# google-research/Splat-SLAM

Measured on AMD Instinct MI355X. Metric: mapping frames/sec + render ms @640x480, 300k Gaussians; PSNR vs ref, higher is better.
Workload: dtype f32

## Files before the change

include/splat_hip.h:

```cpp
#ifndef SPLAT_HIP_H_
#define SPLAT_HIP_H_

#include <stddef.h>
#include <stdint.h>

#ifdef __cplusplus
extern "C" {
#endif

#define SGR_ABI_VERSION 10

#define SGR_HOST

typedef enum SgrStatus {
  SGR_OK = 0,
  SGR_ERR_INVALID = -1,
  SGR_ERR_WORKSPACE = -2,
  SGR_ERR_CAPACITY = -3,
  SGR_ERR_HIP = -4
} SgrStatus;

typedef struct SgrSettings {
  int32_t num_gaussians;
  int32_t image_height;
  int32_t image_width;
  int32_t sh_degree;
  int32_t sh_coeffs;
  float tanfovx;
  float tanfovy;
  float scale_modifier;
  int32_t prefiltered;
  int32_t debug;
  const float* bg;
  const float* viewmatrix;
  const float* projmatrix;
  const float* projmatrix_raw;
  const float* campos;
} SgrSettings;

typedef struct SgrInputs {
  const float* means3D;
  const float* opacities;
  const float* shs;
  const float* colors_precomp;
  const float* scales;
  const float* rotations;
  const float* cov3D_precomp;
} SgrInputs;

typedef struct SgrOutputs {
  float* color;
  float* depth;
  float* opacity;
  int32_t* radii;
  int32_t* n_touched;
} SgrOutputs;

typedef struct SgrWorkspace {
  void* saved;
  size_t saved_bytes;
  void* scratch;
  size_t scratch_bytes;
  int64_t capacity;
  int32_t counters_clean;
  int32_t max_list_hint;
} SgrWorkspace;

typedef struct SgrGradOutputs {
  const float* dL_dcolor;
  const float* dL_ddepth;
} SgrGradOutputs;

typedef struct SgrGradInputs {
  float* dL_dmeans3D;
  float* dL_dmeans2D;
  float* dL_dopacities;
  float* dL_dshs;
  float* dL_dcolors_precomp;
  float* dL_dscales;
  float* dL_drotations;
  float* dL_dcov3D_precomp;
  float* dL_dtau;
  int32_t accumulate;
  float* stat_grad_accum;
  float* stat_denom;
  float* stat_max_radii;
} SgrGradInputs;

int sgr_abi_version(void);
const char* sgr_last_error(void);

size_t sgr_saved_bytes(int32_t num_gaussians, int32_t image_height, int32_t image_width, int64_t capacity);
size_t sgr_scratch_bytes(int32_t num_gaussians, int32_t image_height, int32_t image_width, int64_t capacity);

int sgr_forward(const SgrSettings* settings, const SgrInputs* in, const SgrOutputs* out,
                const SgrWorkspace* ws, SGR_HOST int64_t* num_rendered_host, void* stream);

int sgr_backward(const SgrSettings* settings, const SgrInputs* in, const int32_t* radii,
                 const SgrGradOutputs* grad_out, const SgrGradInputs* grad_in,
                 const SgrWorkspace* ws, void* stream);

typedef struct SgrBackwardView {
  SgrSettings settings;
  const int32_t* radii;
  SgrWorkspace ws;
  const float* dL_dcolor;
  const float* dL_ddepth;
  float* dL_dmeans2D;
  float* dL_dtau;
} SgrBackwardView;
int sgr_backward_views(int32_t num_views, const SgrBackwardView* views, const SgrInputs* in, const SgrGradInputs* grad_in,
                       void* stream);

int sgr_densify_stats(int64_t n, const float* dL_dmeans2D, const int32_t* radii, float* stat_grad_accum, float* stat_denom,
                      float* stat_max_radii, void* stream);

int sgr_query(const void* saved, SGR_HOST int64_t* num_rendered_host, SGR_HOST int32_t* overflow_host, void* stream);

int sgr_query_header(const void* saved, SGR_HOST uint32_t words_host[16], void* stream);

int sgr_header_to_host(const void* saved, void* pinned_host64, void* stream);

int sgr_query_stats(const SgrWorkspace* ws, int32_t num_gaussians, int32_t image_height, int32_t image_width,
                    const int32_t* radii, SGR_HOST int64_t stats_host[4], void* stream);
int sgr_query_depth_keys(const SgrWorkspace* ws, int32_t num_gaussians, int32_t image_height, int32_t image_width,
                         const int32_t* radii, float* depth_out, void* stream);
int sgr_query_list_histogram(const SgrWorkspace* ws, int32_t num_gaussians, int32_t image_height, int32_t image_width,
                             SGR_HOST int64_t hist_host[8], void* stream);

#define SGR_OPT_FUSED_BLEND 0
#define SGR_OPT_UPSTREAM_POSE_JACOBIAN 1
#define SGR_OPT_SEGMENT_TEST 2
#define SGR_OPT_COUNT 3
int sgr_set_option(int32_t option, int32_t value);
int sgr_get_option(int32_t option);

#define SGR_PROFILE_KINDS 7
int sgr_profile_enable(uint32_t kind_mask);
int sgr_profile_read(SGR_HOST float ms_host[SGR_PROFILE_KINDS], SGR_HOST int64_t launches_host[SGR_PROFILE_KINDS]);

int sgr_mapping_loss(int32_t H, int32_t W, const float* image, const float* depth,
                     const float* gt_image, const float* gt_depth,
                     const float* exposure_a, const float* exposure_b,
                     float alpha, float rgb_boundary_threshold, float upstream,
                     float* loss, float* dL_dimage, float* dL_ddepth, float* dL_dexp_a, float* dL_dexp_b,
                     void* scratch, size_t scratch_bytes, void* stream);

size_t sgr_ssim_scratch_bytes(int32_t B, int32_t C, int32_t H, int32_t W);
int sgr_ssim(int32_t B, int32_t C, int32_t H, int32_t W, const float* img1, const float* img2, float* ssim_out, float* maps,
             void* scratch, size_t scratch_bytes, void* stream);
int sgr_ssim_backward(int32_t B, int32_t C, int32_t H, int32_t W, const float* img1, const float* img2, const float* maps,
                      const float* upstream, int32_t upstream_stride, float upstream_scale, float* dL_dimg1, void* stream);

typedef struct SgrMetricFrame {
  const float* render;
  const float* gt_image;
  const float* depth;
  const float* gt_depth;
  const float* exposure_a;
  const float* exposure_b;
} SgrMetricFrame;
int sgr_render_metrics(int32_t n, const SgrMetricFrame* frames, int32_t C, int32_t H, int32_t W, float global_scale, float* out,
                       void* scratch, size_t scratch_bytes, void* stream);

#define SGR_TSDF_UNIT_FLOATS (5 * 4096)
#define SGR_TSDF_MAX_FRAMES 16
typedef struct SgrTsdfVolume {
  float voxel_length;
  float sdf_trunc;
  float depth_trunc;
  int32_t hash_capacity;
  int32_t pool_capacity;
  void* state;
  float* pool;
} SgrTsdfVolume;
typedef struct SgrTsdfFrame {
  const float* render;
  const float* depth;
  const float* gt_depth;
  const float* exposure_a;
  const float* exposure_b;
  float fx, fy, cx, cy;
  float w2c[16];
  float global_scale;
} SgrTsdfFrame;
size_t sgr_tsdf_bytes(int32_t hash_capacity);
int sgr_tsdf_reset(const SgrTsdfVolume* vol, void* stream);
int sgr_tsdf_rehash(const SgrTsdfVolume* src, const SgrTsdfVolume* dst, void* stream);
int sgr_tsdf_touch(const SgrTsdfVolume* vol, int32_t n, const SgrTsdfFrame* frames, int32_t H, int32_t W, void* stream);
int sgr_tsdf_integrate(const SgrTsdfVolume* vol, int32_t n, const SgrTsdfFrame* frames, int32_t H, int32_t W, int32_t n_touched,
                       void* stream);
size_t sgr_tsdf_extract_bytes(int32_t hash_capacity, int32_t pool_capacity);
int sgr_tsdf_extract_count(const SgrTsdfVolume* vol, int32_t n_units, void* scratch, size_t scratch_bytes, int32_t* totals,
                           void* stream);
int sgr_tsdf_extract(const SgrTsdfVolume* vol, int32_t n_units, void* scratch, size_t scratch_bytes, float* vertices,
                     float* colors, int32_t* triangles, void* stream);
size_t sgr_mesh_bytes(int32_t V, int32_t F);
int sgr_mesh_components(int32_t V, int32_t F, const float* vertices, const int32_t* triangles, int32_t min_len, void* scratch,
                        size_t scratch_bytes, int32_t* totals, void* stream);
int sgr_mesh_compact(int32_t V, int32_t F, const float* vertices, const float* colors, const int32_t* triangles, void* scratch,
                     size_t scratch_bytes, float* out_vertices, float* out_colors, int32_t* out_triangles, int32_t* vertex_map,
                     void* stream);

size_t sgr_surface_sample_bytes(int32_t F);
int sgr_surface_sample(int32_t V, int32_t F, const float* vertices, const int32_t* triangles, int32_t n, uint64_t seed, void* scratch,
                       size_t scratch_bytes, float* points, int32_t* tri_idx, double* total_area, void* stream);
size_t sgr_nn_grid_bytes(int32_t n);
int sgr_nn_grid_build(int32_t n, const float* points, SGR_HOST const float* transform, void* grid, size_t grid_bytes, void* stream);
int sgr_nn_query(int32_t n, const void* grid, size_t grid_bytes, int32_t nq, const float* query, SGR_HOST const float* transform,
                 float max_dist, float* dist, int32_t* idx, void* stream);
size_t sgr_eval_reduce_bytes(void);
int sgr_icp_accumulate(int32_t n, const float* source, SGR_HOST const float* transform, const int32_t* idx, int32_t n_target,
                       const float* target, double* sums, void* scratch, size_t scratch_bytes, void* stream);
int sgr_cloud_metrics(int32_t na, const float* dist_a, int32_t nb, const float* dist_b, float thresh, double* out, void* scratch,
                      size_t scratch_bytes, void* stream);

#define SGR_CULL_MAX_FRAMES 16
#define SGR_CULL_SUBPIXEL_BITS 8
#define SGR_CULL_GUARD_PIXELS 16384
#define SGR_CULL_RULE_ALL 0
#define SGR_CULL_RULE_ANY 1
typedef struct SgrCullFrame {
  double w2c[12];
  double fx, fy, cx, cy;
} SgrCullFrame;
int sgr_cull_project(int32_t V, const float* vertices, int32_t n, const SgrCullFrame* frames, double near, int32_t* xy, float* z,
                     void* stream);
size_t sgr_cull_raster_bytes(int32_t F, int32_t n);
int sgr_cull_raster(int32_t V, int32_t F, const int32_t* triangles, int32_t n, const int32_t* xy, const float* z, int32_t H, int32_t W,
                    float* depth, int32_t* skipped, void* scratch, size_t scratch_bytes, void* stream);
int sgr_cull_visibility(int32_t V, int32_t n, const int32_t* xy, const float* z, const float* depth, int32_t H, int32_t W, int32_t edge,
                        float far, float eps, int32_t* seen, void* stream);
size_t sgr_cull_select_bytes(int32_t V, int32_t F);
int sgr_cull_select(int32_t V, int32_t F, const int32_t* triangles, const int32_t* seen, int32_t min_views, int32_t rule, void* scratch,
                    size_t scratch_bytes, int32_t* totals, void* stream);
int sgr_cull_compact(int32_t V, int32_t F, const float* vertices, const float* colors, const int32_t* triangles, void* scratch,
                     size_t scratch_bytes, float* out_vertices, float* out_colors, int32_t* out_triangles, int32_t* vertex_map,
                     void* stream);

int sgr_adam_step(int64_t n, float* param, const float* grad, float* exp_avg, float* exp_avg_sq,
                  float lr, float beta1, float beta2, float eps, int64_t step, void* stream);

typedef struct SgrAdamTensor {
  float* param;
  const float* grad;
  float* exp_avg;
  float* exp_avg_sq;
  int64_t n;
  int64_t step;
} SgrAdamTensor;
int sgr_adam_step_multi(int32_t count, const SgrAdamTensor* tensors, float lr, float beta1, float beta2, float eps, void* stream);

int sgr_activate(int64_t n, const float* scaling, const float* rotation, const float* opacity,
                 float* scales_out, float* rot_out, float* opac_out, void* stream);

typedef struct SgrAdamGroup {
  float* param;
  float* grad;
  float* exp_avg;
  float* exp_avg_sq;
  float lr;
  int32_t skip;
  int64_t step;
} SgrAdamGroup;
int sgr_gaussian_adam_step(int64_t n, const SgrAdamGroup groups[5], float beta1, float beta2, float eps,
                           float iso_weight, void* stream);

int sgr_gaussian_adam_shard(int64_t n_total, const SgrAdamGroup groups[5], SGR_HOST const int64_t row0[5],
                            SGR_HOST const int64_t row1[5], float beta1, float beta2, float eps, float iso_weight, void* stream);

typedef struct SgrMapView {
  SgrSettings settings;
  SgrOutputs out;
  SgrWorkspace ws;
  const float* gt_image;
  const float* gt_depth;
  const float* exposure_a;
  const float* exposure_b;
  float* loss;
  float* dL_dimage;
  float* dL_ddepth;
  float* dL_dexposure;
  float* dL_dtau;
  void* loss_scratch;
  size_t loss_scratch_bytes;
} SgrMapView;
// ... 567 lines not shown
```

splat_slam_amd/csrc/sgr_api.hip:

```cpp
#include <cstdarg>
#include <cstdio>
#include <cstring>
#include <cstdlib>
#include <vector>

#include <hip/hip_runtime.h>

#include "sgr_common.h"

namespace sgr {

void launch_preprocess_fwd(const ViewTab&, int, const LOff&, const Common&, const SgrInputs&, hipStream_t);
void launch_preprocess_bwd(const ViewTab&, int, const LOff&, const Common&, const SgrInputs&, const SgrGradInputs&, const FusedAdam*,
                           hipStream_t, bool mapping_loop = false);
void launch_binning(const ViewTab&, int, const LOff&, hipStream_t);
void launch_zero_heads(const ViewTab&, int, const LOff&, size_t, hipStream_t);
void launch_blend_fwd(const ViewTab&, int, const LOff&, const float*, const LossTab*, const LossCoef*, hipStream_t);
void launch_blend_bwd(const ViewTab&, int, const LOff&, const float*, const LossTab*, const LossCoef*, hipStream_t);
void launch_blend_fused(const ViewTab&, int, const LOff&, const float*, const LossTab&, const LossCoef&, hipStream_t);
bool blend_can_fuse(const LOff&);

static int g_opt[SGR_OPT_COUNT] = {1, 0, 0};

static thread_local char g_err[512] = "";
int set_error(int code, const char* fmt, ...) {
  va_list ap;
  va_start(ap, fmt);
  vsnprintf(g_err, sizeof(g_err), fmt, ap);
  va_end(ap);
  return code;
}
#define HIP_TRY(expr)                                                                                   \
  do {                                                                                                  \
    hipError_t _e = (expr);                                                                             \
    if (_e != hipSuccess) return set_error(SGR_ERR_HIP, "%s failed: %s", #expr, hipGetErrorString(_e)); \
  } while (0)

int debug_flags() {
  static int f = -1;
  if (f < 0) { const char* e = getenv("SGR_DEBUG"); f = e ? atoi(e) : 0; }
  return f | (g_opt[SGR_OPT_SEGMENT_TEST] ? 0 : 4);
}

static Layout make_layout(int N, int H, int W, int64_t cap) { return Layout(N, H, W, cap); }

struct ProfState {
  static constexpr int kRing = 2048;
  uint32_t mask = 0;
  hipEvent_t ev[SGR_PROFILE_KINDS][kRing][2];
  bool created[SGR_PROFILE_KINDS] = {};
  int used[SGR_PROFILE_KINDS] = {};
  double ms[SGR_PROFILE_KINDS] = {};
  int64_t launches[SGR_PROFILE_KINDS] = {};
};
static ProfState g_prof;
static void prof_drain(int k) {
  for (int i = 0; i < g_prof.used[k]; ++i) {
    float t = 0.f;
    if (hipEventSynchronize(g_prof.ev[k][i][1]) == hipSuccess &&
        hipEventElapsedTime(&t, g_prof.ev[k][i][0], g_prof.ev[k][i][1]) == hipSuccess) {
      g_prof.ms[k] += t;
      g_prof.launches[k] += 1;
    }
  }
  g_prof.used[k] = 0;
}
void prof_begin(int k, hipStream_t st) {
  if (!(g_prof.mask & (1u << k))) return;
  if (!g_prof.created[k]) {
    for (int i = 0; i < ProfState::kRing; ++i) { (void)hipEventCreate(&g_prof.ev[k][i][0]); (void)hipEventCreate(&g_prof.ev[k][i][1]); }
    g_prof.created[k] = true;
  }
  if (g_prof.used[k] == ProfState::kRing) prof_drain(k);
  (void)hipEventRecord(g_prof.ev[k][g_prof.used[k]][0], st);
}
void prof_end(int k, hipStream_t st) {
  if (!(g_prof.mask & (1u << k))) return;
  (void)hipEventRecord(g_prof.ev[k][g_prof.used[k]][1], st);
  g_prof.used[k] += 1;
}

__global__ void __launch_bounds__(256) stats_kernel(int N, int ntiles, const int32_t* __restrict__ radii,
                                                     const uint2* __restrict__ ranges, const uint32_t* __restrict__ tile_maxc,
                                                     unsigned long long* __restrict__ out) {
  unsigned long long v = 0, r = 0, re = 0, ne = 0;
  for (int i = blockIdx.x * blockDim.x + threadIdx.x; i < N; i += gridDim.x * blockDim.x) v += radii[i] > 0;
  for (int t = blockIdx.x * blockDim.x + threadIdx.x; t < ntiles; t += gridDim.x * blockDim.x) {
    uint32_t c = ranges[(size_t)t * kRngStride].y - (ranges[(size_t)t * kRngStride].x & ~kOverfull);
    r += c; re += min(c, tile_maxc[t]); ne += c > 0;
  }
  atomicAdd(&out[0], v); atomicAdd(&out[1], r); atomicAdd(&out[2], re); atomicAdd(&out[3], ne);
}

__global__ void __launch_bounds__(256) hist_kernel(int ntiles, const uint2* __restrict__ ranges, const uint32_t* __restrict__ tile_maxc,
                                                    unsigned long long* __restrict__ out) {
  for (int t = blockIdx.x * blockDim.x + threadIdx.x; t < ntiles; t += gridDim.x * blockDim.x) {
    uint32_t c = ranges[(size_t)t * kRngStride].y - (ranges[(size_t)t * kRngStride].x & ~kOverfull);
    c = min(c, tile_maxc[t]);
    int b = c == 0 ? 0 : c <= 4 ? 1 : c <= 8 ? 2 : c <= 16 ? 3 : c <= 32 ? 4 : c <= 64 ? 5 : c <= 256 ? 6 : 7;
    atomicAdd(&out[b], 1ull);
  }
}


__global__ void __launch_bounds__(256) depth_keys_kernel(int N, const GRec* __restrict__ grec, const int32_t* __restrict__ radii,
                                                          float* __restrict__ out) {
  const int i = blockIdx.x * blockDim.x + threadIdx.x;
  if (i < N) out[i] = radii[i] > 0 ? grec[i].depth : 0.f;
}

static int check_settings(const SgrSettings* s, const SgrInputs* in) {
  const int N = s->num_gaussians, H = s->image_height, W = s->image_width;
  if (N < 0 || H <= 0 || W <= 0) return set_error(SGR_ERR_INVALID, "bad sizes N=%d H=%d W=%d", N, H, W);
  if (H > 65535 * kTile || W > 65535 * kTile) return set_error(SGR_ERR_INVALID, "image too large");
  if (!s->bg || !s->viewmatrix || !s->projmatrix || !s->projmatrix_raw || !s->campos)
    return set_error(SGR_ERR_INVALID, "settings: bg/viewmatrix/projmatrix/projmatrix_raw/campos must be device pointers");
  if (N > 0) {
    if (!in->means3D || !in->opacities) return set_error(SGR_ERR_INVALID, "means3D and opacities are required");
    if ((in->shs != nullptr) == (in->colors_precomp != nullptr))
      return set_error(SGR_ERR_INVALID, "Please provide excatly one of either SHs or precomputed colors!");
    if (((in->scales != nullptr) && (in->rotations != nullptr)) == (in->cov3D_precomp != nullptr) ||
        ((in->scales != nullptr) != (in->rotations != nullptr)))
      return set_error(SGR_ERR_INVALID, "Please provide exactly one of either scale/rotation pair or precomputed 3D covariance!");
    if (in->shs && (s->sh_degree < 0 || s->sh_degree > 3 || s->sh_coeffs < (s->sh_degree + 1) * (s->sh_degree + 1)))
      return set_error(SGR_ERR_INVALID, "sh_degree %d needs %d coefficients, shs has %d", s->sh_degree,
                       (s->sh_degree + 1) * (s->sh_degree + 1), s->sh_coeffs);
  }
  return SGR_OK;
}

static int check_workspace(const SgrWorkspace* ws, const Layout& L) {
  if (ws->capacity <= 0 || ws->capacity > 0xffffffffll) return set_error(SGR_ERR_INVALID, "bad capacity %lld", (long long)ws->capacity);
  if (!ws->saved || ws->saved_bytes < L.saved_bytes)
    return set_error(SGR_ERR_WORKSPACE, "saved workspace too small: %zu < %zu", ws->saved_bytes, L.saved_bytes);
  if (!ws->scratch || ws->scratch_bytes < L.scratch_bytes)
    return set_error(SGR_ERR_WORKSPACE, "scratch workspace too small: %zu < %zu", ws->scratch_bytes, L.scratch_bytes);
  return SGR_OK;
}

static Common make_common(const SgrSettings* s) {
  Common c;
  c.deg = s->sh_degree; c.M = s->sh_coeffs; c.tanfovx = s->tanfovx; c.tanfovy = s->tanfovy; c.mod = s->scale_modifier;
  c.bg = s->bg;
  c.upstream_pose_jac = g_opt[SGR_OPT_UPSTREAM_POSE_JACOBIAN];
  return c;
}

static void tab_set_view(ViewTab& t, int v, const SgrSettings* s, const SgrOutputs* out, const SgrWorkspace* ws) {
  t.viewmatrix[v] = s->viewmatrix; t.projmatrix[v] = s->projmatrix; t.campos[v] = s->campos; t.projraw[v] = s->projmatrix_raw;
  t.saved[v] = (char*)ws->saved; t.scratch[v] = (char*)ws->scratch;
  if (out) {
    t.color[v] = out->color; t.depth[v] = out->depth; t.opacity[v] = out->opacity; t.radii[v] = out->radii;
    t.n_touched[v] = out->n_touched;
  }
}

static int forward_batch(const ViewTab& tab, int nviews, const Layout& L, const Common& cm, const SgrInputs& in, hipStream_t st,
                         bool counters_clean = false, int max_list_hint = 0) {
  LOff d = L.dev();
  d.set_hint(max_list_hint);
  if (!counters_clean) launch_zero_heads(tab, nviews, d, L.zero_bytes, st);
  launch_preprocess_fwd(tab, nviews, d, cm, in, st);
  launch_binning(tab, nviews, d, st);
  return SGR_OK;
}

}

using namespace sgr;

extern "C" {

int sgr_abi_version(void) { return SGR_ABI_VERSION; }
const char* sgr_last_error(void) { return g_err; }

size_t sgr_saved_bytes(int32_t N, int32_t H, int32_t W, int64_t cap) { return make_layout(N, H, W, cap).saved_bytes; }
size_t sgr_scratch_bytes(int32_t N, int32_t H, int32_t W, int64_t cap) { return make_layout(N, H, W, cap).scratch_bytes; }

int sgr_forward(const SgrSettings* s, const SgrInputs* in, const SgrOutputs* out, const SgrWorkspace* ws,
                int64_t* num_rendered_host, void* stream) {
  if (!s || !in || !out || !ws) return set_error(SGR_ERR_INVALID, "null argument");
  if (int rc = check_settings(s, in)) return rc;
  const int N = s->num_gaussians;
  if (!out->color || !out->depth || !out->opacity || (N > 0 && (!out->radii || !out->n_touched)))
    return set_error(SGR_ERR_INVALID, "null output pointer");
  Layout L = make_layout(N, s->image_height, s->image_width, ws->capacity);
  if (int rc = check_workspace(ws, L)) return rc;
  hipStream_t st = (hipStream_t)stream;
  ViewTab tab = {};
  tab_set_view(tab, 0, s, out, ws);
  Common cm = make_common(s);
  if (int rc = forward_batch(tab, 1, L, cm, *in, st, ws->counters_clean != 0, ws->max_list_hint)) return rc;
  if (num_rendered_host) {
    uint32_t h2[2] = {0u, 0u};
    HIP_TRY(hipMemcpyAsync(h2, (char*)ws->saved + L.o_hdr, 8, hipMemcpyDeviceToHost, st));
    HIP_TRY(hipStreamSynchronize(st));
    const uint32_t R = h2[0];
    *num_rendered_host = R;
    if (h2[1] == 2u)
      return set_error(SGR_ERR_INVALID, "more than %u splats on one 8x8 tile: the map has degenerated (16-bit tile counters)", kTileCountLimit);
    if ((int64_t)R > L.cap) return set_error(SGR_ERR_CAPACITY, "%u (tile, Gaussian) pairs exceed capacity %lld", R, (long long)L.cap);
  }
  LOff d1 = L.dev();
  d1.set_hint(ws->max_list_hint);
  launch_blend_fwd(tab, 1, d1, s->bg, nullptr, nullptr, st);
  HIP_TRY(hipGetLastError());
  return SGR_OK;
}

int sgr_backward(const SgrSettings* s, const SgrInputs* in, const int32_t* radii, const SgrGradOutputs* go,
                 const SgrGradInputs* gi, const SgrWorkspace* ws, void* stream) {
  if (!s || !in || !go || !gi || !ws) return set_error(SGR_ERR_INVALID, "null argument");
  if (int rc = check_settings(s, in)) return rc;
  const int N = s->num_gaussians;
  if (!go->dL_dcolor) return set_error(SGR_ERR_INVALID, "dL_dcolor is required");
  if (N > 0 && !radii) return set_error(SGR_ERR_INVALID, "radii is required");
  if (gi->stat_grad_accum && (!gi->stat_denom || !gi->stat_max_radii))
    return set_error(SGR_ERR_INVALID, "stat_grad_accum needs stat_denom and stat_max_radii");
  Layout L = make_layout(N, s->image_height, s->image_width, ws->capacity);
  if (int rc = check_workspace(ws, L)) return rc;
  hipStream_t st = (hipStream_t)stream;
  if (N == 0) {
    if (gi->dL_dtau) HIP_TRY(hipMemsetAsync(gi->dL_dtau, 0, 24, st));
    return SGR_OK;
  }
  ViewTab tab = {};
  tab_set_view(tab, 0, s, nullptr, ws);
  tab.radii[0] = const_cast<int32_t*>(radii);
  tab.dL_dcolor[0] = go->dL_dcolor; tab.dL_ddepth[0] = go->dL_ddepth; tab.dL_dtau[0] = gi->dL_dtau;
  LOff d = L.dev();
  Common cm = make_common(s);
  launch_blend_bwd(tab, 1, d, s->bg, nullptr, nullptr, st);
  launch_preprocess_bwd(tab, 1, d, cm, *in, *gi, nullptr, st);
  HIP_TRY(hipGetLastError());
  return SGR_OK;
}

}

__global__ void __launch_bounds__(256) densify_stats_kernel(int64_t n, const float* __restrict__ m2, const int32_t* __restrict__ radii,
                                                            float* __restrict__ accum, float* __restrict__ denom, float* __restrict__ maxr) {
#pragma clang fp contract(off)
  const int64_t i = (int64_t)blockIdx.x * blockDim.x + threadIdx.x;
  if (i >= n) return;
  const int r = radii[i];
  if (r <= 0) return;
  const F3 g = ld3(m2 + 3 * i);
  accum[i] += sqrtf(g.x * g.x + g.y * g.y);
  denom[i] += 1.f;
  maxr[i] = fmaxf(maxr[i], (float)r);
}

extern "C" {

int sgr_densify_stats(int64_t n, const float* dL_dmeans2D, const int32_t* radii, float* stat_grad_accum, float* stat_denom,
                      float* stat_max_radii, void* stream) {
  if (n < 0 || (n > 0 && (!dL_dmeans2D || !radii || !stat_grad_accum || !stat_denom || !stat_max_radii)))
    return set_error(SGR_ERR_INVALID, "densify_stats: null argument");
  if (n > 0)
    hipLaunchKernelGGL(densify_stats_kernel, dim3((unsigned)((n + 255) / 256)), dim3(256), 0, (hipStream_t)stream, n, dL_dmeans2D, radii,
                       stat_grad_accum, stat_denom, stat_max_radii);
  HIP_TRY(hipGetLastError());
  return SGR_OK;
}

int sgr_backward_views(int32_t num_views, const SgrBackwardView* views, const SgrInputs* in, const SgrGradInputs* grad_in, void* stream) {
  if (num_views < 0 || (num_views > 0 && (!views || !in || !grad_in))) return set_error(SGR_ERR_INVALID, "backward_views: null argument");
  if (num_views == 0) return SGR_OK;
  hipStream_t st = (hipStream_t)stream;
  const SgrBackwardView& f = views[0];
  bool uniform = in->shs && in->scales && in->rotations && !in->colors_precomp && !in->cov3D_precomp && f.settings.sh_degree == 0 &&
                 f.settings.num_gaussians > 0;
  for (int v = 0; v < num_views; ++v) {
    const SgrBackwardView& m = views[v];
    if (int rc = check_settings(&m.settings, in)) return rc;
    if (!m.dL_dcolor || (m.settings.num_gaussians > 0 && !m.radii)) return set_error(SGR_ERR_INVALID, "backward_views: dL_dcolor and radii are required");
    uniform = uniform && m.settings.num_gaussians == f.settings.num_gaussians && m.settings.image_height == f.settings.image_height &&
              m.settings.image_width == f.settings.image_width && m.settings.tanfovx == f.settings.tanfovx &&
              m.settings.tanfovy == f.settings.tanfovy && m.settings.scale_modifier == f.settings.scale_modifier &&
              m.settings.sh_degree == f.settings.sh_degree && m.settings.sh_coeffs == f.settings.sh_coeffs &&
              m.settings.bg == f.settings.bg && m.ws.capacity == f.ws.capacity;
    for (int u = 0; u < v; ++u) uniform = uniform && views[u].ws.scratch != m.ws.scratch && views[u].ws.saved != m.ws.saved;
  }
  SgrGradInputs g = *grad_in;
  g.dL_dmeans2D = nullptr;
  g.dL_dtau = nullptr;
  if (!uniform) {
    for (int v = 0; v < num_views; ++v) {
      const SgrBackwardView& m = views[v];
      const int N = m.settings.num_gaussians;
      Layout L = make_layout(N, m.settings.image_height, m.settings.image_width, m.ws.capacity);
      if (int rc = check_workspace(&m.ws, L)) return rc;
      if (N == 0) {
        if (m.dL_dtau) HIP_TRY(hipMemsetAsync(m.dL_dtau, 0, 24, st));
        continue;
      }
      ViewTab tab = {};
      tab_set_view(tab, 0, &m.settings, nullptr, &m.ws);
      tab.radii[0] = const_cast<int32_t*>(m.radii);
      tab.dL_dcolor[0] = m.dL_dcolor; tab.dL_ddepth[0] = m.dL_ddepth; tab.dL_dtau[0] = m.dL_dtau; tab.dL_dmeans2D[0] = m.dL_dmeans2D;
      SgrGradInputs gv = g;
      gv.accumulate = (grad_in->accumulate || v > 0) ? 1 : 0;
      Common cm = make_common(&m.settings);
      LOff d = L.dev();
      launch_blend_bwd(tab, 1, d, m.settings.bg, nullptr, nullptr, st);
      launch_preprocess_bwd(tab, 1, d, cm, *in, gv, nullptr, st);
    }
    HIP_TRY(hipGetLastError());
    return SGR_OK;
  }
  Layout L = make_layout(f.settings.num_gaussians, f.settings.image_height, f.settings.image_width, f.ws.capacity);
  LOff d = L.dev();
  Common cm = make_common(&f.settings);
  for (int base = 0; base < num_views; base += kMaxViews) {
    const int nv = num_views - base < kMaxViews ? num_views - base : kMaxViews;
    ViewTab tab = {};
    for (int v = 0; v < nv; ++v) {
      const SgrBackwardView& m = views[base + v];
      if (int rc = check_workspace(&m.ws, L)) return rc;
      tab_set_view(tab, v, &m.settings, nullptr, &m.ws);
      tab.radii[v] = const_cast<int32_t*>(m.radii);
      tab.dL_dcolor[v] = m.dL_dcolor; tab.dL_ddepth[v] = m.dL_ddepth; tab.dL_dtau[v] = m.dL_dtau; tab.dL_dmeans2D[v] = m.dL_dmeans2D;
    }
    SgrGradInputs gv = g;
    gv.accumulate = (grad_in->accumulate || base > 0) ? 1 : 0;
    launch_blend_bwd(tab, nv, d, f.settings.bg, nullptr, nullptr, st);
    launch_preprocess_bwd(tab, nv, d, cm, *in, gv, nullptr, st);
  }
  HIP_TRY(hipGetLastError());
  return SGR_OK;
}

}

static int map_views_impl(int32_t num_views, const SgrMapView* views, const SgrInputs* in, const SgrGradInputs* grads, float alpha,
                          float rgb_boundary_threshold, int32_t forward_only, FusedAdam* fused, bool* fused_done,
                          void* stream, bool store_sinks = false, const SgrSsimTerm* term = nullptr) {
  if (fused_done) *fused_done = false;
  if (num_views < 0 || (num_views > 0 && (!views || !in)) || (!forward_only && !grads))
    return set_error(SGR_ERR_INVALID, "map_views: null argument");
  if (num_views == 0) return SGR_OK;
  if (forward_only) term = nullptr;
  if (term) {
    if (!term->arena || term->max_views <= 0)
      return set_error(SGR_ERR_INVALID, "map_views: SSIM term without an arena");
    for (int v = 0; v < num_views; ++v) {
      const SgrMapView& m = views[v];
      const int H = m.settings.image_height, W = m.settings.image_width;
      if (!m.out.color || !m.out.depth || !m.out.opacity)
        return set_error(SGR_ERR_INVALID, "map_views: the SSIM loss needs every view's rendered image, depth and opacity");
      if (term->arena_bytes < sgr_ssim_term_bytes(term->max_views, H, W))
        return set_error(SGR_ERR_WORKSPACE, "map_views: SSIM arena too small (need %zu for %d views of %dx%d)",
                         sgr_ssim_term_bytes(term->max_views, H, W), term->max_views, W, H);
      if (!m.loss_scratch || m.loss_scratch_bytes < (size_t)ssim_loss_nparts(H, W) * sizeof(LossPart))
        return set_error(SGR_ERR_WORKSPACE, "map_views: loss_scratch too small for the SSIM loss (need %zu)",
                         (size_t)ssim_loss_nparts(H, W) * sizeof(LossPart));
    }
  }
  hipStream_t st = (hipStream_t)stream;
  bool uniform = true;
  const SgrMapView& f = views[0];
  for (int v = 0; v < num_views; ++v) {
    const SgrMapView& m = views[v];
    if (int rc = check_settings(&m.settings, in)) return rc;
    uniform = uniform && m.settings.num_gaussians == f.settings.num_gaussians && m.settings.image_height == f.settings.image_height &&
              m.settings.image_width == f.settings.image_width && m.settings.tanfovx == f.settings.tanfovx &&
              m.settings.tanfovy == f.settings.tanfovy && m.settings.scale_modifier == f.settings.scale_modifier &&
              m.settings.sh_degree == f.settings.sh_degree && m.settings.sh_coeffs == f.settings.sh_coeffs &&
              m.settings.bg == f.settings.bg &&
              m.ws.capacity == f.ws.capacity;
    if (num_views > 1) uniform = uniform && in->shs && m.settings.sh_degree == 0 && in->scales && in->rotations;
    for (int u = 0; u < v; ++u) uniform = uniform && views[u].ws.scratch != m.ws.scratch && views[u].ws.saved != m.ws.saved;
    if (!forward_only && grads && !grads->accumulate && num_views > 1)
      return set_error(SGR_ERR_INVALID, "map_views: several views need accumulate != 0");
  }
  if (store_sinks && !forward_only && grads && !(fused && uniform && f.settings.num_gaussians > 0 && num_views <= kMaxViews)) {
    const size_t n = (size_t)f.settings.num_gaussians, m = (size_t)(f.settings.sh_coeffs > 0 ? f.settings.sh_coeffs : 1);
    if (grads->dL_dmeans3D) HIP_TRY(hipMemsetAsync(grads->dL_dmeans3D, 0, n * 12, st));
    if (grads->dL_dshs) HIP_TRY(hipMemsetAsync(grads->dL_dshs, 0, n * m * 12, st));
    if (grads->dL_dopacities) HIP_TRY(hipMemsetAsync(grads->dL_dopacities, 0, n * 4, st));
    if (grads->dL_dscales) HIP_TRY(hipMemsetAsync(grads->dL_dscales, 0, n * 12, st));
    if (grads->dL_drotations) HIP_TRY(hipMemsetAsync(grads->dL_drotations, 0, n * 16, st));
  }
  if (!uniform || f.settings.num_gaussians == 0) {
    for (int v = 0; v < num_views; ++v) {
      const SgrMapView& mv = views[v];
      if (!mv.out.color || !mv.out.depth || !mv.out.opacity || !mv.out.n_touched)
        return set_error(SGR_ERR_INVALID, "map_views: outputs may only be omitted in uniform batches");
      if (int rc = sgr_forward(&mv.settings, in, &mv.out, &mv.ws, nullptr, stream)) return rc;
      if (forward_only) continue;
      if (term) {
        if (int rc = sgr_mapping_loss_ssim(mv.settings.image_height, mv.settings.image_width, mv.out.color, mv.out.depth, mv.gt_image,
                                           mv.gt_depth, mv.exposure_a, mv.exposure_b, alpha, rgb_boundary_threshold, 1.0f, term,
                                           mv.loss, mv.dL_dimage, mv.dL_ddepth, mv.dL_dexposure,
                                           mv.dL_dexposure ? mv.dL_dexposure + 1 : nullptr, stream))
          return rc;
      } else if (int rc = sgr_mapping_loss(mv.settings.image_height, mv.settings.image_width, mv.out.color, mv.out.depth, mv.gt_image,
                                           mv.gt_depth, mv.exposure_a, mv.exposure_b, alpha, rgb_boundary_threshold, 1.0f, mv.loss,
                                           mv.dL_dimage, mv.dL_ddepth, mv.dL_dexposure, mv.dL_dexposure ? mv.dL_dexposure + 1 : nullptr,
                                           mv.loss_scratch, mv.loss_scratch_bytes, stream)) {
        return rc;
      }
      SgrGradOutputs go = {mv.dL_dimage, mv.dL_ddepth};
      SgrGradInputs gi = *grads;
      gi.dL_dtau = mv.dL_dtau;
      if (int rc = sgr_backward(&mv.settings, in, mv.out.radii, &go, &gi, &mv.ws, stream)) return rc;
    }
    return SGR_OK;
  }
  Layout L = make_layout(f.settings.num_gaussians, f.settings.image_height, f.settings.image_width, f.ws.capacity);
  LOff d = L.dev();
  int hint = 0;
  for (int v = 0; v < num_views; ++v) hint = views[v].ws.max_list_hint > hint ? views[v].ws.max_list_hint : hint;
  d.set_hint(hint);
  Common cm = make_common(&f.settings);
  const int HW = f.settings.image_height * f.settings.image_width;
  for (int base = 0; base < num_views; base += kMaxViews) {
    const int nv = num_views - base < kMaxViews ? num_views - base : kMaxViews;
    ViewTab tab = {};
    LossTab lt = {};
    bool all_clean = true;
    for (int v = 0; v < nv; ++v) {
      const SgrMapView& m = views[base + v];
      all_clean = all_clean && m.ws.counters_clean != 0;
      if (int rc = check_workspace(&m.ws, L)) return rc;
      const bool no_images = !m.out.color && !m.out.depth && !m.out.opacity && !forward_only;
      if ((!no_images && (!m.out.color || !m.out.depth || !m.out.opacity)) || !m.out.radii)
        return set_error(SGR_ERR_INVALID, "map_views: null output pointer");
      tab_set_view(tab, v, &m.settings, &m.out, &m.ws);
      if (!forward_only) {
        if (!m.gt_image || !m.gt_depth || !m.dL_dimage || !m.dL_ddepth || !m.loss_scratch ||
            m.loss_scratch_bytes < (size_t)L.ntiles * sizeof(LossPart))
          return set_error(SGR_ERR_INVALID, "map_views: loss buffers missing (loss_scratch needs 16 B per 8x8 tile = %zu)",
                           (size_t)L.ntiles * sizeof(LossPart));
        tab.dL_dcolor[v] = m.dL_dimage; tab.dL_ddepth[v] = m.dL_ddepth; tab.dL_dtau[v] = m.dL_dtau;
        lt.image[v] = m.out.color; lt.depth[v] = m.out.depth; lt.gt_image[v] = m.gt_image; lt.gt_depth[v] = m.gt_depth;
        lt.exp_a[v] = m.exposure_a; lt.exp_b[v] = m.exposure_b; lt.loss[v] = m.loss; lt.dimage[v] = m.dL_dimage;
        lt.ddepth[v] = m.dL_ddepth; lt.da[v] = m.dL_dexposure; lt.db[v] = m.dL_dexposure ? m.dL_dexposure + 1 : nullptr;
        lt.parts[v] = m.loss_scratch;
      }
    }
    if (int rc = forward_batch(tab, nv, L, cm, *in, st, all_clean, d.mean_hint)) return rc;
    if (forward_only) {
      launch_blend_fwd(tab, nv, d, f.settings.bg, nullptr, nullptr, st);
      continue;
    }
    LossCoef lc = {alpha / (3.f * (float)HW), (1.f - alpha) / (float)HW, rgb_boundary_threshold};
    const bool fused_blend = !term && g_opt[SGR_OPT_FUSED_BLEND] != 0 && blend_can_fuse(d);
    int nparts = L.ntiles;
    if (term) {
      const int H = f.settings.image_height, W = f.settings.image_width;
      launch_blend_fwd(tab, nv, d, f.settings.bg, nullptr, nullptr, st);
      for (int g0 = 0; g0 < nv; g0 += term->max_views)
        launch_ssim_mapping_loss(lt, g0, nv - g0 < term->max_views ? nv - g0 : term->max_views, H, W, alpha, term->lambda_dssim,
                                 rgb_boundary_threshold, 1.f, (float*)term->arena, st);
      nparts = ssim_loss_nparts(H, W);
    } else if (fused_blend) {
      launch_blend_fused(tab, nv, d, f.settings.bg, lt, lc, st);
    } else {
      launch_blend_fwd(tab, nv, d, f.settings.bg, &lt, &lc, st);
    }
    const bool fuse = fused && num_views <= kMaxViews;
    if (fuse) {
      fused->tail_views = nv; fused->tail_nparts = nparts;
      fused->tail_inv_rgb = 1.f / (3.f * (float)HW); fused->tail_inv_dep = 1.f / (float)HW; fused->tail_alpha = alpha;
      for (int v = 0; v < nv; ++v) {
        fused->tail_parts[v] = lt.parts[v]; fused->tail_loss[v] = lt.loss[v]; fused->tail_da[v] = lt.da[v]; fused->tail_db[v] = lt.db[v];
      }
    } else {
      launch_mapping_loss_final(lt, nv, HW, nparts, alpha, st);
    }
    if (term) launch_blend_bwd(tab, nv, d, f.settings.bg, nullptr, nullptr, st);
    else if (!fused_blend) launch_blend_bwd(tab, nv, d, f.settings.bg, &lt, &lc, st);
    launch_preprocess_bwd(tab, nv, d, cm, *in, *grads, fuse ? fused : nullptr, st, true);
    if (fuse && fused_done) *fused_done = true;
  }
  HIP_TRY(hipGetLastError());
  return SGR_OK;
}

extern "C" {

int sgr_map_views(int32_t num_views, const SgrMapView* views, const SgrInputs* in, const SgrGradInputs* grads, float alpha,
                  float rgb_boundary_threshold, int32_t forward_only, void* stream) {
  return map_views_impl(num_views, views, in, grads, alpha, rgb_boundary_threshold, forward_only, nullptr, nullptr, stream);
}

}

static int map_step_impl(const SgrMapStep* p, bool skip_activate, bool grads_clean, bool allow_fuse, bool* fused_out, void* stream,
                         const SgrSsimTerm* term = nullptr) {
  if (fused_out) *fused_out = false;
  if (!p) return set_error(SGR_ERR_INVALID, "map_step: null argument");
  const bool adam_only = p->num_views == 0 && p->adam_groups;
  if (!skip_activate && !adam_only && (p->scaling || p->rotation || p->opacity))
    if (int rc = sgr_activate(p->num_gaussians, p->scaling, p->rotation, p->opacity, p->scales_out, p->rot_out, p->opac_out, stream)) return rc;
  FusedAdam fa;
  bool try_fuse = false;
  if (allow_fuse && p->adam_groups && p->num_views > 0 && p->num_views <= kMaxViews && !p->forward_only && p->grads && p->in && p->views) {
    const SgrGradInputs& g = *p->grads;
    const SgrAdamGroup* G = p->adam_groups;
    try_fuse = g.accumulate && g.dL_dmeans3D == G[0].grad && g.dL_dshs == G[1].grad && g.dL_dopacities == G[2].grad &&
               g.dL_dscales == G[3].grad && g.dL_drotations == G[4].grad && !g.dL_dmeans2D && !g.dL_dcolors_precomp &&
               !g.dL_dcov3D_precomp && p->in->shs && !p->in->colors_precomp && p->in->scales && p->in->rotations &&
               p->num_gaussians == p->views[0].settings.num_gaussians;
    for (int v = 0; v < p->num_views && try_fuse; ++v)
      try_fuse = !p->views[v].dL_dtau && p->views[v].settings.sh_degree == 0 && p->views[v].settings.sh_coeffs == 1;
    if (try_fuse) {
      if (int rc = make_fused_adam(p->num_gaussians, G, p->beta1, p->beta2, p->eps, p->iso_weight, &fa)) return rc;
      fa.grads_clean = grads_clean ? 1 : 0;
      fa.s_out = p->scales_out; fa.r_out = p->rot_out; fa.o_out = p->opac_out;
      fa.stat_accum = g.stat_grad_accum;
      fa.stat_denom = g.stat_grad_accum ? g.stat_denom : nullptr;
      fa.stat_maxr = g.stat_grad_accum ? g.stat_max_radii : nullptr;
      if (p->exp_rows > 0) {
        if (!p->exp_param || !p->exp_grad || !p->exp_avg || !p->exp_avg_sq || !p->exp_step || !p->exp_active || p->exp_row_width <= 0)
          return set_error(SGR_ERR_INVALID, "map_step: exposure block incomplete");
        fa.exp_rows = p->exp_rows; fa.exp_width = p->exp_row_width; fa.exp_param = p->exp_param; fa.exp_grad = p->exp_grad;
        fa.exp_avg = p->exp_avg; fa.exp_avg_sq = p->exp_avg_sq; fa.exp_step = p->exp_step; fa.exp_active = p->exp_active;
        fa.exp_lr = p->exp_lr; fa.exp_b1 = p->exp_beta1; fa.exp_b2 = p->exp_beta2; fa.exp_eps = p->exp_eps;
      }
    }
  }
  if ((p->grads_clean == -2 || p->grads_clean == -3) && !p->adam_groups && p->num_views > 0 && p->num_views <= kMaxViews && !p->forward_only && p->grads &&
      p->in && p->views) {
    const SgrGradInputs& g = *p->grads;
    try_fuse = g.accumulate && g.dL_dmeans3D && g.dL_dshs && g.dL_dopacities && g.dL_dscales && g.dL_drotations &&
               !g.dL_dmeans2D && !g.dL_dcolors_precomp && !g.dL_dcov3D_precomp && p->in->shs && !p->in->colors_precomp &&
               p->in->scales && p->in->rotations && p->num_gaussians == p->views[0].settings.num_gaussians;
    for (int v = 0; v < p->num_views && try_fuse; ++v)
      try_fuse = !p->views[v].dL_dtau && p->views[v].settings.sh_degree == 0 && p->views[v].settings.sh_coeffs == 1;
    if (try_fuse) {
      fa = FusedAdam{};
      fa.gather_only = p->grads_clean == -3 ? 2 : 1;
      fa.G.g[0].grad = g.dL_dmeans3D; fa.G.g[1].grad = g.dL_dshs; fa.G.g[2].grad = g.dL_dopacities;
      fa.G.g[3].grad = g.dL_dscales; fa.G.g[4].grad = g.dL_drotations;
      fa.stat_accum = g.stat_grad_accum;
      fa.stat_denom = g.stat_grad_accum ? g.stat_denom : nullptr;
      fa.stat_maxr = g.stat_grad_accum ? g.stat_max_radii : nullptr;
      if (p->exp_rows > 0) {
        if (!p->exp_param || !p->exp_grad || !p->exp_avg || !p->exp_avg_sq || !p->exp_step || !p->exp_active || p->exp_row_width <= 0)
          return set_error(SGR_ERR_INVALID, "map_step: exposure block incomplete");
        fa.exp_rows = p->exp_rows; fa.exp_width = p->exp_row_width; fa.exp_param = p->exp_param; fa.exp_grad = p->exp_grad;
        fa.exp_avg = p->exp_avg; fa.exp_avg_sq = p->exp_avg_sq; fa.exp_step = p->exp_step; fa.exp_active = p->exp_active;
        fa.exp_lr = p->exp_lr; fa.exp_b1 = p->exp_beta1; fa.exp_b2 = p->exp_beta2; fa.exp_eps = p->exp_eps;
      }
    }
  }
  bool fused = false;
  if (p->num_views > 0)
    if (int rc = map_views_impl(p->num_views, p->views, p->in, p->grads, p->alpha, p->rgb_boundary_threshold, p->forward_only,
                                try_fuse ? &fa : nullptr, &fused, stream, p->grads_clean == -3 && !p->adam_groups, term))
      return rc;
  if (p->adam_groups && !fused)
    if (int rc = gaussian_adam_step_act(p->num_gaussians, p->adam_groups, p->beta1, p->beta2, p->eps, p->iso_weight,
                                        adam_only && p->scaling ? p->scales_out : nullptr,
                                        adam_only && p->rotation ? p->rot_out : nullptr,
                                        adam_only && p->opacity ? p->opac_out : nullptr, stream))
      return rc;
  if (p->exp_rows > 0 && !fused)
    if (int rc = sgr_masked_adam(p->exp_rows, p->exp_row_width, p->exp_param, p->exp_grad, p->exp_avg, p->exp_avg_sq, p->exp_step,
                                 p->exp_active, p->exp_lr, p->exp_beta1, p->exp_beta2, p->exp_eps, stream))
      return rc;
  if (fused_out) *fused_out = fused;
  return SGR_OK;
}

extern "C" {

int sgr_map_step(const SgrMapStep* p, void* stream) {
  if (!p) return set_error(SGR_ERR_INVALID, "map_step: null argument");
  return map_step_impl(p, false, p->grads_clean > 0, p->grads_clean >= 0, nullptr, stream);
}

int sgr_map_step_ssim(const SgrMapStep* p, const SgrSsimTerm* term, void* stream) {
  if (!p) return set_error(SGR_ERR_INVALID, "map_step: null argument");
  return map_step_impl(p, false, p->grads_clean > 0, p->grads_clean >= 0, nullptr, stream, term);
}

}

static int map_run_impl(const SgrMapRun* r, const SgrSsimTerm* term, void* stream) {
  if (!r || r->num_iters < 0 || r->num_window < 0 || r->picks_per_iter < 0 || (r->num_window > 0 && !r->window) ||
      (r->picks_per_iter > 0 && (!r->pool || !r->picks || r->pool_size <= 0)))
    return set_error(SGR_ERR_INVALID, "map_run: bad argument");
  const int nv = r->num_window + r->picks_per_iter;
  if (nv > 64) return set_error(SGR_ERR_INVALID, "map_run: more than 64 views per iteration");
  SgrMapView views[64];
  for (int v = 0; v < r->num_window; ++v) views[v] = r->window[v];
  std::vector<char> pool_used((size_t)(r->pool_size > 0 ? r->pool_size : 0), 0);
  std::vector<char> slot_used((size_t)(r->picks_per_iter > 0 ? r->picks_per_iter : 0), 0);
  SgrMapStep st = r->step;
  st.views = views;
  st.num_views = nv;
  st.adam_groups = r->adam_groups;
  const int32_t exp_rows = st.exp_rows;
  bool prev_fused = false;
  for (int it = 0; it < r->num_iters; ++it) {
    for (int j = 0; j < r->picks_per_iter; ++j) {
      const int32_t k = r->picks[(size_t)it * r->picks_per_iter + j];
      if (k < 0 || k >= r->pool_size) return set_error(SGR_ERR_INVALID, "map_run: pick %d outside the pool", k);
      views[r->num_window + j] = r->pool[k];
      if (r->pick_ws) {
        views[r->num_window + j].ws = r->pick_ws[j];
        if (slot_used[j]) views[r->num_window + j].ws.counters_clean = 1;
        slot_used[j] = 1;
      } else if (pool_used[k]) {
        views[r->num_window + j].ws.counters_clean = 1;
      }
      pool_used[k] = 1;
    }
    if (it == 1)
      for (int v = 0; v < r->num_window; ++v) views[v].ws.counters_clean = 1;
    if (r->n_touched_last_only) {
      const bool last = it == r->num_iters - 1;
      for (int v = 0; v < r->num_window; ++v) views[v].out.n_touched = last ? r->window[v].out.n_touched : nullptr;
      if (!last)
        for (int j = 0; j < r->picks_per_iter; ++j) views[r->num_window + j].out.n_touched = nullptr;
    }
    if (r->adam_groups) {
      if (r->lr0) r->adam_groups[0].lr = r->lr0[it];
      for (int g = 0; g < 5; ++g)
        if (!r->adam_groups[g].skip) r->adam_groups[g].step += 1;
    }
    if (r->pool_exp_row && r->picks_per_iter > 0 && exp_rows > 0) {
      const int32_t row = r->pool_exp_row[r->picks[(size_t)it * r->picks_per_iter]];
      const size_t o = (size_t)(row < 0 ? 0 : row) * (size_t)st.exp_row_width;
      st.exp_rows = row < 0 ? 0 : 1;
      st.exp_param = r->step.exp_param + o; st.exp_grad = r->step.exp_grad + o;
      st.exp_avg = r->step.exp_avg + o; st.exp_avg_sq = r->step.exp_avg_sq + o;
      st.exp_step = r->step.exp_step + (row < 0 ? 0 : row);
    }
    bool fused = false;
    if (int rc = map_step_impl(&st, prev_fused, it == 0 ? r->step.grads_clean > 0 : r->adam_groups != nullptr, r->step.grads_clean >= 0,
                               &fused, stream, term))
      return rc;
    prev_fused = fused;
  }
  return SGR_OK;
}

extern "C" {

int sgr_map_run(const SgrMapRun* r, void* stream) { return map_run_impl(r, nullptr, stream); }
int sgr_map_run_ssim(const SgrMapRun* r, const SgrSsimTerm* term, void* stream) { return map_run_impl(r, term, stream); }

int sgr_query_stats(const SgrWorkspace* ws, int32_t N, int32_t H, int32_t W, const int32_t* radii, int64_t stats_host[4],
                    void* stream) {
  if (!ws || !ws->saved || !ws->scratch || !stats_host) return set_error(SGR_ERR_INVALID, "null argument");
  Layout L = make_layout(N, H, W, ws->capacity);
  hipStream_t st = (hipStream_t)stream;
  unsigned long long* d = (unsigned long long*)ws->scratch;
  HIP_TRY(hipMemsetAsync(d, 0, 32, st));
  hipLaunchKernelGGL(stats_kernel, dim3(64), dim3(256), 0, st, N, L.ntiles, radii, (const uint2*)((char*)ws->saved + L.o_ranges),
                     (const uint32_t*)((char*)ws->saved + L.o_tile_maxc), d);
  unsigned long long h[4];
  HIP_TRY(hipMemcpyAsync(h, d, 32, hipMemcpyDeviceToHost, st));
  HIP_TRY(hipStreamSynchronize(st));
  for (int i = 0; i < 4; ++i) stats_host[i] = (int64_t)h[i];
  return SGR_OK;
}

int sgr_query_depth_keys(const SgrWorkspace* ws, int32_t N, int32_t H, int32_t W, const int32_t* radii, float* depth_out, void* stream) {
  if (!ws || !ws->saved || !radii || !depth_out) return set_error(SGR_ERR_INVALID, "null argument");
  Layout L = make_layout(N, H, W, ws->capacity);
  if (N > 0)
    hipLaunchKernelGGL(depth_keys_kernel, dim3((N + 255) / 256), dim3(256), 0, (hipStream_t)stream, N,
                       (const GRec*)((const char*)ws->saved + L.o_grec), radii, depth_out);
  HIP_TRY(hipGetLastError());
  return SGR_OK;
}

int sgr_query_list_histogram(const SgrWorkspace* ws, int32_t N, int32_t H, int32_t W, int64_t hist_host[8], void* stream) {
  if (!ws || !ws->saved || !ws->scratch || !hist_host) return set_error(SGR_ERR_INVALID, "null argument");
  Layout L = make_layout(N, H, W, ws->capacity);
  hipStream_t st = (hipStream_t)stream;
  unsigned long long* d = (unsigned long long*)ws->scratch;
  HIP_TRY(hipMemsetAsync(d, 0, 64, st));
  hipLaunchKernelGGL(hist_kernel, dim3(32), dim3(256), 0, st, L.ntiles, (const uint2*)((char*)ws->saved + L.o_ranges),
                     (const uint32_t*)((char*)ws->saved + L.o_tile_maxc), d);
  unsigned long long h[8];
  HIP_TRY(hipMemcpyAsync(h, d, 64, hipMemcpyDeviceToHost, st));
  HIP_TRY(hipStreamSynchronize(st));
  for (int i = 0; i < 8; ++i) hist_host[i] = (int64_t)h[i];
  return SGR_OK;
}

int sgr_set_option(int32_t option, int32_t value) {
  if (option < 0 || option >= SGR_OPT_COUNT) return set_error(SGR_ERR_INVALID, "unknown option %d", option);
  g_opt[option] = value;
  return SGR_OK;
}

int sgr_get_option(int32_t option) { return option >= 0 && option < SGR_OPT_COUNT ? g_opt[option] : -1; }

int sgr_profile_enable(uint32_t kind_mask) {
  g_prof.mask = kind_mask & ((1u << SGR_PROFILE_KINDS) - 1);
  return SGR_OK;
}

int sgr_profile_read(float ms_host[SGR_PROFILE_KINDS], int64_t launches_host[SGR_PROFILE_KINDS]) {
  for (int k = 0; k < SGR_PROFILE_KINDS; ++k) {
    prof_drain(k);
    if (ms_host) ms_host[k] = (float)g_prof.ms[k];
    if (launches_host) launches_host[k] = g_prof.launches[k];
    g_prof.ms[k] = 0.0;
    g_prof.launches[k] = 0;
  }
  return SGR_OK;
}

int sgr_header_to_host(const void* saved, void* pinned_host64, void* stream) {
  if (!saved || !pinned_host64) return set_error(SGR_ERR_INVALID, "null argument");
  HIP_TRY(hipMemcpyAsync(pinned_host64, saved, sizeof(SavedHeader), hipMemcpyDeviceToHost, (hipStream_t)stream));
  return SGR_OK;
}

int sgr_query_header(const void* saved, uint32_t words_host[16], void* stream) {
  if (!saved || !words_host) return set_error(SGR_ERR_INVALID, "null argument");
  static_assert(sizeof(SavedHeader) == 64, "header is 16 words");
  HIP_TRY(hipMemcpyAsync(words_host, saved, sizeof(SavedHeader), hipMemcpyDeviceToHost, (hipStream_t)stream));
  HIP_TRY(hipStreamSynchronize((hipStream_t)stream));
  return SGR_OK;
}

int sgr_query(const void* saved, int64_t* num_rendered_host, int32_t* overflow_host, void* stream) {
  if (!saved) return set_error(SGR_ERR_INVALID, "null saved block");
  SavedHeader h;
  HIP_TRY(hipMemcpyAsync(&h, saved, sizeof(h), hipMemcpyDeviceToHost, (hipStream_t)stream));
  HIP_TRY(hipStreamSynchronize((hipStream_t)stream));
  if (num_rendered_host) *num_rendered_host = h.num_rendered;
  if (overflow_host) *overflow_host = (int32_t)h.overflow;
  return SGR_OK;
}

}
```

splat_slam_amd/csrc/sgr_aux.hip:

```cpp
#include <cmath>

#include <cstdint>

#include "sgr_common.h"
#include "sgr_se3_device.h"

namespace sgr {
int set_error(int code, const char* fmt, ...);


__global__ void __launch_bounds__(256) mapping_loss_kernel(LossTab tab, int HW, float w_rgb, float w_dep, float thr) {
  const int vw = blockIdx.y;
  const float* __restrict__ image = tab.image[vw];
  const float* __restrict__ depth = tab.depth[vw];
  const float* __restrict__ gt_image = tab.gt_image[vw];
  const float* __restrict__ gt_depth = tab.gt_depth[vw];
  float* __restrict__ dimage = tab.dimage[vw];
  float* __restrict__ ddepth = tab.ddepth[vw];
  LossPart* __restrict__ parts = (LossPart*)tab.parts[vw];
  const float ea = tab.exp_a[vw] ? __expf(tab.exp_a[vw][0]) : 1.f;
  const float eb = tab.exp_b[vw] ? tab.exp_b[vw][0] : 0.f;
  LossPart acc = {0.f, 0.f, 0.f, 0.f};
  for (int p = blockIdx.x * blockDim.x + threadIdx.x; p < HW; p += gridDim.x * blockDim.x) {
    float g0 = gt_image[p], g1 = gt_image[HW + p], g2 = gt_image[2 * HW + p];
    bool m = (g0 + g1 + g2) > thr;
    float gt[3] = {g0, g1, g2};
#pragma unroll
    for (int c = 0; c < 3; ++c) {
      float I = image[c * HW + p];
      float r = m ? (ea * I + eb) - gt[c] : 0.f;
      acc.rgb += fabsf(r);
      float sgn = (r > 0.f) ? 1.f : ((r < 0.f) ? -1.f : 0.f);
      float dab = w_rgb * sgn;
      if (dimage) dimage[c * HW + p] = dab * ea;
      acc.da += dab * ea * I;
      acc.db += dab;
    }
    float gd = gt_depth[p];
    bool md = gd > 0.01f;
    float rd = md ? depth[p] - gd : 0.f;
    acc.dep += fabsf(rd);
    if (ddepth) ddepth[p] = w_dep * ((rd > 0.f) ? 1.f : ((rd < 0.f) ? -1.f : 0.f));
  }
  __shared__ LossPart red[4];
  float v[4] = {acc.rgb, acc.dep, acc.da, acc.db};
#pragma unroll
  for (int k = 0; k < 4; ++k) v[k] = wave_sum(v[k]);
  int lane = threadIdx.x & 63, wv = threadIdx.x >> 6;
  if (lane == 0) red[wv] = {v[0], v[1], v[2], v[3]};
  __syncthreads();
  if (threadIdx.x == 0) {
    LossPart t = red[0];
    for (int w = 1; w < 4; ++w) { t.rgb += red[w].rgb; t.dep += red[w].dep; t.da += red[w].da; t.db += red[w].db; }
    parts[blockIdx.x] = t;
  }
}

__device__ __forceinline__ void loss_final_view(const LossPart* __restrict__ parts, int nparts, float inv_rgb, float inv_dep,
                                                float alpha, float* loss, float* da, float* db, LossPart* red ) {
#pragma clang fp contract(off)
  LossPart t = {0.f, 0.f, 0.f, 0.f};
  for (int i = threadIdx.x; i < nparts; i += 256) {
    LossPart p = parts[i];
    t.rgb += p.rgb; t.dep += p.dep; t.da += p.da; t.db += p.db;
  }
  float v[4] = {t.rgb, t.dep, t.da, t.db};
#pragma unroll
  for (int k = 0; k < 4; ++k) v[k] = wave_sum(v[k]);
  const int lane = threadIdx.x & 63, wv = threadIdx.x >> 6;
  if (lane == 0) red[wv] = {v[0], v[1], v[2], v[3]};
  __syncthreads();
  if (threadIdx.x == 0) {
    LossPart s = red[0];
    for (int w = 1; w < 4; ++w) { s.rgb += red[w].rgb; s.dep += red[w].dep; s.da += red[w].da; s.db += red[w].db; }
    if (loss) loss[0] = alpha * (s.rgb * inv_rgb) + (1.f - alpha) * (s.dep * inv_dep);
    if (da) da[0] = s.da;
    if (db) db[0] = s.db;
  }
  __syncthreads();
}

__global__ void __launch_bounds__(256) mapping_loss_final_kernel(LossTab tab, int nparts, float inv_rgb, float inv_dep, float alpha) {
  __shared__ LossPart red[4];
  const int vw = blockIdx.x;
  loss_final_view((const LossPart*)tab.parts[vw], nparts, inv_rgb, inv_dep, alpha, tab.loss[vw], tab.da[vw], tab.db[vw], red);
}

static int loss_blocks(int HW) {
  int blocks = (HW + 255) / 256;
  return blocks > 1024 ? 1024 : blocks;
}

void launch_mapping_loss_final(const LossTab& tab, int nviews, int HW, int nparts, float alpha, hipStream_t st) {
  float inv_rgb = 1.f / (3.f * (float)HW), inv_dep = 1.f / (float)HW;
  hipLaunchKernelGGL(mapping_loss_final_kernel, dim3(nviews), dim3(256), 0, st, tab, nparts, inv_rgb, inv_dep, alpha);
}

void launch_mapping_loss(const LossTab& tab, int nviews, int HW, float alpha, float thr, float upstream, hipStream_t st) {
  int blocks = loss_blocks(HW);
  float inv_rgb = 1.f / (3.f * (float)HW), inv_dep = 1.f / (float)HW;
  hipLaunchKernelGGL(mapping_loss_kernel, dim3(blocks, nviews), dim3(256), 0, st, tab, HW, upstream * alpha * inv_rgb,
                     upstream * (1.f - alpha) * inv_dep, thr);
  hipLaunchKernelGGL(mapping_loss_final_kernel, dim3(nviews), dim3(256), 0, st, tab, blocks, inv_rgb, inv_dep, alpha);
}

__global__ void __launch_bounds__(256) adam_kernel(int64_t n, float* __restrict__ p, const float* __restrict__ g,
                                                   float* __restrict__ m, float* __restrict__ v, float b1, float b2,
                                                   float eps, float step_size, float bc2_sqrt) {
  for (int64_t i = (int64_t)blockIdx.x * blockDim.x + threadIdx.x; i < n; i += (int64_t)gridDim.x * blockDim.x) {
    float gi = g[i];
    float mi = m[i], vi = v[i];
    mi = mi + (gi - mi) * (1.f - b1);
    vi = vi * b2 + (1.f - b2) * gi * gi;
    float denom = sqrtf(vi) / bc2_sqrt + eps;
    p[i] = p[i] - step_size * (mi / denom);
    m[i] = mi;
    v[i] = vi;
  }
}

constexpr int kAdamMulti = 48;
struct AdamMulti {
  float* p[kAdamMulti]; const float* g[kAdamMulti]; float* m[kAdamMulti]; float* v[kAdamMulti];
  int32_t n[kAdamMulti]; float step_size[kAdamMulti], bc2_sqrt[kAdamMulti];
};
__global__ void __launch_bounds__(256) adam_multi_kernel(AdamMulti t, float b1, float b2, float eps) {
  const int k = blockIdx.x;
  float* __restrict__ p = t.p[k]; const float* __restrict__ g = t.g[k]; float* __restrict__ m = t.m[k]; float* __restrict__ v = t.v[k];
  const float step_size = t.step_size[k], bc2_sqrt = t.bc2_sqrt[k];
  for (int i = threadIdx.x; i < t.n[k]; i += blockDim.x) {
    float gi = g[i];
    float mi = m[i], vi = v[i];
    mi = mi + (gi - mi) * (1.f - b1);
    vi = vi * b2 + (1.f - b2) * gi * gi;
    float denom = sqrtf(vi) / bc2_sqrt + eps;
    p[i] = p[i] - step_size * (mi / denom);
    m[i] = mi;
    v[i] = vi;
  }
}

__device__ __forceinline__ void masked_adam_row(int r, int width, float* __restrict__ p, const float* __restrict__ g,
                                                float* __restrict__ m, float* __restrict__ v, int32_t* __restrict__ step,
                                                float lr, float b1, float b2, float eps) {
#pragma clang fp contract(off)
  int st = step[r] + 1;
  step[r] = st;
  float bc1 = 1.f - powf(b1, (float)st), bc2 = 1.f - powf(b2, (float)st);
  float step_size = lr / bc1, bc2s = sqrtf(bc2);
  for (int k = 0; k < width; ++k) {
    int i = r * width + k;
    float gi = g[i], mi = m[i], vi = v[i];
    mi = mi + (gi - mi) * (1.f - b1);
    vi = vi * b2 + (1.f - b2) * gi * gi;
    p[i] = p[i] - step_size * (mi / (sqrtf(vi) / bc2s + eps));
    m[i] = mi;
    v[i] = vi;
  }
}

__global__ void masked_adam_kernel(int rows, int width, float* __restrict__ p, const float* __restrict__ g,
                                   float* __restrict__ m, float* __restrict__ v, int32_t* __restrict__ step,
                                   const int32_t* __restrict__ active, float lr, float b1, float b2, float eps) {
#pragma clang fp contract(off)
  int r = blockIdx.x * blockDim.x + threadIdx.x;
  if (r >= rows || !active[r]) return;
  masked_adam_row(r, width, p, g, m, v, step, lr, b1, b2, eps);
}

__global__ void __launch_bounds__(256) activate_kernel(int64_t n, const float* __restrict__ scaling,
                                                       const float* __restrict__ rotation, const float* __restrict__ opacity,
                                                       float* __restrict__ s_out, float* __restrict__ r_out,
                                                       float* __restrict__ o_out) {
#pragma clang fp contract(off)
  int64_t i = (int64_t)blockIdx.x * blockDim.x + threadIdx.x;
  if (i >= n) return;
  if (s_out) {
    const F3 sc = ld3(scaling + 3 * i);
    st3(s_out + 3 * i, F3{expf(sc.x), expf(sc.y), expf(sc.z)});
  }
  if (r_out) {
    float4 q = *(const float4*)(rotation + 4 * i);
    float nn = fmaxf(sqrtf(q.x * q.x + q.y * q.y + q.z * q.z + q.w * q.w), 1e-12f);
    *(float4*)(r_out + 4 * i) = make_float4(q.x / nn, q.y / nn, q.z / nn, q.w / nn);
  }
  if (o_out) o_out[i] = 1.f / (1.f + expf(-opacity[i]));
}

#define adam_update(p, g, m, v, GRP, c)                      \
  do {                                                       \
    m = m + (g - m) * (1.f - c.b1);                          \
    v = v * c.b2 + (1.f - c.b2) * g * g;                     \
    float denom_ = sqrtf(v) / c.bc2_sqrt[GRP] + c.eps;       \
    p = p - c.step_size[GRP] * (m / denom_);                 \
  } while (0)

template <int MODE>
__device__ __forceinline__ float take_grad(float* __restrict__ sink, int64_t j, float gathered) {
  if (MODE == 2) return gathered;
  float g = sink[j];
  sink[j] = 0.f;
  return MODE == 1 ? g + gathered : g;
}

template <int MODE>
__device__ __forceinline__ void gaussian_adam_one(int64_t i, const AdamGroups& G, const AdamConst& c, float iso_coef,
                                                  const float* e , float* __restrict__ s_out,
                                                  float* __restrict__ r_out, float* __restrict__ o_out) {
#pragma clang fp contract(off)
#pragma unroll
  for (int grp = 0; grp < 2; ++grp) {
    const SgrAdamGroup& A = G.g[grp];
    if (i < G.r0[grp] || i >= G.r1[grp]) continue;
    float g[3];
    if (MODE == 2) {
      g[0] = e[3 * grp]; g[1] = e[3 * grp + 1]; g[2] = e[3 * grp + 2];
    } else {
      F3 gs = ld3(A.grad + 3 * i);
      st3(A.grad + 3 * i, F3{0.f, 0.f, 0.f});
      g[0] = gs.x; g[1] = gs.y; g[2] = gs.z;
      if (MODE == 1) { g[0] = g[0] + e[3 * grp]; g[1] = g[1] + e[3 * grp + 1]; g[2] = g[2] + e[3 * grp + 2]; }
    }
    if (A.skip) continue;
    F3 p3 = ld3(A.param + 3 * i), m3 = ld3(A.exp_avg + 3 * i), v3 = ld3(A.exp_avg_sq + 3 * i);
    float p[3] = {p3.x, p3.y, p3.z}, m[3] = {m3.x, m3.y, m3.z}, v[3] = {v3.x, v3.y, v3.z};
#pragma unroll
    for (int k = 0; k < 3; ++k) adam_update(p[k], g[k], m[k], v[k], grp, c);
    st3(A.param + 3 * i, F3{p[0], p[1], p[2]});
    st3(A.exp_avg + 3 * i, F3{m[0], m[1], m[2]});
    st3(A.exp_avg_sq + 3 * i, F3{v[0], v[1], v[2]});
  }
  if (i >= G.r0[2] && i < G.r1[2]) {
    const SgrAdamGroup& A = G.g[2];
    float p = A.param[i];
    float sg = 1.f / (1.f + expf(-p));
    float g = take_grad<MODE>(A.grad, i, e[6]) * sg * (1.f - sg);
    if (!A.skip) {
      float m = A.exp_avg[i], v = A.exp_avg_sq[i];
      adam_update(p, g, m, v, 2, c);
      A.param[i] = p; A.exp_avg[i] = m; A.exp_avg_sq[i] = v;
    }
    if (o_out) o_out[i] = 1.f / (1.f + expf(-p));
  }
  if (i >= G.r0[3] && i < G.r1[3]) {
    const SgrAdamGroup& A = G.g[3];
    const F3 p3 = ld3(A.param + 3 * i);
    float p[3] = {p3.x, p3.y, p3.z}, s[3];
#pragma unroll
    for (int k = 0; k < 3; ++k) s[k] = expf(p[k]);
    float mean = (s[0] + s[1] + s[2]) / 3.f;
    float sg[3], ssum = 0.f;
#pragma unroll
    for (int k = 0; k < 3; ++k) { float d = s[k] - mean; sg[k] = d > 0.f ? 1.f : (d < 0.f ? -1.f : 0.f); ssum += sg[k]; }
    float gin[3];
    if (MODE == 2) {
      gin[0] = e[7]; gin[1] = e[8]; gin[2] = e[9];
    } else {
      F3 gs = ld3(A.grad + 3 * i);
      st3(A.grad + 3 * i, F3{0.f, 0.f, 0.f});
      gin[0] = gs.x; gin[1] = gs.y; gin[2] = gs.z;
      if (MODE == 1) { gin[0] = gin[0] + e[7]; gin[1] = gin[1] + e[8]; gin[2] = gin[2] + e[9]; }
    }
    if (!A.skip) {
      F3 m3 = ld3(A.exp_avg + 3 * i), v3 = ld3(A.exp_avg_sq + 3 * i);
      float m[3] = {m3.x, m3.y, m3.z}, v[3] = {v3.x, v3.y, v3.z};
#pragma unroll
      for (int k = 0; k < 3; ++k) {
        float gs = gin[k] + iso_coef * (sg[k] - ssum / 3.f);
        float g = gs * s[k];
        adam_update(p[k], g, m[k], v[k], 3, c);
      }
      st3(A.param + 3 * i, F3{p[0], p[1], p[2]});
      st3(A.exp_avg + 3 * i, F3{m[0], m[1], m[2]});
      st3(A.exp_avg_sq + 3 * i, F3{v[0], v[1], v[2]});
    }
    if (s_out) st3(s_out + 3 * i, F3{expf(p[0]), expf(p[1]), expf(p[2])});
  }
  if (i >= G.r0[4] && i < G.r1[4]) {
    const SgrAdamGroup& A = G.g[4];
    float4 x = *(const float4*)(A.param + 4 * i);
    float4 gy;
    if (MODE == 2) {
      gy = make_float4(e[10], e[11], e[12], e[13]);
    } else {
      gy = *(const float4*)(A.grad + 4 * i);
      *(float4*)(A.grad + 4 * i) = make_float4(0.f, 0.f, 0.f, 0.f);
      if (MODE == 1) { gy.x += e[10]; gy.y += e[11]; gy.z += e[12]; gy.w += e[13]; }
    }
    float nrm = sqrtf(x.x * x.x + x.y * x.y + x.z * x.z + x.w * x.w);
    float gx[4];
    if (nrm > 1e-12f) {
      float inv = 1.f / nrm;
      float y[4] = {x.x * inv, x.y * inv, x.z * inv, x.w * inv};
      float dot = y[0] * gy.x + y[1] * gy.y + y[2] * gy.z + y[3] * gy.w;
      gx[0] = (gy.x - y[0] * dot) * inv; gx[1] = (gy.y - y[1] * dot) * inv;
      gx[2] = (gy.z - y[2] * dot) * inv; gx[3] = (gy.w - y[3] * dot) * inv;
    } else {
      gx[0] = gy.x * 1e12f; gx[1] = gy.y * 1e12f; gx[2] = gy.z * 1e12f; gx[3] = gy.w * 1e12f;
    }
    float pp[4] = {x.x, x.y, x.z, x.w};
    if (!A.skip) {
      float4 m = *(const float4*)(A.exp_avg + 4 * i), v = *(const float4*)(A.exp_avg_sq + 4 * i);
      float mm[4] = {m.x, m.y, m.z, m.w}, vv[4] = {v.x, v.y, v.z, v.w};
#pragma unroll
      for (int k = 0; k < 4; ++k) adam_update(pp[k], gx[k], mm[k], vv[k], 4, c);
      *(float4*)(A.param + 4 * i) = make_float4(pp[0], pp[1], pp[2], pp[3]);
      *(float4*)(A.exp_avg + 4 * i) = make_float4(mm[0], mm[1], mm[2], mm[3]);
      *(float4*)(A.exp_avg_sq + 4 * i) = make_float4(vv[0], vv[1], vv[2], vv[3]);
    }
    if (r_out) {
      float nn = fmaxf(sqrtf(pp[0] * pp[0] + pp[1] * pp[1] + pp[2] * pp[2] + pp[3] * pp[3]), 1e-12f);
      *(float4*)(r_out + 4 * i) = make_float4(pp[0] / nn, pp[1] / nn, pp[2] / nn, pp[3] / nn);
    }
  }
}

__global__ void __launch_bounds__(256) gaussian_adam_kernel(int64_t n, AdamGroups G, AdamConst c, float iso_coef,
                                                            float* __restrict__ s_out, float* __restrict__ r_out,
                                                            float* __restrict__ o_out) {
  int64_t i = (int64_t)blockIdx.x * blockDim.x + threadIdx.x;
  if (i >= n) return;
  const float zero[14] = {0.f, 0.f, 0.f, 0.f, 0.f, 0.f, 0.f, 0.f, 0.f, 0.f, 0.f, 0.f, 0.f, 0.f};
  gaussian_adam_one<0>(i, G, c, iso_coef, zero, s_out, r_out, o_out);
}

template <int MODE>
__global__ void __launch_bounds__(256) gather_adam_kernel(ViewTab tab, int nviews, LOff L, FusedAdam fa) {
  if ((int)blockIdx.x < fa.tail_views) {
    __shared__ LossPart red[4];
    const int v = blockIdx.x;
    loss_final_view((const LossPart*)fa.tail_parts[v], fa.tail_nparts, fa.tail_inv_rgb, fa.tail_inv_dep, fa.tail_alpha,
                    fa.tail_loss[v], fa.tail_da[v], fa.tail_db[v], red);
    if (threadIdx.x == 0 && fa.exp_rows > 0 && fa.tail_da[v] && ((const SavedHeader*)tab.saved[v])->overflow == 0u) {
      const ptrdiff_t d = fa.tail_da[v] - fa.exp_grad;
      if (d >= 0 && d < (ptrdiff_t)fa.exp_rows * fa.exp_width && d % fa.exp_width == 0) {
        const int r = (int)(d / fa.exp_width);
        if (fa.exp_active[r])
          masked_adam_row(r, fa.exp_width, fa.exp_param, fa.exp_grad, fa.exp_avg, fa.exp_avg_sq, fa.exp_step, fa.exp_lr,
                          fa.exp_b1, fa.exp_b2, fa.exp_eps);
      }
    }
    return;
  }
  __shared__ const char* s_scratch[kMaxViews];
  __shared__ const int32_t* s_radii[kMaxViews];
  __shared__ uint32_t s_over[kMaxViews];
#pragma unroll
  for (int u = 0; u < kMaxViews; ++u)
    if ((int)threadIdx.x == u && u < nviews) {
      s_scratch[u] = tab.scratch[u];
      s_radii[u] = tab.radii[u];
      s_over[u] = ((const SavedHeader*)tab.saved[u])->overflow;
    }
  __syncthreads();
  uint32_t truncated = 0u;
  for (int u = 0; u < nviews; ++u) truncated |= (s_over[u] != 0u ? 1u : 0u) << u;
  const int i = ((int)blockIdx.x - fa.tail_views) * blockDim.x + threadIdx.x;
  if (i >= L.N) return;
  float a[14];
#pragma unroll
  for (int k = 0; k < 14; ++k) a[k] = 0.f;
  float st_norm = 0.f, st_cnt = 0.f, st_maxr = 0.f;
  uint32_t seen = 0u;
  for (int p = 0; p < min(L.k1_parts, nviews); ++p) seen |= ((const uint32_t*)(tab.saved[0] + L.o_vismask))[(size_t)p * L.N + i];
  seen &= ~truncated;
  const bool any = seen != 0u;
  while (seen) {
    const int v = __builtin_ctz(seen);
    seen &= seen - 1u;
    const float4* rec = (const float4*)(s_scratch[v] + L.o_gradrec) + (size_t)i * 4;
    const int r = s_radii[v][i];
    float4 r0 = rec[0], r1 = rec[1], r2 = rec[2], r3 = rec[3];
    a[0] += r0.x; a[1] += r0.y; a[2] += r0.z; a[3] += r0.w; a[4] += r1.x; a[5] += r1.y; a[6] += r1.z; a[7] += r1.w;
    a[8] += r2.x; a[9] += r2.y; a[10] += r2.z; a[11] += r2.w; a[12] += r3.x; a[13] += r3.y;
    st_norm += sqrtf(r3.z * r3.z + r3.w * r3.w);
    st_cnt += 1.f;
    st_maxr = fmaxf(st_maxr, (float)r);
  }
  if (any && fa.stat_accum) {
    fa.stat_accum[i] += st_norm;
    fa.stat_denom[i] += st_cnt;
    fa.stat_maxr[i] = fmaxf(fa.stat_maxr[i], st_maxr);
  }
  if (MODE == 3) {
    if (!any) return;
    float* g0 = fa.G.g[0].grad + 3 * (size_t)i; float* g1 = fa.G.g[1].grad + 3 * (size_t)i; float* g3 = fa.G.g[3].grad + 3 * (size_t)i;
    float* g4 = fa.G.g[4].grad + 4 * (size_t)i;
    g0[0] += a[0]; g0[1] += a[1]; g0[2] += a[2];
    g1[0] += a[3]; g1[1] += a[4]; g1[2] += a[5];
    fa.G.g[2].grad[i] += a[6];
    g3[0] += a[7]; g3[1] += a[8]; g3[2] += a[9];
    g4[0] += a[10]; g4[1] += a[11]; g4[2] += a[12]; g4[3] += a[13];
    return;
  }
  if (MODE == 4) {
    st3(fa.G.g[0].grad + 3 * (size_t)i, F3{a[0], a[1], a[2]});
    st3(fa.G.g[1].grad + 3 * (size_t)i, F3{a[3], a[4], a[5]});
    fa.G.g[2].grad[i] = a[6];
    st3(fa.G.g[3].grad + 3 * (size_t)i, F3{a[7], a[8], a[9]});
    *(float4*)(fa.G.g[4].grad + 4 * (size_t)i) = make_float4(a[10], a[11], a[12], a[13]);
    return;
  }
  gaussian_adam_one<MODE >= 3 ? 1 : MODE>(i, fa.G, fa.c, fa.iso_coef, a, fa.s_out, fa.r_out, fa.o_out);
}

int gaussian_adam_step_act(int64_t n, const SgrAdamGroup groups[5], float beta1, float beta2, float eps, float iso_weight,
                           float* s_out, float* r_out, float* o_out, void* stream) {
  if (n < 0 || !groups) return set_error(SGR_ERR_INVALID, "gaussian_adam: bad argument");
  if (n == 0) return SGR_OK;
  FusedAdam fa;
  if (int rc = make_fused_adam(n, groups, beta1, beta2, eps, iso_weight, &fa)) return rc;
  hipLaunchKernelGGL(gaussian_adam_kernel, dim3((unsigned)((n + 255) / 256)), dim3(256), 0, (hipStream_t)stream, n, fa.G, fa.c,
                     fa.iso_coef, s_out, r_out, o_out);
  return hipGetLastError() == hipSuccess ? SGR_OK : set_error(SGR_ERR_HIP, "gaussian_adam launch failed");
}

void launch_gather_adam(const ViewTab& tab, int nviews, const LOff& L, const FusedAdam& fa, hipStream_t st) {
  if (L.N <= 0) return;
  const int grid = L.pre_blocks + fa.tail_views;
  if (fa.gather_only == 2)
    hipLaunchKernelGGL(gather_adam_kernel<4>, dim3(grid), dim3(256), 0, st, tab, nviews, L, fa);
  else if (fa.gather_only)
    hipLaunchKernelGGL(gather_adam_kernel<3>, dim3(grid), dim3(256), 0, st, tab, nviews, L, fa);
  else if (fa.grads_clean)
    hipLaunchKernelGGL(gather_adam_kernel<2>, dim3(grid), dim3(256), 0, st, tab, nviews, L, fa);
  else
    hipLaunchKernelGGL(gather_adam_kernel<1>, dim3(grid), dim3(256), 0, st, tab, nviews, L, fa);
}

struct Top3 { float a, b, c; };
__device__ __forceinline__ void top3_push(Top3& t, float d) {
  if (d < t.c) {
    if (d < t.b) {
      t.c = t.b;
      if (d < t.a) { t.b = t.a; t.a = d; } else { t.b = d; }
    } else {
      t.c = d;
    }
  }
}

__global__ void __launch_bounds__(256) knn_partial_kernel(int n, const float* __restrict__ xyz, int per_split,
                                                          Top3* __restrict__ part) {
  __shared__ float sx[256], sy[256], sz[256];
  int i = blockIdx.x * 256 + threadIdx.x;
  float qx = 0.f, qy = 0.f, qz = 0.f;
  if (i < n) { qx = xyz[3 * i]; qy = xyz[3 * i + 1]; qz = xyz[3 * i + 2]; }
  Top3 best = {INFINITY, INFINITY, INFINITY};
  int j0 = blockIdx.y * per_split, j1 = min(n, j0 + per_split);
  for (int base = j0; base < j1; base += 256) {
    int j = base + threadIdx.x;
    if (j < j1) { sx[threadIdx.x] = xyz[3 * j]; sy[threadIdx.x] = xyz[3 * j + 1]; sz[threadIdx.x] = xyz[3 * j + 2]; }
    __syncthreads();
    int cnt = min(256, j1 - base);
    for (int k = 0; k < cnt; ++k) {
      float dx = sx[k] - qx, dy = sy[k] - qy, dz = sz[k] - qz;
      float d = dx * dx + dy * dy + dz * dz;
      if (base + k != i) top3_push(best, d);
    }
    __syncthreads();
  }
  if (i < n) part[(size_t)blockIdx.y * n + i] = best;
}

__global__ void __launch_bounds__(256) knn_merge_kernel(int n, int splits, const Top3* __restrict__ part,
                                                        float* __restrict__ out) {
  int i = blockIdx.x * 256 + threadIdx.x;
  if (i >= n) return;
  Top3 best = {INFINITY, INFINITY, INFINITY};
  for (int s = 0; s < splits; ++s) {
    Top3 t = part[(size_t)s * n + i];
    top3_push(best, t.a); top3_push(best, t.b); top3_push(best, t.c);
  }
  float a = isinf(best.a) ? 0.f : best.a, b = isinf(best.b) ? 0.f : best.b, c = isinf(best.c) ? 0.f : best.c;
  out[i] = (a + b + c) / 3.f;
}

static int knn_splits(int n) {
  int qb = (n + 255) / 256;
  int s = (2048 + qb - 1) / qb;
  if (s < 1) s = 1;
  if (s > 64) s = 64;
  int max_s = (n + 255) / 256;
  if (s > max_s) s = max_s;
  return s < 1 ? 1 : s;
}

constexpr int kKnnGridFrom = 16384;
struct KnnGrid { float lo[3]; float h, inv_h, eps; int g[3]; int cells; };
__device__ __forceinline__ uint32_t knn_ordered(float f) { const uint32_t u = __float_as_uint(f); return (u & 0x80000000u) ? ~u : (u | 0x80000000u); }
__device__ __forceinline__ float knn_unordered(uint32_t u) { return __uint_as_float((u & 0x80000000u) ? (u & 0x7fffffffu) : ~u); }
static size_t knn_max_cells(int n) { return (size_t)n / 2 + 1024; }

__global__ void __launch_bounds__(256) knn_bounds_kernel(int n, const float* __restrict__ xyz, uint32_t* __restrict__ mm ) {
  __shared__ float red[4][6];
  float lo[3] = {INFINITY, INFINITY, INFINITY}, hi[3] = {-INFINITY, -INFINITY, -INFINITY};
  for (int i = blockIdx.x * blockDim.x + threadIdx.x; i < n; i += gridDim.x * blockDim.x) {
    const F3 p = ld3(xyz + 3 * (size_t)i);
    lo[0] = fminf(lo[0], p.x); hi[0] = fmaxf(hi[0], p.x);
    lo[1] = fminf(lo[1], p.y); hi[1] = fmaxf(hi[1], p.y);
    lo[2] = fminf(lo[2], p.z); hi[2] = fmaxf(hi[2], p.z);
  }
#pragma unroll
  for (int k = 0; k < 3; ++k) {
    for (int off = 32; off > 0; off >>= 1) { lo[k] = fminf(lo[k], __shfl_xor(lo[k], off)); hi[k] = fmaxf(hi[k], __shfl_xor(hi[k], off)); }
    if ((threadIdx.x & 63) == 0) { red[threadIdx.x >> 6][k] = lo[k]; red[threadIdx.x >> 6][3 + k] = hi[k]; }
  }
  __syncthreads();
  if (threadIdx.x < 6) {
    const int k = threadIdx.x;
    if (k < 3) atomicMin(&mm[k], knn_ordered(fminf(fminf(red[0][k], red[1][k]), fminf(red[2][k], red[3][k]))));
    else atomicMax(&mm[k], knn_ordered(fmaxf(fmaxf(red[0][k], red[1][k]), fmaxf(red[2][k], red[3][k]))));
  }
}

__global__ void knn_grid_setup_kernel(int n, int max_cells, const uint32_t* __restrict__ mm, KnnGrid* __restrict__ out) {
  if (threadIdx.x != 0 || blockIdx.x != 0) return;
  KnnGrid G;
  float ext[3], amax = 0.f;
  for (int k = 0; k < 3; ++k) {
    const float lo = knn_unordered(mm[k]), hi = knn_unordered(mm[3 + k]);
    G.lo[k] = lo;
    ext[k] = fmaxf(hi - lo, 0.f);
    amax = fmaxf(amax, fmaxf(fabsf(lo), fabsf(hi)));
  }
  const float emax = fmaxf(ext[0], fmaxf(ext[1], ext[2]));
  float vol = 1.f;
  for (int k = 0; k < 3; ++k) vol *= fmaxf(ext[k], emax * (1.f / 1024.f));
  float h = emax > 0.f ? cbrtf(vol * 8.f / (float)n) : 1.f;
  h = fmaxf(h, emax * (1.f / 1024.f));
  if (!(h > 0.f) || !isfinite(h)) h = 1.f;
  for (int iter = 0; iter < 32; ++iter) {
    long long cells = 1;
    for (int k = 0; k < 3; ++k) { G.g[k] = min(1024, max(1, (int)floorf(ext[k] / h) + 1)); cells *= G.g[k]; }
    if (cells <= (long long)max_cells) break;
    h *= 1.26f;
  }
  G.cells = G.g[0] * G.g[1] * G.g[2];
  G.h = h; G.inv_h = 1.f / h;
  G.eps = 8e-6f * (amax + emax) + 1e-30f;
  *out = G;
}

__device__ __forceinline__ int knn_cell_coord(float v, float lo, float inv_h, int g) { return min(g - 1, max(0, (int)floorf((v - lo) * inv_h))); }

__global__ void __launch_bounds__(256) knn_count_kernel(int n, const float* __restrict__ xyz, const KnnGrid* __restrict__ Gp,
                                                        uint32_t* __restrict__ count, uint32_t* __restrict__ cell_of) {
  const int i = blockIdx.x * 256 + threadIdx.x;
  if (i >= n) return;
  const KnnGrid G = *Gp;
  const int cx = knn_cell_coord(xyz[3 * i], G.lo[0], G.inv_h, G.g[0]), cy = knn_cell_coord(xyz[3 * i + 1], G.lo[1], G.inv_h, G.g[1]),
            cz = knn_cell_coord(xyz[3 * i + 2], G.lo[2], G.inv_h, G.g[2]);
  const uint32_t c = (uint32_t)((cz * G.g[1] + cy) * G.g[0] + cx);
  cell_of[i] = c;
  atomicAdd(&count[c], 1u);
}
// ... 352 lines not shown
```

splat_slam_amd/csrc/sgr_common.h:

```cpp
#pragma once

#include <hip/hip_runtime.h>
#include <stdint.h>

#include "../../include/splat_hip.h"

namespace sgr {

constexpr float kNearPlane = 0.001f;
constexpr float kAlphaMin = 1.0f / 255.0f;
constexpr float kAlphaMax = 0.99f;
constexpr float kTEps = 1e-4f;
constexpr float kDilation = 0.3f;
constexpr float kTouchedT = 0.5f;
constexpr int kRefTile = 16;
constexpr int kTile = 8;
constexpr int kWave = 64;
constexpr int kCntSlotWords = 8;
constexpr uint32_t kTileCountLimit = 0xff00u;
__host__ __device__ inline size_t tile_counter_word(int x, int y, int gxp) { return ((size_t)(y >> 1) * gxp + (x >> 1)) * (kCntSlotWords / 2); }
__host__ __device__ inline int tile_counter_shift(int x, int y) { return 16 * ((y & 1) * 2 + (x & 1)); }
constexpr int kK1MaxParts = 4;
#ifndef SGR_K1_DENSE_PARTS
#define SGR_K1_DENSE_PARTS 2
// ... 104 lines not shown
      o_tile_maxc, o_final_T, o_tile_order, o_block_touched, o_block_vis, o_block_base_t, o_block_base_v, o_vis_list,
      o_seg_list, o_vismask, o_entries, o_bucket, o_ovf, o_partials, o_tau_part, o_gradrec, o_taurec;
};
#ifndef SGR_TILE_ORDER_MIN_LIST
#define SGR_TILE_ORDER_MIN_LIST 64
#endif
__host__ __device__ inline bool tile_order_used(const LOff& L) { return !(L.mean_hint != 0 && L.mean_hint <= SGR_TILE_ORDER_MIN_LIST); }
struct __attribute__((aligned(16))) OvfEntry { uint32_t tile, rank; uint64_t key; };
struct Common {
  int deg, M;
  int upstream_pose_jac;
  float tanfovx, tanfovy, mod;
  const float* bg;
};

int debug_flags();

struct __attribute__((aligned(16))) GRec {
  float px, py;
  uint32_t rect01, rect23;
  float A, B, C, opacity;
  float r, g, b, depth;
  uint32_t touched, offset, vis_pos, clamped;
};
static_assert(sizeof(GRec) == 64, "GRec must be one 64-byte record");
struct Rect { int x0, y0, x1, y1; };
__device__ __forceinline__ Rect unpack_rect(uint32_t r01, uint32_t r23) {
  return {(int)(r01 & 0xffffu), (int)(r01 >> 16), (int)(r23 & 0xffffu), (int)(r23 >> 16)};
}

struct Layout {
  int N, H, W;
  int64_t cap;
  int gx, gy, ntiles;
  int sgx, sgy;
  int tile_bits;
  size_t o_hdr, o_tile_count, o_grec, o_point_list, o_ranges,
      o_tile_maxc, o_final_T, o_tile_order, o_block_touched, o_block_vis, o_block_base_t, o_block_base_v, o_vis_list,
      o_seg_list, o_vismask, saved_bytes, zero_bytes;
  size_t o_entries, o_bucket, o_ovf;
  size_t o_partials, o_tau_part, o_gradrec, o_taurec, scratch_bytes;
  int pre_blocks, nseg;

  __host__ Layout(int N_, int H_, int W_, int64_t cap_) : N(N_), H(H_), W(W_), cap(cap_) {
    gx = (W + kTile - 1) / kTile;
    gy = (H + kTile - 1) / kTile;
    ntiles = gx * gy;
    sgx = (W + kRefTile - 1) / kRefTile;
    sgy = (H + kRefTile - 1) / kRefTile;
    tile_bits = 1;
    while ((1ll << tile_bits) < (long long)ntiles + 1) ++tile_bits;
    size_t o = 0;
    auto take = [&](size_t bytes) { size_t r = o; o = align_up(o + bytes); return r; };
    size_t n = (size_t)(N > 0 ? N : 1), c = (size_t)(cap > 0 ? cap : 1);
    pre_blocks = (N + 255) / 256;
    nseg = (N + kSeg - 1) / kSeg;
    size_t nb = (size_t)(pre_blocks > 0 ? pre_blocks : 1);
    o_hdr = take(sizeof(SavedHeader));
    o_tile_count = take((size_t)((gy + 1) / 2) * ((gx + 1) / 2) * 4 * kCntSlotWords);
    zero_bytes = o;
    o_grec = take(n * sizeof(GRec));
    o_point_list = take(c * 4);
    o_ranges = take((size_t)ntiles * 8 * kRngStride);
    o_tile_maxc = take((size_t)ntiles * 4);
    o_final_T = take((size_t)ntiles * 64 * 8);
    o_tile_order = take((size_t)sgx * sgy * 4 + 16);
    o_block_touched = take(nb * 4);
    o_block_vis = take(nb * 4);
    o_block_base_t = take(nb * 4);
    o_block_base_v = take(nb * 4);
    o_vis_list = take(n * 4);
    o_seg_list = take(n * 4);
    o_vismask = take(n * 4 * kK1MaxParts);
    saved_bytes = o;

    o = 0;
    o_entries = take(c * 8);
    o_bucket = take((size_t)ntiles * kBucket * 8);
    o_ovf = take(c * sizeof(OvfEntry));
    o_partials = take(c * 48);
    o_tau_part = take((size_t)(pre_blocks > 0 ? pre_blocks : 1) * 6 * 4);
    o_gradrec = take(n * 64);
    o_taurec = take(n * 24);
    scratch_bytes = o;
  }
  __host__ LOff dev() const {
    LOff d;
    d.N = N; d.H = H; d.W = W; d.gx = gx; d.gy = gy; d.gxp = (gx + 1) / 2; d.sgx = sgx; d.sgy = sgy; d.ntiles = ntiles; d.pre_blocks = pre_blocks; d.nseg = nseg; d.dbg = debug_flags(); d.mean_hint = 0; d.k1_parts = k1_parts_for(nseg); d.sgx_magic = (uint32_t)((1ull << 32) / (uint64_t)(sgx > 0 ? sgx : 1)) + 1u;
    d.cap = cap;
    d.o_hdr = o_hdr; d.o_tile_count = o_tile_count; d.o_grec = o_grec;
    d.o_point_list = o_point_list; d.o_ranges = o_ranges; d.o_tile_maxc = o_tile_maxc; d.o_final_T = o_final_T;
    d.o_tile_order = o_tile_order; d.o_block_touched = o_block_touched; d.o_block_vis = o_block_vis;
    d.o_block_base_t = o_block_base_t; d.o_block_base_v = o_block_base_v; d.o_vis_list = o_vis_list;
    d.o_seg_list = o_seg_list; d.o_vismask = o_vismask; d.o_entries = o_entries; d.o_bucket = o_bucket; d.o_ovf = o_ovf; d.o_partials = o_partials; d.o_tau_part = o_tau_part;
    d.o_gradrec = o_gradrec; d.o_taurec = o_taurec;
    return d;
  }
};

__device__ __forceinline__ float exposed_image(float ea, float r, float eb) {
#pragma clang fp contract(off)
  const float scaled = ea * r;
  return fminf(fmaxf(scaled + eb, 0.f), 1.f);
}
__device__ __forceinline__ int color_level(float image) { return (int)(image * 255.f); }

struct LossTab {
  const float* image[kMaxViews];
  const float* depth[kMaxViews];
  const float* gt_image[kMaxViews];
  const float* gt_depth[kMaxViews];
  const float* exp_a[kMaxViews];
  const float* exp_b[kMaxViews];
  float* loss[kMaxViews];
  float* dimage[kMaxViews];
  float* ddepth[kMaxViews];
  float* da[kMaxViews];
  float* db[kMaxViews];
  void* parts[kMaxViews];
};
void launch_mapping_loss(const LossTab& tab, int nviews, int HW, float alpha, float thr, float upstream, hipStream_t st);
void launch_mapping_loss_final(const LossTab& tab, int nviews, int HW, int nparts, float alpha, hipStream_t st);
struct LossPart { float rgb, dep, da, db; };
size_t ssim_term_view_maps(int H, int W);
int ssim_loss_nparts(int H, int W);
void launch_ssim_mapping_loss(const LossTab& lt, int v0, int nv, int H, int W, float alpha, float lam, float thr, float upstream,
                              float* maps, hipStream_t st);
struct LossCoef { float w_rgb, w_dep, thr; };

struct AdamConst { float b1, b2, eps; float bc2_sqrt[5], step_size[5]; };
struct AdamGroups { SgrAdamGroup g[5]; int64_t r0[5], r1[5]; };
struct FusedAdam {
  AdamGroups G;
  AdamConst c;
  float iso_coef;
  int grads_clean;
  int gather_only;
  float *s_out, *r_out, *o_out;
  float *stat_accum, *stat_denom, *stat_maxr;
  int tail_views, tail_nparts;
  float tail_inv_rgb, tail_inv_dep, tail_alpha;
  const void* tail_parts[kMaxViews];
  float* tail_loss[kMaxViews];
  float* tail_da[kMaxViews];
  float* tail_db[kMaxViews];
  int exp_rows, exp_width;
  float* exp_param; const float* exp_grad; float* exp_avg; float* exp_avg_sq; int32_t* exp_step; const int32_t* exp_active;
  float exp_lr, exp_b1, exp_b2, exp_eps;
};
int make_fused_adam(int64_t n, const SgrAdamGroup groups[5], float beta1, float beta2, float eps, float iso_weight, FusedAdam* out);
int gaussian_adam_step_act(int64_t n, const SgrAdamGroup groups[5], float beta1, float beta2, float eps, float iso_weight,
                           float* s_out, float* r_out, float* o_out, void* stream);
void launch_gather_adam(const ViewTab& tab, int nviews, const LOff& L, const FusedAdam& fa, hipStream_t st);

enum ProfKind { PK_PRE_FWD = 0, PK_SCAN, PK_SCATTER, PK_BLEND_FUSED, PK_BLEND_FWD, PK_BLEND_BWD, PK_PRE_BWD };
void prof_begin(int kind, hipStream_t st);
void prof_end(int kind, hipStream_t st);
struct ProfScope {
  int kind; hipStream_t st;
  ProfScope(int k, hipStream_t s) : kind(k), st(s) { prof_begin(kind, st); }
  ~ProfScope() { prof_end(kind, st); }
};

__device__ __forceinline__ uint32_t abs_offset(const char* saved, const LOff& L, uint32_t g, uint32_t rel_offset) {
  return rel_offset + ((const uint32_t*)(saved + L.o_block_base_t))[g >> kSegShift];
}
__device__ __forceinline__ const GRec* grec_of(const char* saved, const LOff& L) { return (const GRec*)(saved + L.o_grec); }

struct __attribute__((packed, aligned(4))) F3 { float x, y, z; };
__device__ __forceinline__ F3 ld3(const float* p) { return *(const F3*)p; }
__device__ __forceinline__ void st3(float* p, F3 v) { *(F3*)p = v; }

struct V3 { float x, y, z; };
__device__ __forceinline__ V3 cross(V3 a, V3 b) {
  return {a.y * b.z - a.z * b.y, a.z * b.x - a.x * b.z, a.x * b.y - a.y * b.x};
}

template <int CTRL, int ROW_MASK = 0xf, int BANK_MASK = 0xf>
__device__ __forceinline__ float dpp_f(float old, float v) {
  return __builtin_bit_cast(float, __builtin_amdgcn_update_dpp(__builtin_bit_cast(int, old),
                                                                __builtin_bit_cast(int, v), CTRL, ROW_MASK,
                                                                BANK_MASK, false));
}
constexpr int DPP_ROW_SHR1 = 0x111, DPP_ROW_SHR2 = 0x112, DPP_ROW_SHR4 = 0x114, DPP_ROW_SHR8 = 0x118;
constexpr int DPP_WAVE_SHR1 = 0x138, DPP_ROW_BCAST15 = 0x142, DPP_ROW_BCAST31 = 0x143;

__device__ __forceinline__ float wave_scan_add(float v) {
  v += dpp_f<DPP_ROW_SHR1>(0.f, v);
  v += dpp_f<DPP_ROW_SHR2>(0.f, v);
  v += dpp_f<DPP_ROW_SHR4>(0.f, v);
  v += dpp_f<DPP_ROW_SHR8>(0.f, v);
  v += dpp_f<DPP_ROW_BCAST15, 0xa>(0.f, v);
  v += dpp_f<DPP_ROW_BCAST31, 0xc>(0.f, v);
  return v;
}
__device__ __forceinline__ float wave_scan_mul(float v) {
  v *= dpp_f<DPP_ROW_SHR1>(1.f, v);
  v *= dpp_f<DPP_ROW_SHR2>(1.f, v);
  v *= dpp_f<DPP_ROW_SHR4>(1.f, v);
  v *= dpp_f<DPP_ROW_SHR8>(1.f, v);
  v *= dpp_f<DPP_ROW_BCAST15, 0xa>(1.f, v);
  v *= dpp_f<DPP_ROW_BCAST31, 0xc>(1.f, v);
  return v;
}
template <int CTRL, int ROW_MASK = 0xf>
__device__ __forceinline__ uint32_t dpp_u(uint32_t v) {
  return (uint32_t)__builtin_amdgcn_update_dpp(0, (int)v, CTRL, ROW_MASK, 0xf, false);
}
__device__ __forceinline__ uint32_t wave_scan_add_u32(uint32_t v) {
  v += dpp_u<DPP_ROW_SHR1>(v);
  v += dpp_u<DPP_ROW_SHR2>(v);
  v += dpp_u<DPP_ROW_SHR4>(v);
  v += dpp_u<DPP_ROW_SHR8>(v);
  v += dpp_u<DPP_ROW_BCAST15, 0xa>(v);
  v += dpp_u<DPP_ROW_BCAST31, 0xc>(v);
  return v;
}
__device__ __forceinline__ int wave_max_i32(int v) {
#pragma unroll
  for (int off = 32; off > 0; off >>= 1) v = max(v, __shfl_xor(v, off));
  return v;
}
__device__ __forceinline__ uint32_t block256_exclusive_scan(uint32_t v, uint32_t* red, uint32_t& total) {
  const int lane = threadIdx.x & 63, wv = threadIdx.x >> 6;
  uint32_t inc = wave_scan_add_u32(v);
  if (lane == 63) red[wv] = inc;
  __syncthreads();
  uint32_t w0 = red[0], w1 = red[1], w2 = red[2], w3 = red[3];
  __syncthreads();
  total = w0 + w1 + w2 + w3;
  uint32_t base = (wv > 0 ? w0 : 0u) + (wv > 1 ? w1 : 0u) + (wv > 2 ? w2 : 0u);
  return base + inc - v;
}

__device__ __forceinline__ float wave_shr1(float v, float fill) { return dpp_f<DPP_WAVE_SHR1>(fill, v); }

__device__ __forceinline__ float readlane_f(float v, int lane) {
  return __builtin_bit_cast(float, __builtin_amdgcn_readlane(__builtin_bit_cast(int, v), lane));
}
__device__ __forceinline__ float wave_sum(float v) {
  v = wave_scan_add(v);
  return readlane_f(v, 63);
}

__device__ __forceinline__ double wave_sum_f64(double v) {
#pragma unroll
  for (int off = 32; off > 0; off >>= 1) v += __shfl_xor(v, off);
  return v;
}
template <int N, int WAVES = 4>
__device__ __forceinline__ void block_partials(double (&acc)[N], double* __restrict__ out) {
  __shared__ double red[WAVES][N];
  const int lane = threadIdx.x & 63, wv = threadIdx.x >> 6;
#pragma unroll
  for (int k = 0; k < N; ++k) {
    const double s = wave_sum_f64(acc[k]);
    if (lane == 0) red[wv][k] = s;
  }
  __syncthreads();
  if (threadIdx.x < N) {
    double s = red[0][threadIdx.x];
#pragma unroll
    for (int w = 1; w < WAVES; ++w) s += red[w][threadIdx.x];
    out[threadIdx.x] = s;
  }
}

}
```

splat_slam_amd/csrc/sgr_preprocess.hip:

```cpp
#include "sgr_common.h"

namespace sgr {

struct Cam {
  float vm[16];
  float pm[16];
};

__device__ __forceinline__ void load16(const float* __restrict__ src, float* dst) {
#pragma unroll
  for (int i = 0; i < 16; ++i) dst[i] = src[i];
}

__device__ __forceinline__ void quat_to_R(const float q[4], float R[3][3]) {
  float r = q[0], x = q[1], y = q[2], z = q[3];
  R[0][0] = 1.f - 2.f * (y * y + z * z); R[0][1] = 2.f * (x * y - r * z); R[0][2] = 2.f * (x * z + r * y);
  R[1][0] = 2.f * (x * y + r * z); R[1][1] = 1.f - 2.f * (x * x + z * z); R[1][2] = 2.f * (y * z - r * x);
  R[2][0] = 2.f * (x * z - r * y); R[2][1] = 2.f * (y * z + r * x); R[2][2] = 1.f - 2.f * (x * x + y * y);
}

__device__ __forceinline__ void cov3d_from_scale_rot(const float s[3], float mod, const float q[4], float S6[6]) {
  float R[3][3];
  quat_to_R(q, R);
  float M[3][3];
#pragma unroll
  for (int i = 0; i < 3; ++i)
#pragma unroll
    for (int k = 0; k < 3; ++k) M[i][k] = R[i][k] * (mod * s[k]);
  S6[0] = M[0][0] * M[0][0] + M[0][1] * M[0][1] + M[0][2] * M[0][2];
  S6[1] = M[0][0] * M[1][0] + M[0][1] * M[1][1] + M[0][2] * M[1][2];
  S6[2] = M[0][0] * M[2][0] + M[0][1] * M[2][1] + M[0][2] * M[2][2];
  S6[3] = M[1][0] * M[1][0] + M[1][1] * M[1][1] + M[1][2] * M[1][2];
  S6[4] = M[1][0] * M[2][0] + M[1][1] * M[2][1] + M[1][2] * M[2][2];
  S6[5] = M[2][0] * M[2][0] + M[2][1] * M[2][1] + M[2][2] * M[2][2];
}

struct Ewa {
  float tx, ty, tz;
  bool clamp_x, clamp_y;
  float T[2][3];
  float a, b, c;
};

__device__ __forceinline__ void ewa_T(const float pv[3], const float* vm, float fx, float fy, float limx, float limy, Ewa& e) {
  float tz = pv[2];
  float txtz = pv[0] / tz, tytz = pv[1] / tz;
  e.clamp_x = (txtz < -limx) || (txtz > limx);
  e.clamp_y = (tytz < -limy) || (tytz > limy);
  e.tx = fminf(limx, fmaxf(-limx, txtz)) * tz;
  e.ty = fminf(limy, fmaxf(-limy, tytz)) * tz;
  e.tz = tz;
  float itz = 1.f / tz;
  float J00 = fx * itz, J02 = -fx * e.tx * itz * itz;
  float J11 = fy * itz, J12 = -fy * e.ty * itz * itz;
#pragma unroll
  for (int k = 0; k < 3; ++k) {
    e.T[0][k] = J00 * vm[k * 4 + 0] + J02 * vm[k * 4 + 2];
    e.T[1][k] = J11 * vm[k * 4 + 1] + J12 * vm[k * 4 + 2];
  }
}

__device__ __forceinline__ void ewa_project(const float pv[3], const float* vm, const float S6[6], float fx, float fy,
                                            float limx, float limy, Ewa& e) {
  ewa_T(pv, vm, fx, fy, limx, limy, e);
  float S[3][3] = {{S6[0], S6[1], S6[2]}, {S6[1], S6[3], S6[4]}, {S6[2], S6[4], S6[5]}};
  float TS[2][3];
#pragma unroll
  for (int i = 0; i < 2; ++i)
#pragma unroll
    for (int k = 0; k < 3; ++k) TS[i][k] = e.T[i][0] * S[0][k] + e.T[i][1] * S[1][k] + e.T[i][2] * S[2][k];
  e.a = TS[0][0] * e.T[0][0] + TS[0][1] * e.T[0][1] + TS[0][2] * e.T[0][2] + kDilation;
  e.b = TS[0][0] * e.T[1][0] + TS[0][1] * e.T[1][1] + TS[0][2] * e.T[1][2];
  e.c = TS[1][0] * e.T[1][0] + TS[1][1] * e.T[1][1] + TS[1][2] * e.T[1][2] + kDilation;
}

__device__ __forceinline__ unsigned sh_to_rgb(int deg, const float* __restrict__ sh, const float dir[3], float rgb[3]) {
  float x = dir[0], y = dir[1], z = dir[2];
  unsigned clamped = 0;
#pragma unroll
  for (int c = 0; c < 3; ++c) {
    float r = SH_C0 * sh[c];
    if (deg > 0) {
      r = r - SH_C1 * y * sh[3 + c] + SH_C1 * z * sh[6 + c] - SH_C1 * x * sh[9 + c];
      if (deg > 1) {
        float xx = x * x, yy = y * y, zz = z * z, xy = x * y, yz = y * z, xz = x * z;
        r += SH_C2[0] * xy * sh[12 + c] + SH_C2[1] * yz * sh[15 + c] + SH_C2[2] * (2.f * zz - xx - yy) * sh[18 + c] +
             SH_C2[3] * xz * sh[21 + c] + SH_C2[4] * (xx - yy) * sh[24 + c];
        if (deg > 2) {
          r += SH_C3[0] * y * (3.f * xx - yy) * sh[27 + c] + SH_C3[1] * xy * z * sh[30 + c] +
               SH_C3[2] * y * (4.f * zz - xx - yy) * sh[33 + c] + SH_C3[3] * z * (2.f * zz - 3.f * xx - 3.f * yy) * sh[36 + c] +
               SH_C3[4] * x * (4.f * zz - xx - yy) * sh[39 + c] + SH_C3[5] * z * (xx - yy) * sh[42 + c] +
               SH_C3[6] * x * (xx - 3.f * yy) * sh[45 + c];
        }
      }
    }
    r += 0.5f;
    if (r < 0.f) { clamped |= 1u << c; r = 0.f; }
    rgb[c] = r;
  }
  return clamped;
}

struct PreOut {
  bool visible;
  float rad, px, py, A, B, C, opac, depth, rgb[3];
  int x0, y0, x1, y1;
  unsigned clamped;
};

struct PreIn {
  float p[3], opac, S6[6], c_in[3];
};

__device__ __forceinline__ void preprocess_view(const PreIn& in, int i, int H, int W, int deg, int M, float tanfovx,
                                                float tanfovy, const float* vm, const float* pm,
                                                const float* __restrict__ campos, const float* __restrict__ shs,
                                                bool has_colors, int gx, int gy, int sgx, int sgy, PreOut& o) {
  o.visible = false;
  o.x0 = o.x1 = o.y0 = o.y1 = 0;
  const float* p = in.p;
  float pv[3];
#pragma unroll
  for (int r = 0; r < 3; ++r) pv[r] = vm[r] * p[0] + vm[4 + r] * p[1] + vm[8 + r] * p[2] + vm[12 + r];
  if (!(pv[2] > kNearPlane)) return;
  float ph[4];
#pragma unroll
  for (int r = 0; r < 4; ++r) ph[r] = pm[r] * p[0] + pm[4 + r] * p[1] + pm[8 + r] * p[2] + pm[12 + r];
  float pw = 1.f / (ph[3] + 1e-7f);
  float ndcx = ph[0] * pw, ndcy = ph[1] * pw;
  float fx = W / (2.f * tanfovx), fy = H / (2.f * tanfovy);
  Ewa e;
  ewa_project(pv, vm, in.S6, fx, fy, 1.3f * tanfovx, 1.3f * tanfovy, e);
  float det = e.a * e.c - e.b * e.b;
  if (det == 0.f) return;
  float det_inv = 1.f / det;
  float A = e.c * det_inv, B = -e.b * det_inv, C = e.a * det_inv;
  float mid = 0.5f * (e.a + e.c);
  float disc = sqrtf(fmaxf(0.1f, mid * mid - det));
  float lam = fmaxf(mid + disc, mid - disc);
  float rad = ceilf(3.f * sqrtf(lam));
  float px = ((ndcx + 1.f) * W - 1.f) * 0.5f, py = ((ndcy + 1.f) * H - 1.f) * 0.5f;
  if (!(isfinite(px) && isfinite(py) && isfinite(rad))) return;

  int rx0 = min(sgx, max(0, (int)((px - rad) / (float)kRefTile)));
  int ry0 = min(sgy, max(0, (int)((py - rad) / (float)kRefTile)));
  int rx1 = min(sgx, max(0, (int)((px + rad + (kRefTile - 1)) / (float)kRefTile)));
  int ry1 = min(sgy, max(0, (int)((py + rad + (kRefTile - 1)) / (float)kRefTile)));
  if ((rx1 - rx0) * (ry1 - ry0) == 0) return;

  const float opac = in.opac;
  int x0 = min(gx, 2 * rx0), x1 = min(gx, 2 * rx1), y0 = min(gy, 2 * ry0), y1 = min(gy, 2 * ry1);
  {
    float detc = A * C - B * B;
    float o255 = 255.f * opac;
    if (!(o255 >= 1.f)) {
      x1 = x0;
    } else if (A > 0.f && C > 0.f && detc > 0.f) {
      float tau = 2.f * __logf(o255) * 1.001f + 0.02f;
      float ex = sqrtf(tau * C / detc), ey = sqrtf(tau * A / detc);
      float ext = fmaxf(ex, ey) + 2.f * kTile;
      float err = 4e-7f * (A + C + 2.f * fabsf(B)) * ext * ext;
      if (err < 0.005f && isfinite(ex) && isfinite(ey)) {
        int cx0 = (int)ceilf((px - ex - (kTile - 1)) / (float)kTile - 1e-3f);
        int cx1 = (int)floorf((px + ex) / (float)kTile + 1e-3f) + 1;
        int cy0 = (int)ceilf((py - ey - (kTile - 1)) / (float)kTile - 1e-3f);
        int cy1 = (int)floorf((py + ey) / (float)kTile + 1e-3f) + 1;
        x0 = max(x0, cx0); x1 = min(x1, cx1); y0 = max(y0, cy0); y1 = min(y1, cy1);
        if (x1 < x0) x1 = x0;
        if (y1 < y0) y1 = y0;
      }
    }
  }

  o.clamped = 0;
  if (has_colors) {
    o.rgb[0] = in.c_in[0]; o.rgb[1] = in.c_in[1]; o.rgb[2] = in.c_in[2];
  } else if (deg == 0) {
#pragma unroll
    for (int c = 0; c < 3; ++c) {
      float r = SH_C0 * in.c_in[c] + 0.5f;
      if (r < 0.f) { o.clamped |= 1u << c; r = 0.f; }
      o.rgb[c] = r;
    }
  } else {
    float dir[3] = {p[0] - campos[0], p[1] - campos[1], p[2] - campos[2]};
    float inv = 1.f / sqrtf(dir[0] * dir[0] + dir[1] * dir[1] + dir[2] * dir[2]);
    dir[0] *= inv; dir[1] *= inv; dir[2] *= inv;
    o.clamped = sh_to_rgb(deg, shs + (size_t)i * M * 3, dir, o.rgb);
  }
  o.visible = true;
  o.rad = rad; o.px = px; o.py = py; o.A = A; o.B = B; o.C = C; o.opac = opac; o.depth = pv[2];
  o.x0 = x0; o.y0 = y0; o.x1 = x1; o.y1 = y1;
}

__device__ __forceinline__ bool maybe_visible(const float p[3], float trS, int H, int W, float tanfovx, float tanfovy,
                                              const float* vm, const float* pm, int sgx, int sgy) {
  float pv[3];
#pragma unroll
  for (int r = 0; r < 3; ++r) pv[r] = vm[r] * p[0] + vm[4 + r] * p[1] + vm[8 + r] * p[2] + vm[12 + r];
  if (!(pv[2] > kNearPlane)) return false;
  float ph0 = pm[0] * p[0] + pm[4] * p[1] + pm[8] * p[2] + pm[12];
  float ph1 = pm[1] * p[0] + pm[5] * p[1] + pm[9] * p[2] + pm[13];
  float ph3 = pm[3] * p[0] + pm[7] * p[1] + pm[11] * p[2] + pm[15];
  float pw = __builtin_amdgcn_rcpf(ph3 + 1e-7f);
  float px = ((ph0 * pw + 1.f) * W - 1.f) * 0.5f, py = ((ph1 * pw + 1.f) * H - 1.f) * 0.5f;
  float fx = W / (2.f * tanfovx), fy = H / (2.f * tanfovy);
  const float limx = 1.3f * tanfovx, limy = 1.3f * tanfovy;
  const float itz = __builtin_amdgcn_rcpf(pv[2]);
  const float cx = fminf(limx, fmaxf(-limx, pv[0] * itz)), cy = fminf(limy, fmaxf(-limy, pv[1] * itz));
  const float J00 = fx * itz, J02 = -J00 * cx, J11 = fy * itz, J12 = -J11 * cy;
  float tn = 0.f;
#pragma unroll
  for (int k = 0; k < 3; ++k) {
    const float t0 = J00 * vm[k * 4 + 0] + J02 * vm[k * 4 + 2], t1 = J11 * vm[k * 4 + 1] + J12 * vm[k * 4 + 2];
    tn += t0 * t0 + t1 * t1;
  }
  float rad_b = ceilf(3.f * __builtin_amdgcn_sqrtf(tn * trS * 1.002f + 1.0f)) + 1.f;
  if (!(isfinite(px) && isfinite(py) && isfinite(rad_b))) return true;
  int rx0 = min(sgx, max(0, (int)((px - rad_b) * (1.f / kRefTile))));
  int ry0 = min(sgy, max(0, (int)((py - rad_b) * (1.f / kRefTile))));
  int rx1 = min(sgx, max(0, (int)((px + rad_b + (kRefTile - 1)) * (1.f / kRefTile))));
  int ry1 = min(sgy, max(0, (int)((py + rad_b + (kRefTile - 1)) * (1.f / kRefTile))));
  return (rx1 - rx0) * (ry1 - ry0) != 0;
}

__device__ __forceinline__ float cull_radius_factor(const float* vm, int H, int W, float tanfovx, float tanfovy) {
  float g[3] = {0.f, 0.f, 0.f};
#pragma unroll
  for (int i = 0; i < 3; ++i)
#pragma unroll
    for (int j = 0; j < 3; ++j) {
      const float gij = vm[i] * vm[j] + vm[4 + i] * vm[4 + j] + vm[8 + i] * vm[8 + j];
      g[i] += fabsf(gij);
    }
  const float gmax = fmaxf(g[0], fmaxf(g[1], g[2]));
  const float fx = W / (2.f * tanfovx), fy = H / (2.f * tanfovy), limx = 1.3f * tanfovx, limy = 1.3f * tanfovy;
  return 3.f * sqrtf(gmax * (fx * fx * (1.f + limx * limx) + fy * fy * (1.f + limy * limy))) * 1.003f;
}
__device__ __forceinline__ bool maybe_visible_planes(const float p[3], float s, const float* vm, const float* pm, float K, int H, int W,
                                                     int sgx, int sgy) {
  const float z = vm[2] * p[0] + vm[6] * p[1] + vm[10] * p[2] + vm[14];
  if (!(z > kNearPlane * 0.999f)) return false;
  const float w = pm[3] * p[0] + pm[7] * p[1] + pm[11] * p[2] + pm[15] + 1e-7f;
  if (!(w > 0.f)) return true;
  const float ph0 = pm[0] * p[0] + pm[4] * p[1] + pm[8] * p[2] + pm[12];
  const float ph1 = pm[1] * p[0] + pm[5] * p[1] + pm[9] * p[2] + pm[13];
  const float hx = 0.5f * (float)W, hy = 0.5f * (float)H, ksw = K * s * w;
  const float ax = hx * ph0, ay = hy * ph1;
  const float l = (ax + (hx + 4.5f) * w) * z + ksw;
  const float r = (ax + (hx - 5.5f - (float)(sgx * kRefTile)) * w) * z - ksw;
  const float t = (ay + (hy + 4.5f) * w) * z + ksw;
  const float b = (ay + (hy - 5.5f - (float)(sgy * kRefTile)) * w) * z - ksw;
  return !(l < 0.f) && !(r >= 0.f) && !(t < 0.f) && !(b >= 0.f);
}

__global__ void __launch_bounds__(256) __attribute__((amdgpu_waves_per_eu(5, 8))) preprocess_fwd_kernel(
    ViewTab tab, int nviews, LOff L, Common cm, const float* __restrict__ means3D, const float* __restrict__ opacities,
    const float* __restrict__ shs, const float* __restrict__ colors_precomp, const float* __restrict__ scales,
    const float* __restrict__ rotations, const float* __restrict__ cov3D_precomp) {
  __shared__ float mats[kMaxViews][32];
  __shared__ char* p_saved[kMaxViews];
  __shared__ int32_t* p_radii[kMaxViews];
  __shared__ int32_t* p_ntouched[kMaxViews];
  __shared__ const float* p_campos[kMaxViews];
  __shared__ char* p_scratch[kMaxViews];
  __shared__ const float* p_projraw[kMaxViews];
  __shared__ uint8_t cand[kMaxViews][kSeg];
  __shared__ uint32_t wtot[kMaxViews][4];
  __shared__ uint32_t vstart[kMaxViews + 1];
  __shared__ uint32_t vbase_t[kMaxViews + 1], vbase_v[kMaxViews + 1];
  __shared__ uint32_t red[4];
  __shared__ uint32_t vis_bits[kSeg];
  __shared__ uint32_t op_ex[kSeg];
  __shared__ uint4 op_rect[kSeg];
  __shared__ uint32_t op_depth[kSeg];
  __shared__ float4 op_foot[kSeg][2];
  __shared__ float cullK[kMaxViews];
  __shared__ float seg_box[4][8];
  __shared__ uint32_t seg_views;
  const int N = L.N;
  const int seg = blockIdx.x, seg0 = seg * kSeg;
  const int part = blockIdx.y, nparts = gridDim.y;
  const int tid = threadIdx.x, lane = tid & 63, wv = tid >> 6;

#pragma unroll
  for (int u = 0; u < kMaxViews; ++u) {
    if (u < nviews) {
      if (tid < 16) mats[u][tid] = tab.viewmatrix[u][tid];
      else if (tid < 32) mats[u][tid] = tab.projmatrix[u][tid - 16];
      if (tid == 32) { p_saved[u] = tab.saved[u]; p_radii[u] = tab.radii[u]; p_ntouched[u] = tab.n_touched[u]; p_campos[u] = tab.campos[u]; p_scratch[u] = tab.scratch[u]; p_projraw[u] = tab.projraw[u]; }
    }
  }
  if (tid <= kMaxViews) { vbase_t[tid] = 0u; vbase_v[tid] = 0u; }
  if (tid == 0) seg_views = 0xffffffffu;
  vis_bits[tid] = 0u;
  __syncthreads();
  if (tid < nviews) cullK[tid] = cull_radius_factor(mats[tid], L.H, L.W, cm.tanfovx, cm.tanfovy);
  __syncthreads();

  const int ia = seg0 + tid;
  uint32_t passbits = 0, ranks[4] = {0u, 0u, 0u, 0u};
  {
    float p[3] = {0.f, 0.f, 0.f};
    float trS = 0.f;
    if (ia < N) {
      { const F3 t = ld3(means3D + 3 * ia); p[0] = t.x; p[1] = t.y; p[2] = t.z; }
      if (cov3D_precomp) {
        trS = cov3D_precomp[6 * ia] + cov3D_precomp[6 * ia + 3] + cov3D_precomp[6 * ia + 5];
      } else {
        const F3 sc3 = ld3(scales + 3 * ia);
        const float s0 = sc3.x, s1 = sc3.y, s2 = sc3.z;
        const float4 q = *(const float4*)(rotations + 4 * ia);
        const float n2 = q.x * q.x + q.y * q.y + q.z * q.z + q.w * q.w;
        if (fabsf(n2 - 1.f) < 1e-3f) {
          trS = cm.mod * cm.mod * (s0 * s0 + s1 * s1 + s2 * s2) * 1.01f;
        } else {
          float s_in[3] = {s0, s1, s2}, q_in[4] = {q.x, q.y, q.z, q.w}, S6[6];
          cov3d_from_scale_rot(s_in, cm.mod, q_in, S6);
          trS = (S6[0] + S6[3] + S6[5]) * 1.001f;
        }
      }
    }
    if (!(L.dbg & 4)) {
      const bool in = ia < N && isfinite(p[0]) && isfinite(p[1]) && isfinite(p[2]) && isfinite(trS);
      const bool bad = ia < N && !in;
      float lo[3], hi[3], ts = in ? trS : 0.f;
#pragma unroll
      for (int k = 0; k < 3; ++k) { lo[k] = in ? p[k] : 3.0e38f; hi[k] = in ? p[k] : -3.0e38f; }
#pragma unroll
      for (int off = 32; off > 0; off >>= 1) {
#pragma unroll
        for (int k = 0; k < 3; ++k) { lo[k] = fminf(lo[k], __shfl_xor(lo[k], off)); hi[k] = fmaxf(hi[k], __shfl_xor(hi[k], off)); }
        ts = fmaxf(ts, __shfl_xor(ts, off));
      }
      const unsigned long long anybad = __ballot(bad);
      if (lane == 0) {
        seg_box[wv][0] = lo[0]; seg_box[wv][1] = lo[1]; seg_box[wv][2] = lo[2];
        seg_box[wv][3] = hi[0]; seg_box[wv][4] = hi[1]; seg_box[wv][5] = hi[2];
        seg_box[wv][6] = ts; seg_box[wv][7] = anybad ? 1.f : 0.f;
      }
      __syncthreads();
      if (tid == 0) seg_views = 0u;
      __syncthreads();
      if (tid < nviews) {
        float b0[3], b1[3], tsm = 0.f, anyb = 0.f;
#pragma unroll
        for (int k = 0; k < 3; ++k) { b0[k] = 3.0e38f; b1[k] = -3.0e38f; }
#pragma unroll
        for (int w = 0; w < 4; ++w) {
#pragma unroll
          for (int k = 0; k < 3; ++k) { b0[k] = fminf(b0[k], seg_box[w][k]); b1[k] = fmaxf(b1[k], seg_box[w][3 + k]); }
          tsm = fmaxf(tsm, seg_box[w][6]); anyb = fmaxf(anyb, seg_box[w][7]);
        }
        bool maybe = true;
        if (anyb == 0.f && b0[0] <= b1[0]) {
          const float* vm = mats[tid];
          float v0[3], v1[3];
#pragma unroll
          for (int r = 0; r < 3; ++r) {
            float a = vm[12 + r], bsum = vm[12 + r];
#pragma unroll
            for (int c = 0; c < 3; ++c) {
              const float m = vm[c * 4 + r];
              a += fminf(m * b0[c], m * b1[c]);
              bsum += fmaxf(m * b0[c], m * b1[c]);
            }
            const float pad = 1e-3f * (fabsf(a) + fabsf(bsum)) + 1e-4f;
            v0[r] = a - pad; v1[r] = bsum + pad;
          }
          if (v1[2] <= kNearPlane) {
            maybe = false;
          } else if (v0[2] > kNearPlane) {
            const float fx = L.W / (2.f * cm.tanfovx), fy = L.H / (2.f * cm.tanfovy);
            const float iz0 = 1.f / v0[2], iz1 = 1.f / v1[2];
            const float xz0 = fminf(fminf(v0[0] * iz0, v0[0] * iz1), fminf(v1[0] * iz0, v1[0] * iz1));
            const float xz1 = fmaxf(fmaxf(v0[0] * iz0, v0[0] * iz1), fmaxf(v1[0] * iz0, v1[0] * iz1));
            const float yz0 = fminf(fminf(v0[1] * iz0, v0[1] * iz1), fminf(v1[1] * iz0, v1[1] * iz1));
            const float yz1 = fmaxf(fmaxf(v0[1] * iz0, v0[1] * iz1), fmaxf(v1[1] * iz0, v1[1] * iz1));
            const float limx = 1.3f * cm.tanfovx, limy = 1.3f * cm.tanfovy;
            const float tn = (fx * fx * (1.f + limx * limx) + fy * fy * (1.f + limy * limy)) * iz0 * iz0;
            const float rad = ceilf(3.f * sqrtf(tn * tsm * 1.01f + 1.0f)) + 3.f;
            const float ox = 0.5f * L.W * (p_projraw[tid][8] + 1.f) - 0.5f, oy = 0.5f * L.H * (p_projraw[tid][9] + 1.f) - 0.5f;
            const float px0 = fx * xz0 + ox - rad - 1.f, px1 = fx * xz1 + ox + rad + (kRefTile - 1) + 1.f;
            const float py0 = fy * yz0 + oy - rad - 1.f, py1 = fy * yz1 + oy + rad + (kRefTile - 1) + 1.f;
            if (isfinite(px0) && isfinite(px1) && isfinite(py0) && isfinite(py1) && isfinite(rad))
              maybe = !(px1 < 0.f || py1 < 0.f || px0 >= (float)(L.sgx * kRefTile) || py0 >= (float)(L.sgy * kRefTile));
          }
        }
        if (maybe) atomicOr(&seg_views, 1u << tid);
      }
      __syncthreads();
    }
    const uint32_t segv = seg_views;
    const float sroot = __builtin_amdgcn_sqrtf(fmaxf(trS, 0.f)) * 1.0005f;
#pragma unroll 2
    for (int v = 0; v < nviews; ++v) {
      bool pass = false;
      if (ia < N && (v % nparts) == part) {
        if (!(L.dbg & 16)) {
        p_radii[v][ia] = 0;
        if (p_ntouched[v]) p_ntouched[v][ia] = 0;
        }
        if (L.dbg & 2) pass = (p[0] + trS == 12345.678f);
        else if (segv & (1u << v)) pass = (L.dbg & 8) ? maybe_visible(p, trS, L.H, L.W, cm.tanfovx, cm.tanfovy, mats[v], mats[v] + 16, L.sgx, L.sgy)
                                                      : maybe_visible_planes(p, sroot, mats[v], mats[v] + 16, cullK[v], L.H, L.W, L.sgx, L.sgy);
      }
      const unsigned long long m = __ballot(pass);
      if (lane == 0) wtot[v][wv] = (uint32_t)__popcll(m);
      if (pass) {
        passbits |= 1u << v;
        ranks[v >> 2] |= (uint32_t)__popcll(m & ((1ull << lane) - 1ull)) << ((v & 3) * 8);
      }
    }
  }
  __syncthreads();
  if (tid == 0) {
    uint32_t run = 0;
    for (int v = 0; v < nviews; ++v) {
      vstart[v] = run;
      run += wtot[v][0] + wtot[v][1] + wtot[v][2] + wtot[v][3];
    }
    for (int v = nviews; v <= kMaxViews; ++v) vstart[v] = run;
  }
#pragma unroll 1
  for (int v = 0; v < nviews; ++v) {
    if (passbits & (1u << v)) {
      const uint32_t base = (wv > 0 ? wtot[v][0] : 0u) + (wv > 1 ? wtot[v][1] : 0u) + (wv > 2 ? wtot[v][2] : 0u);
      cand[v][base + ((ranks[v >> 2] >> ((v & 3) * 8)) & 0xffu)] = (uint8_t)tid;
    }
  }
  __syncthreads();
  const uint32_t total = (L.dbg & 1) ? 0u : vstart[kMaxViews];

  uint32_t carry_t = 0, carry_v = 0;
#pragma unroll 1
  for (uint32_t f0 = 0; f0 < total; f0 += 256) {
    const uint32_t f = f0 + tid;
    const bool live = f < total;
    int v = 0;
#pragma unroll
    for (int u = 1; u < kMaxViews; ++u) v += (f >= vstart[u] && u < nviews) ? 1 : 0;
    PreOut o;
    o.visible = false;
    o.x0 = o.x1 = o.y0 = o.y1 = 0;
    int i = 0;
    char* saved = p_saved[v];
    if (live) {
      i = seg0 + (int)cand[v][f - vstart[v]];
      const float* vm = mats[v];
      const float* pm = mats[v] + 16;
      PreIn in;
      { const F3 t = ld3(means3D + 3 * i); in.p[0] = t.x; in.p[1] = t.y; in.p[2] = t.z; }
      in.opac = opacities[i];
      if (cov3D_precomp) {
#pragma unroll
        for (int k = 0; k < 6; ++k) in.S6[k] = cov3D_precomp[6 * i + k];
      } else {
        const F3 sc3 = ld3(scales + 3 * i);
        const float4 q4 = *(const float4*)(rotations + 4 * i);
        float s_in[3] = {sc3.x, sc3.y, sc3.z};
        float q_in[4] = {q4.x, q4.y, q4.z, q4.w};
        cov3d_from_scale_rot(s_in, cm.mod, q_in, in.S6);
      }
      in.c_in[0] = in.c_in[1] = in.c_in[2] = 0.f;
      if (colors_precomp) { in.c_in[0] = colors_precomp[3 * i]; in.c_in[1] = colors_precomp[3 * i + 1]; in.c_in[2] = colors_precomp[3 * i + 2]; }
// ... 544 lines not shown
        for (int off = 1; off < 64; off <<= 1)
#pragma unroll
          for (int j = 0; j < 10; ++j) part[j] += __shfl_xor(part[j], off);
        if ((lane & ~(LPG - 1)) == src)
#pragma unroll
          for (int j = 0; j < 10; ++j) gsum[j] = part[j];
      }
    }
  }
  if (!have || (LPG > 1 && (threadIdx.x & (LPG - 1)) != 0)) return;
  {
    const float G0 = gsum[0], G1 = gsum[1], Gxx = gsum[2], Gxy = gsum[3], Go = gsum[4], Gr = gsum[5], Gg = gsum[6], Gb = gsum[7],
                Gyy = gsum[8], Gd = gsum[9];
    gsum[0] = (-(g1.x * G0) - g1.y * G1) * (0.5f * (float)L.W);
    gsum[1] = (-(g1.z * G1) - g1.y * G0) * (0.5f * (float)L.H);
    gsum[2] = -0.5f * Gxx;
    gsum[3] = -Gxy;
    gsum[4] = -0.5f * Gyy;
    gsum[5] = Go; gsum[6] = Gr; gsum[7] = Gg; gsum[8] = Gb; gsum[9] = Gd;
  }
  float tau[6] = {0.f, 0.f, 0.f, 0.f, 0.f, 0.f};
  GaussGrad acc;
#pragma unroll
  for (int j = 0; j < 3; ++j) { acc.p[j] = 0.f; acc.s[j] = 0.f; acc.rgb_or_sh0[j] = 0.f; }
#pragma unroll
  for (int j = 0; j < 4; ++j) acc.q[j] = 0.f;
#pragma unroll
  for (int j = 0; j < 6; ++j) acc.S6[j] = 0.f;
  acc.op = 0.f; acc.m2[0] = 0.f; acc.m2[1] = 0.f;
  preprocess_bwd_one_view(i, L.H, L.W, cm.deg, cm.M, cm.tanfovx, cm.tanfovy, cm.mod, tab.viewmatrix[v], tab.projmatrix[v],
                          tab.projraw[v], tab.campos[v], means3D, shs, colors_precomp, scales, rotations, cov3D_precomp,
                          gsum, q3.w, dshs, accumulate, acc, tau, cm.upstream_pose_jac);
  float4* rec = (float4*)(tab.scratch[v] + L.o_gradrec) + (size_t)i * 4;
  rec[0] = make_float4(acc.p[0], acc.p[1], acc.p[2], acc.rgb_or_sh0[0]);
  rec[1] = make_float4(acc.rgb_or_sh0[1], acc.rgb_or_sh0[2], acc.op, acc.s[0]);
  rec[2] = make_float4(acc.s[1], acc.s[2], acc.q[0], acc.q[1]);
  rec[3] = make_float4(acc.q[2], acc.q[3], acc.m2[0], acc.m2[1]);
  if (float* m2 = tab.dL_dmeans2D[v]) {
    if (((const SavedHeader*)(saved + L.o_hdr))->overflow == 0u) {
      m2[3 * (size_t)i] = acc.m2[0];
      m2[3 * (size_t)i + 1] = acc.m2[1];
    }
  }
  if (dcov3D) {
#pragma unroll
    for (int j = 0; j < 6; ++j) { if (accumulate) dcov3D[6 * i + j] += acc.S6[j]; else dcov3D[6 * i + j] = acc.S6[j]; }
  }
  if (tab.dL_dtau[v]) {
    float* tr = (float*)(tab.scratch[v] + L.o_taurec) + (size_t)t * 6;
#pragma unroll
    for (int j = 0; j < 6; ++j) tr[j] = tau[j];
  }
}

__global__ void __launch_bounds__(256) grad_gather_kernel(
    ViewTab tab, int nviews, LOff L, int deg, int M, int has_colors, float* __restrict__ dmeans3D,
    float* __restrict__ dmeans2D, float* __restrict__ dopac, float* __restrict__ dshs, float* __restrict__ dcolors,
    float* __restrict__ dscales, float* __restrict__ drots, float* __restrict__ dcov3D, int accumulate,
    float* __restrict__ stat_accum, float* __restrict__ stat_denom, float* __restrict__ stat_maxr) {
  __shared__ float red[4][6];
  const int i = blockIdx.x * blockDim.x + threadIdx.x;
  const bool in_range = i < L.N;
  float a[14];
#pragma unroll
  for (int k = 0; k < 14; ++k) a[k] = 0.f;
  float m2x = 0.f, m2y = 0.f, st_norm = 0.f, st_cnt = 0.f, st_maxr = 0.f;
  bool any = false;
  for (int v = 0; v < nviews; ++v) {
    const bool truncated = ((const SavedHeader*)tab.saved[v])->overflow != 0u;
    const int r = in_range && !truncated ? tab.radii[v][i] : 0;
    uint32_t pos = 0;
    if (r > 0) {
      any = true;
      if (tab.dL_dtau[v]) pos = grec_of(tab.saved[v], L)[i].vis_pos;
      const float4* rec = (const float4*)(tab.scratch[v] + L.o_gradrec) + (size_t)i * 4;
      float4 r0 = rec[0], r1 = rec[1], r2 = rec[2], r3 = rec[3];
      a[0] += r0.x; a[1] += r0.y; a[2] += r0.z; a[3] += r0.w; a[4] += r1.x; a[5] += r1.y; a[6] += r1.z; a[7] += r1.w;
      a[8] += r2.x; a[9] += r2.y; a[10] += r2.z; a[11] += r2.w; a[12] += r3.x; a[13] += r3.y;
      m2x += r3.z; m2y += r3.w;
      st_norm += sqrtf(r3.z * r3.z + r3.w * r3.w);
      st_cnt += 1.f;
      st_maxr = fmaxf(st_maxr, (float)r);
    }
    if (tab.dL_dtau[v]) {
      const float* tr = (const float*)(tab.scratch[v] + L.o_taurec) + (size_t)pos * 6;
      int lane = threadIdx.x & 63, wv = threadIdx.x >> 6;
#pragma unroll
      for (int k = 0; k < 6; ++k) {
        float s = wave_sum(r > 0 ? tr[k] : 0.f);
        if (lane == 0) red[wv][k] = s;
      }
      __syncthreads();
      if (threadIdx.x < 6) {
        int k = threadIdx.x;
        ((float*)(tab.scratch[v] + L.o_tau_part))[(size_t)blockIdx.x * 6 + k] = ((red[0][k] + red[1][k]) + red[2][k]) + red[3][k];
      }
      __syncthreads();
    }
  }
  if (!in_range) return;
  float* sh0 = has_colors ? dcolors : dshs;
  const size_t sh_stride = has_colors ? 3 : (size_t)M * 3;
  if (accumulate) {
    if (!any) return;
    if (dmeans3D) { dmeans3D[3 * i] += a[0]; dmeans3D[3 * i + 1] += a[1]; dmeans3D[3 * i + 2] += a[2]; }
    if (sh0 && (has_colors || deg == 0)) { sh0[i * sh_stride] += a[3]; sh0[i * sh_stride + 1] += a[4]; sh0[i * sh_stride + 2] += a[5]; }
    if (dopac) dopac[i] += a[6];
    if (dscales) { dscales[3 * i] += a[7]; dscales[3 * i + 1] += a[8]; dscales[3 * i + 2] += a[9]; }
    if (drots) { drots[4 * i] += a[10]; drots[4 * i + 1] += a[11]; drots[4 * i + 2] += a[12]; drots[4 * i + 3] += a[13]; }
    if (dmeans2D) { dmeans2D[3 * i] += m2x; dmeans2D[3 * i + 1] += m2y; }
  } else {
    if (dmeans3D) { dmeans3D[3 * i] = a[0]; dmeans3D[3 * i + 1] = a[1]; dmeans3D[3 * i + 2] = a[2]; }
    if (sh0 && (has_colors || deg == 0)) {
      sh0[i * sh_stride] = a[3]; sh0[i * sh_stride + 1] = a[4]; sh0[i * sh_stride + 2] = a[5];
      for (size_t k = 3; k < sh_stride; ++k) sh0[i * sh_stride + k] = 0.f;
    } else if (dshs && !any) {
      for (size_t k = 0; k < sh_stride; ++k) dshs[i * sh_stride + k] = 0.f;
    }
    if (dopac) dopac[i] = a[6];
    if (dscales) { dscales[3 * i] = a[7]; dscales[3 * i + 1] = a[8]; dscales[3 * i + 2] = a[9]; }
    if (drots) { drots[4 * i] = a[10]; drots[4 * i + 1] = a[11]; drots[4 * i + 2] = a[12]; drots[4 * i + 3] = a[13]; }
    if (dmeans2D) { dmeans2D[3 * i] = m2x; dmeans2D[3 * i + 1] = m2y; dmeans2D[3 * i + 2] = 0.f; }
    if (dcov3D && !any) {
#pragma unroll
      for (int k = 0; k < 6; ++k) dcov3D[6 * i + k] = 0.f;
    }
  }
  if (any && stat_accum) {
    stat_accum[i] += st_norm;
    stat_denom[i] += st_cnt;
    stat_maxr[i] = fmaxf(stat_maxr[i], st_maxr);
  }
}

__global__ void __launch_bounds__(384) tau_reduce_kernel(ViewTab tab, LOff L) {
  __shared__ float red[6][64];
  const int v = blockIdx.x;
  float* dtau = tab.dL_dtau[v];
  if (!dtau) return;
  const float* tau_part = (const float*)(tab.scratch[v] + L.o_tau_part);
  const int nblk = L.pre_blocks;
  int k = threadIdx.x / 64, lane = threadIdx.x & 63;
  float acc = 0.f;
  for (int b = lane; b < nblk; b += 64) acc += tau_part[(size_t)b * 6 + k];
  red[k][lane] = acc;
  __syncthreads();
  if (lane == 0) {
    float t = 0.f;
    for (int l = 0; l < 64; ++l) t += red[k][l];
    dtau[k] = t;
  }
}

void launch_preprocess_fwd(const ViewTab& tab, int nviews, const LOff& L, const Common& cm, const SgrInputs& in, hipStream_t st) {
  if (L.N <= 0) return;
  ProfScope prof(PK_PRE_FWD, st);
  hipLaunchKernelGGL(preprocess_fwd_kernel, dim3(L.nseg, min(L.k1_parts, nviews)), dim3(256), 0, st, tab, nviews, L, cm, in.means3D, in.opacities,
                     in.shs, in.colors_precomp, in.scales, in.rotations, in.cov3D_precomp);
}

void launch_preprocess_bwd(const ViewTab& tab, int nviews, const LOff& L, const Common& cm, const SgrInputs& in,
                           const SgrGradInputs& g, const FusedAdam* fused, hipStream_t st, bool mapping_loop) {
  if (L.N <= 0) return;
  ProfScope prof(PK_PRE_BWD, st);
  static const int forced = []() { const char* e = getenv("SGR_DENSE_QUAD"); return e ? atoi(e) : -1; }();
  const bool quad = forced >= 0 ? forced != 0 : (mapping_loop && nviews == 1);
  if (quad)
    hipLaunchKernelGGL(preprocess_bwd_dense_kernel<4>, dim3(L.pre_blocks * 4, nviews), dim3(256), 0, st, tab, L, cm, in.means3D, in.shs,
                       in.colors_precomp, in.scales, in.rotations, in.cov3D_precomp, g.dL_dshs, g.dL_dcov3D_precomp, g.accumulate);
  else
    hipLaunchKernelGGL(preprocess_bwd_dense_kernel<1>, dim3(L.pre_blocks, nviews), dim3(256), 0, st, tab, L, cm, in.means3D, in.shs,
                       in.colors_precomp, in.scales, in.rotations, in.cov3D_precomp, g.dL_dshs, g.dL_dcov3D_precomp, g.accumulate);
  if (fused) {
    launch_gather_adam(tab, nviews, L, *fused, st);
    return;
  }
  hipLaunchKernelGGL(grad_gather_kernel, dim3(L.pre_blocks), dim3(256), 0, st, tab, nviews, L, cm.deg, cm.M,
                     in.colors_precomp != nullptr ? 1 : 0, g.dL_dmeans3D, g.dL_dmeans2D, g.dL_dopacities, g.dL_dshs,
                     g.dL_dcolors_precomp, g.dL_dscales, g.dL_drotations, g.dL_dcov3D_precomp, g.accumulate,
                     g.stat_grad_accum, (g.stat_grad_accum ? g.stat_denom : nullptr),
                     (g.stat_grad_accum ? g.stat_max_radii : nullptr));
  bool any_tau = false;
  for (int v = 0; v < nviews; ++v) any_tau = any_tau || tab.dL_dtau[v] != nullptr;
  if (any_tau) hipLaunchKernelGGL(tau_reduce_kernel, dim3(nviews), dim3(384), 0, st, tab, L);
}

}
```

Baseline: 62.67.

## Defer fused Adam step into next iteration's preprocess forward kernel

Measured after the change: 65.61 (median of 6 runs). 1.05x the previous value.

```diff
diff --git a/include/splat_hip.h b/include/splat_hip.h
--- a/include/splat_hip.h
+++ b/include/splat_hip.h
@@ -131,7 +131,8 @@
 #define SGR_OPT_FUSED_BLEND 0
 #define SGR_OPT_UPSTREAM_POSE_JACOBIAN 1
 #define SGR_OPT_SEGMENT_TEST 2
-#define SGR_OPT_COUNT 3
+#define SGR_OPT_ADAM_IN_K1 3
+#define SGR_OPT_COUNT 4
 int sgr_set_option(int32_t option, int32_t value);
 int sgr_get_option(int32_t option);
 
diff --git a/splat_slam_amd/csrc/sgr_adam_device.h b/splat_slam_amd/csrc/sgr_adam_device.h
--- /dev/null
+++ b/splat_slam_amd/csrc/sgr_adam_device.h
@@ -0,0 +1,269 @@
+#pragma once
+
+#include "sgr_common.h"
+
+namespace sgr {
+
+__device__ __forceinline__ void loss_final_view(const LossPart* __restrict__ parts, int nparts, float inv_rgb, float inv_dep,
+                                                float alpha, float* loss, float* da, float* db, LossPart* red ) {
+#pragma clang fp contract(off)
+  LossPart t = {0.f, 0.f, 0.f, 0.f};
+  for (int i = threadIdx.x; i < nparts; i += 256) {
+    LossPart p = parts[i];
+    t.rgb += p.rgb; t.dep += p.dep; t.da += p.da; t.db += p.db;
+  }
+  float v[4] = {t.rgb, t.dep, t.da, t.db};
+#pragma unroll
+  for (int k = 0; k < 4; ++k) v[k] = wave_sum(v[k]);
+  const int lane = threadIdx.x & 63, wv = threadIdx.x >> 6;
+  if (lane == 0) red[wv] = {v[0], v[1], v[2], v[3]};
+  __syncthreads();
+  if (threadIdx.x == 0) {
+    LossPart s = red[0];
+    for (int w = 1; w < 4; ++w) { s.rgb += red[w].rgb; s.dep += red[w].dep; s.da += red[w].da; s.db += red[w].db; }
+    if (loss) loss[0] = alpha * (s.rgb * inv_rgb) + (1.f - alpha) * (s.dep * inv_dep);
+    if (da) da[0] = s.da;
+    if (db) db[0] = s.db;
+  }
+  __syncthreads();
+}
+
+__device__ __forceinline__ void masked_adam_row(int r, int width, float* __restrict__ p, const float* __restrict__ g,
+                                                float* __restrict__ m, float* __restrict__ v, int32_t* __restrict__ step,
+                                                float lr, float b1, float b2, float eps) {
+#pragma clang fp contract(off)
+  int st = step[r] + 1;
+  step[r] = st;
+  float bc1 = 1.f - powf(b1, (float)st), bc2 = 1.f - powf(b2, (float)st);
+  float step_size = lr / bc1, bc2s = sqrtf(bc2);
+  for (int k = 0; k < width; ++k) {
+    int i = r * width + k;
+    float gi = g[i], mi = m[i], vi = v[i];
+    mi = mi + (gi - mi) * (1.f - b1);
+    vi = vi * b2 + (1.f - b2) * gi * gi;
+    p[i] = p[i] - step_size * (mi / (sqrtf(vi) / bc2s + eps));
+    m[i] = mi;
+    v[i] = vi;
+  }
+}
+
+#define adam_update(p, g, m, v, GRP, c)                      \
+  do {                                                       \
+    m = m + (g - m) * (1.f - c.b1);                          \
+    v = v * c.b2 + (1.f - c.b2) * g * g;                     \
+    float denom_ = sqrtf(v) / c.bc2_sqrt[GRP] + c.eps;       \
+    p = p - c.step_size[GRP] * (m / denom_);                 \
+  } while (0)
+
+template <int MODE>
+__device__ __forceinline__ float take_grad(float* __restrict__ sink, int64_t j, float gathered) {
+  if (MODE == 2) return gathered;
+  float g = sink[j];
+  sink[j] = 0.f;
+  return MODE == 1 ? g + gathered : g;
+}
+
+template <int MODE>
+__device__ __forceinline__ void gaussian_adam_one(int64_t i, const AdamGroups& G, const AdamConst& c, float iso_coef,
+                                                  const float* e , float* __restrict__ s_out,
+                                                  float* __restrict__ r_out, float* __restrict__ o_out, float* keep = nullptr) {
+#pragma clang fp contract(off)
+#pragma unroll
+  for (int grp = 0; grp < 2; ++grp) {
+    const SgrAdamGroup& A = G.g[grp];
+    if (i < G.r0[grp] || i >= G.r1[grp]) continue;
+    float g[3];
+    if (MODE == 2) {
+      g[0] = e[3 * grp]; g[1] = e[3 * grp + 1]; g[2] = e[3 * grp + 2];
+    } else {
+      F3 gs = ld3(A.grad + 3 * i);
+      st3(A.grad + 3 * i, F3{0.f, 0.f, 0.f});
+      g[0] = gs.x; g[1] = gs.y; g[2] = gs.z;
+      if (MODE == 1) { g[0] = g[0] + e[3 * grp]; g[1] = g[1] + e[3 * grp + 1]; g[2] = g[2] + e[3 * grp + 2]; }
+    }
+    if (A.skip) continue;
+    F3 p3 = ld3(A.param + 3 * i), m3 = ld3(A.exp_avg + 3 * i), v3 = ld3(A.exp_avg_sq + 3 * i);
+    float p[3] = {p3.x, p3.y, p3.z}, m[3] = {m3.x, m3.y, m3.z}, v[3] = {v3.x, v3.y, v3.z};
+#pragma unroll
+    for (int k = 0; k < 3; ++k) adam_update(p[k], g[k], m[k], v[k], grp, c);
+    st3(A.param + 3 * i, F3{p[0], p[1], p[2]});
+    st3(A.exp_avg + 3 * i, F3{m[0], m[1], m[2]});
+    st3(A.exp_avg_sq + 3 * i, F3{v[0], v[1], v[2]});
+    if (keep && grp == 0) { keep[0] = p[0]; keep[1] = p[1]; keep[2] = p[2]; }
+  }
+  if (i >= G.r0[2] && i < G.r1[2]) {
+    const SgrAdamGroup& A = G.g[2];
+    float p = A.param[i];
+    float sg = 1.f / (1.f + expf(-p));
+    float g = take_grad<MODE>(A.grad, i, e[6]) * sg * (1.f - sg);
+    if (!A.skip) {
+      float m = A.exp_avg[i], v = A.exp_avg_sq[i];
+      adam_update(p, g, m, v, 2, c);
+      A.param[i] = p; A.exp_avg[i] = m; A.exp_avg_sq[i] = v;
+    }
+    if (o_out) o_out[i] = 1.f / (1.f + expf(-p));
+  }
+  if (i >= G.r0[3] && i < G.r1[3]) {
+    const SgrAdamGroup& A = G.g[3];
+    const F3 p3 = ld3(A.param + 3 * i);
+    float p[3] = {p3.x, p3.y, p3.z}, s[3];
+#pragma unroll
+    for (int k = 0; k < 3; ++k) s[k] = expf(p[k]);
+    float mean = (s[0] + s[1] + s[2]) / 3.f;
+    float sg[3], ssum = 0.f;
+#pragma unroll
+    for (int k = 0; k < 3; ++k) { float d = s[k] - mean; sg[k] = d > 0.f ? 1.f : (d < 0.f ? -1.f : 0.f); ssum += sg[k]; }
+    float gin[3];
+    if (MODE == 2) {
+      gin[0] = e[7]; gin[1] = e[8]; gin[2] = e[9];
+    } else {
+      F3 gs = ld3(A.grad + 3 * i);
+      st3(A.grad + 3 * i, F3{0.f, 0.f, 0.f});
+      gin[0] = gs.x; gin[1] = gs.y; gin[2] = gs.z;
+      if (MODE == 1) { gin[0] = gin[0] + e[7]; gin[1] = gin[1] + e[8]; gin[2] = gin[2] + e[9]; }
+    }
+    if (!A.skip) {
+      F3 m3 = ld3(A.exp_avg + 3 * i), v3 = ld3(A.exp_avg_sq + 3 * i);
+      float m[3] = {m3.x, m3.y, m3.z}, v[3] = {v3.x, v3.y, v3.z};
+#pragma unroll
+      for (int k = 0; k < 3; ++k) {
+        float gs = gin[k] + iso_coef * (sg[k] - ssum / 3.f);
+        float g = gs * s[k];
+        adam_update(p[k], g, m[k], v[k], 3, c);
+      }
+      st3(A.param + 3 * i, F3{p[0], p[1], p[2]});
+      st3(A.exp_avg + 3 * i, F3{m[0], m[1], m[2]});
+      st3(A.exp_avg_sq + 3 * i, F3{v[0], v[1], v[2]});
+    }
+    if (s_out) {
+      const F3 so = F3{expf(p[0]), expf(p[1]), expf(p[2])};
+      st3(s_out + 3 * i, so);
+      if (keep) { keep[3] = so.x; keep[4] = so.y; keep[5] = so.z; }
+    }
+  }
+  if (i >= G.r0[4] && i < G.r1[4]) {
+    const SgrAdamGroup& A = G.g[4];
+    float4 x = *(const float4*)(A.param + 4 * i);
+    float4 gy;
+    if (MODE == 2) {
+      gy = make_float4(e[10], e[11], e[12], e[13]);
+    } else {
+      gy = *(const float4*)(A.grad + 4 * i);
+      *(float4*)(A.grad + 4 * i) = make_float4(0.f, 0.f, 0.f, 0.f);
+      if (MODE == 1) { gy.x += e[10]; gy.y += e[11]; gy.z += e[12]; gy.w += e[13]; }
+    }
+    float nrm = sqrtf(x.x * x.x + x.y * x.y + x.z * x.z + x.w * x.w);
+    float gx[4];
+    if (nrm > 1e-12f) {
+      float inv = 1.f / nrm;
+      float y[4] = {x.x * inv, x.y * inv, x.z * inv, x.w * inv};
+      float dot = y[0] * gy.x + y[1] * gy.y + y[2] * gy.z + y[3] * gy.w;
+      gx[0] = (gy.x - y[0] * dot) * inv; gx[1] = (gy.y - y[1] * dot) * inv;
+      gx[2] = (gy.z - y[2] * dot) * inv; gx[3] = (gy.w - y[3] * dot) * inv;
+    } else {
+      gx[0] = gy.x * 1e12f; gx[1] = gy.y * 1e12f; gx[2] = gy.z * 1e12f; gx[3] = gy.w * 1e12f;
+    }
+    float pp[4] = {x.x, x.y, x.z, x.w};
+    if (!A.skip) {
+      float4 m = *(const float4*)(A.exp_avg + 4 * i), v = *(const float4*)(A.exp_avg_sq + 4 * i);
+      float mm[4] = {m.x, m.y, m.z, m.w}, vv[4] = {v.x, v.y, v.z, v.w};
+#pragma unroll
+      for (int k = 0; k < 4; ++k) adam_update(pp[k], gx[k], mm[k], vv[k], 4, c);
+      *(float4*)(A.param + 4 * i) = make_float4(pp[0], pp[1], pp[2], pp[3]);
+      *(float4*)(A.exp_avg + 4 * i) = make_float4(mm[0], mm[1], mm[2], mm[3]);
+      *(float4*)(A.exp_avg_sq + 4 * i) = make_float4(vv[0], vv[1], vv[2], vv[3]);
+    }
+    if (r_out) {
+      float nn = fmaxf(sqrtf(pp[0] * pp[0] + pp[1] * pp[1] + pp[2] * pp[2] + pp[3] * pp[3]), 1e-12f);
+      const float4 ro = make_float4(pp[0] / nn, pp[1] / nn, pp[2] / nn, pp[3] / nn);
+      *(float4*)(r_out + 4 * i) = ro;
+      if (keep) { keep[6] = ro.x; keep[7] = ro.y; keep[8] = ro.z; keep[9] = ro.w; }
+    }
+  }
+}
+
+struct AdamShared {
+  const char* scratch[kMaxViews];
+  const int32_t* radii[kMaxViews];
+  uint32_t over[kMaxViews];
+  LossPart red[4];
+};
+
+__device__ __forceinline__ void adam_rider_view(const FusedAdam& fa, const char* saved_v, int v, AdamShared& sh) {
+  loss_final_view((const LossPart*)fa.tail_parts[v], fa.tail_nparts, fa.tail_inv_rgb, fa.tail_inv_dep, fa.tail_alpha,
+                  fa.tail_loss[v], fa.tail_da[v], fa.tail_db[v], sh.red);
+  if (threadIdx.x == 0 && fa.exp_rows > 0 && fa.tail_da[v] && ((const SavedHeader*)saved_v)->overflow == 0u) {
+    const ptrdiff_t d = fa.tail_da[v] - fa.exp_grad;
+    if (d >= 0 && d < (ptrdiff_t)fa.exp_rows * fa.exp_width && d % fa.exp_width == 0) {
+      const int r = (int)(d / fa.exp_width);
+      if (fa.exp_active[r])
+        masked_adam_row(r, fa.exp_width, fa.exp_param, fa.exp_grad, fa.exp_avg, fa.exp_avg_sq, fa.exp_step, fa.exp_lr,
+                        fa.exp_b1, fa.exp_b2, fa.exp_eps);
+    }
+  }
+}
+
+template <int MODE>
+__device__ __forceinline__ void gather_adam_segment(const FusedAdam& fa, const AdamViews& av, const LOff& L, int seg, AdamShared& sh,
+                                                    float* keep = nullptr) {
+  const int nviews = av.nviews;
+#pragma unroll
+  for (int u = 0; u < kMaxViews; ++u)
+    if ((int)threadIdx.x == u && u < nviews) {
+      sh.scratch[u] = av.scratch[u];
+      sh.radii[u] = av.radii[u];
+      sh.over[u] = ((const SavedHeader*)av.saved[u])->overflow;
+    }
+  __syncthreads();
+  uint32_t truncated = 0u;
+  for (int u = 0; u < nviews; ++u) truncated |= (sh.over[u] != 0u ? 1u : 0u) << u;
+  const int i = seg * 256 + (int)threadIdx.x;
+  if (i >= L.N) return;
+  float a[14];
+#pragma unroll
+  for (int k = 0; k < 14; ++k) a[k] = 0.f;
+  float st_norm = 0.f, st_cnt = 0.f, st_maxr = 0.f;
+  uint32_t seen = 0u;
+  for (int p = 0; p < min(av.k1_parts, nviews); ++p) seen |= ((const uint32_t*)(av.saved[0] + L.o_vismask))[(size_t)p * L.N + i];
+  seen &= ~truncated;
+  const bool any = seen != 0u;
+  while (seen) {
+    const int v = __builtin_ctz(seen);
+    seen &= seen - 1u;
+    const float4* rec = (const float4*)(sh.scratch[v] + L.o_gradrec) + (size_t)i * 4;
+    const int r = sh.radii[v][i];
+    float4 r0 = rec[0], r1 = rec[1], r2 = rec[2], r3 = rec[3];
+    a[0] += r0.x; a[1] += r0.y; a[2] += r0.z; a[3] += r0.w; a[4] += r1.x; a[5] += r1.y; a[6] += r1.z; a[7] += r1.w;
+    a[8] += r2.x; a[9] += r2.y; a[10] += r2.z; a[11] += r2.w; a[12] += r3.x; a[13] += r3.y;
+    st_norm += sqrtf(r3.z * r3.z + r3.w * r3.w);
+    st_cnt += 1.f;
+    st_maxr = fmaxf(st_maxr, (float)r);
+  }
+  if (any && fa.stat_accum) {
+    fa.stat_accum[i] += st_norm;
+    fa.stat_denom[i] += st_cnt;
+    fa.stat_maxr[i] = fmaxf(fa.stat_maxr[i], st_maxr);
+  }
+  if (MODE == 3) {
+    if (!any) return;
+    float* g0 = fa.G.g[0].grad + 3 * (size_t)i; float* g1 = fa.G.g[1].grad + 3 * (size_t)i; float* g3 = fa.G.g[3].grad + 3 * (size_t)i;
+    float* g4 = fa.G.g[4].grad + 4 * (size_t)i;
+    g0[0] += a[0]; g0[1] += a[1]; g0[2] += a[2];
+    g1[0] += a[3]; g1[1] += a[4]; g1[2] += a[5];
+    fa.G.g[2].grad[i] += a[6];
+    g3[0] += a[7]; g3[1] += a[8]; g3[2] += a[9];
+    g4[0] += a[10]; g4[1] += a[11]; g4[2] += a[12]; g4[3] += a[13];
+    return;
+  }
+  if (MODE == 4) {
+    st3(fa.G.g[0].grad + 3 * (size_t)i, F3{a[0], a[1], a[2]});
+    st3(fa.G.g[1].grad + 3 * (size_t)i, F3{a[3], a[4], a[5]});
+    fa.G.g[2].grad[i] = a[6];
+    st3(fa.G.g[3].grad + 3 * (size_t)i, F3{a[7], a[8], a[9]});
+    *(float4*)(fa.G.g[4].grad + 4 * (size_t)i) = make_float4(a[10], a[11], a[12], a[13]);
+    return;
+  }
+  gaussian_adam_one<MODE >= 3 ? 1 : MODE>(i, fa.G, fa.c, fa.iso_coef, a, fa.s_out, fa.r_out, fa.o_out, keep);
+}
+
+}
diff --git a/splat_slam_amd/csrc/sgr_api.hip b/splat_slam_amd/csrc/sgr_api.hip
--- a/splat_slam_amd/csrc/sgr_api.hip
+++ b/splat_slam_amd/csrc/sgr_api.hip
@@ -10,9 +10,10 @@
 
 namespace sgr {
 
-void launch_preprocess_fwd(const ViewTab&, int, const LOff&, const Common&, const SgrInputs&, hipStream_t);
+void launch_preprocess_fwd(const ViewTab&, int, const LOff&, const Common&, const SgrInputs&, hipStream_t, const K1Adam* adam = nullptr);
+bool k1_can_run_adam(const LOff&, int);
 void launch_preprocess_bwd(const ViewTab&, int, const LOff&, const Common&, const SgrInputs&, const SgrGradInputs&, const FusedAdam*,
-                           hipStream_t, bool mapping_loop = false);
+                           hipStream_t, bool mapping_loop = false, bool defer_adam = false);
 void launch_binning(const ViewTab&, int, const LOff&, hipStream_t);
 void launch_zero_heads(const ViewTab&, int, const LOff&, size_t, hipStream_t);
 void launch_blend_fwd(const ViewTab&, int, const LOff&, const float*, const LossTab*, const LossCoef*, hipStream_t);
@@ -20,7 +21,7 @@
 void launch_blend_fused(const ViewTab&, int, const LOff&, const float*, const LossTab&, const LossCoef&, hipStream_t);
 bool blend_can_fuse(const LOff&);
 
-static int g_opt[SGR_OPT_COUNT] = {1, 0, 0};
+static int g_opt[SGR_OPT_COUNT] = {1, 0, 0, 1};
 
 static thread_local char g_err[512] = "";
 int set_error(int code, const char* fmt, ...) {
@@ -43,6 +44,31 @@
 }
 
 static Layout make_layout(int N, int H, int W, int64_t cap) { return Layout(N, H, W, cap); }
+
+static int adam_in_k1_level() {
+  static const int env = []() { const char* e = getenv("SGR_ADAM_IN_K1"); return e ? atoi(e) : 1; }();
+  return (SGR_ADAM_IN_K1 != 0 && env != 0) ? g_opt[SGR_OPT_ADAM_IN_K1] : 0;
+}
+static bool adam_in_k1_ok(const LOff& d, int nv) {
+  const int level = adam_in_k1_level();
+  return level >= 2 ? d.N > 0 : (level == 1 && k1_can_run_adam(d, nv));
+}
+
+struct AdamCarry {
+  bool allow = false;
+  bool pending = false;
+  int iter = -1, owner = -1;
+  K1Adam step;
+  LOff L;
+};
+static void flush_adam(AdamCarry* c, hipStream_t st) {
+  if (!c || !c->pending) return;
+  ViewTab tab = {};
+  for (int v = 0; v < c->step.av.nviews; ++v) { tab.saved[v] = c->step.av.saved[v]; tab.scratch[v] = c->step.av.scratch[v]; tab.radii[v] = c->step.av.radii[v]; }
+  ProfScope prof(PK_PRE_BWD, st);
+  launch_gather_adam(tab, c->step.av.nviews, c->L, c->step.fa, st);
+  c->pending = false;
+}
 
 struct ProfState {
   static constexpr int kRing = 2048;
@@ -156,11 +182,11 @@
 }
 
 static int forward_batch(const ViewTab& tab, int nviews, const Layout& L, const Common& cm, const SgrInputs& in, hipStream_t st,
-                         bool counters_clean = false, int max_list_hint = 0) {
+                         bool counters_clean = false, int max_list_hint = 0, const K1Adam* adam = nullptr) {
   LOff d = L.dev();
   d.set_hint(max_list_hint);
   if (!counters_clean) launch_zero_heads(tab, nviews, d, L.zero_bytes, st);
-  launch_preprocess_fwd(tab, nviews, d, cm, in, st);
+  launch_preprocess_fwd(tab, nviews, d, cm, in, st, adam);
   launch_binning(tab, nviews, d, st);
   return SGR_OK;
 }
@@ -335,7 +361,7 @@
 
 static int map_views_impl(int32_t num_views, const SgrMapView* views, const SgrInputs* in, const SgrGradInputs* grads, float alpha,
                           float rgb_boundary_threshold, int32_t forward_only, FusedAdam* fused, bool* fused_done,
-                          void* stream, bool store_sinks = false, const SgrSsimTerm* term = nullptr) {
+                          void* stream, bool store_sinks = false, const SgrSsimTerm* term = nullptr, AdamCarry* carry = nullptr) {
   if (fused_done) *fused_done = false;
   if (num_views < 0 || (num_views > 0 && (!views || !in)) || (!forward_only && !grads))
     return set_error(SGR_ERR_INVALID, "map_views: null argument");
@@ -374,6 +400,7 @@
     if (!forward_only && grads && !grads->accumulate && num_views > 1)
       return set_error(SGR_ERR_INVALID, "map_views: several views need accumulate != 0");
   }
+  if (!uniform || f.settings.num_gaussians == 0 || store_sinks || num_views > kMaxViews) flush_adam(carry, st);
   if (store_sinks && !forward_only && grads && !(fused && uniform && f.settings.num_gaussians > 0 && num_views <= kMaxViews)) {
     const size_t n = (size_t)f.settings.num_gaussians, m = (size_t)(f.settings.sh_coeffs > 0 ? f.settings.sh_coeffs : 1);
     if (grads->dL_dmeans3D) HIP_TRY(hipMemsetAsync(grads->dL_dmeans3D, 0, n * 12, st));
@@ -440,7 +467,19 @@
         lt.parts[v] = m.loss_scratch;
       }
     }
-    if (int rc = forward_batch(tab, nv, L, cm, *in, st, all_clean, d.mean_hint)) return rc;
+    const K1Adam* ride = nullptr;
+    if (carry && carry->pending) {
+      if (adam_in_k1_ok(d, nv) && all_clean && !forward_only && !term && carry->L.N == d.N &&
+          carry->L.H == d.H && carry->L.W == d.W && carry->L.cap == d.cap)
+        ride = &carry->step;
+      else
+        flush_adam(carry, st);
+    }
+    if (int rc = forward_batch(tab, nv, L, cm, *in, st, all_clean, d.mean_hint, ride)) return rc;
+    if (ride) {
+      carry->pending = false;
+      d.k1_parts = 1;
+    }
     if (forward_only) {
       launch_blend_fwd(tab, nv, d, f.settings.bg, nullptr, nullptr, st);
       continue;
@@ -472,7 +511,15 @@
     }
     if (term) launch_blend_bwd(tab, nv, d, f.settings.bg, nullptr, nullptr, st);
     else if (!fused_blend) launch_blend_bwd(tab, nv, d, f.settings.bg, &lt, &lc, st);
-    launch_preprocess_bwd(tab, nv, d, cm, *in, *grads, fuse ? fused : nullptr, st, true);
+    const bool defer = fuse && carry && carry->allow && !term && fused->gather_only == 0 && adam_in_k1_ok(d, nv);
+    launch_preprocess_bwd(tab, nv, d, cm, *in, *grads, fuse ? fused : nullptr, st, true, defer);
+    if (defer) {
+      carry->step.fa = *fused;
+      for (int v = 0; v < kMaxViews; ++v) { carry->step.av.saved[v] = tab.saved[v]; carry->step.av.scratch[v] = tab.scratch[v]; carry->step.av.radii[v] = tab.radii[v]; }
+      carry->step.av.nviews = nv; carry->step.av.k1_parts = d.k1_parts;
+      carry->L = d;
+      carry->pending = true; carry->owner = carry->iter;
+    }
     if (fuse && fused_done) *fused_done = true;
   }
   HIP_TRY(hipGetLastError());
@@ -489,9 +536,10 @@
 }
 
 static int map_step_impl(const SgrMapStep* p, bool skip_activate, bool grads_clean, bool allow_fuse, bool* fused_out, void* stream,
-                         const SgrSsimTerm* term = nullptr) {
+                         const SgrSsimTerm* term = nullptr, AdamCarry* carry = nullptr) {
   if (fused_out) *fused_out = false;
   if (!p) return set_error(SGR_ERR_INVALID, "map_step: null argument");
+  if (p->num_views <= 0) flush_adam(carry, (hipStream_t)stream);
   const bool adam_only = p->num_views == 0 && p->adam_groups;
   if (!skip_activate && !adam_only && (p->scaling || p->rotation || p->opacity))
     if (int rc = sgr_activate(p->num_gaussians, p->scaling, p->rotation, p->opacity, p->scales_out, p->rot_out, p->opac_out, stream)) return rc;
@@ -550,7 +598,7 @@
   bool fused = false;
   if (p->num_views > 0)
     if (int rc = map_views_impl(p->num_views, p->views, p->in, p->grads, p->alpha, p->rgb_boundary_threshold, p->forward_only,
-                                try_fuse ? &fa : nullptr, &fused, stream, p->grads_clean == -3 && !p->adam_groups, term))
+                                try_fuse ? &fa : nullptr, &fused, stream, p->grads_clean == -3 && !p->adam_groups, term, carry))
       return rc;
   if (p->adam_groups && !fused)
     if (int rc = gaussian_adam_step_act(p->num_gaussians, p->adam_groups, p->beta1, p->beta2, p->eps, p->iso_weight,
@@ -596,6 +644,7 @@
   st.adam_groups = r->adam_groups;
   const int32_t exp_rows = st.exp_rows;
   bool prev_fused = false;
+  AdamCarry carry;
   for (int it = 0; it < r->num_iters; ++it) {
     for (int j = 0; j < r->picks_per_iter; ++j) {
       const int32_t k = r->picks[(size_t)it * r->picks_per_iter + j];
@@ -632,11 +681,15 @@
       st.exp_step = r->step.exp_step + (row < 0 ? 0 : row);
     }
     bool fused = false;
-    if (int rc = map_step_impl(&st, prev_fused, it == 0 ? r->step.grads_clean > 0 : r->adam_groups != nullptr, r->step.grads_clean >= 0,
-                               &fused, stream, term))
-      return rc;
+    carry.iter = it;
+    carry.allow = it + 1 < r->num_iters && nv > 0 && nv <= kMaxViews;
+    const int rc = map_step_impl(&st, prev_fused, it == 0 ? r->step.grads_clean > 0 : r->adam_groups != nullptr, r->step.grads_clean >= 0,
+                                 &fused, stream, term, &carry);
+    if (carry.pending && (rc != SGR_OK || carry.owner != it)) flush_adam(&carry, (hipStream_t)stream);
+    if (rc) return rc;
     prev_fused = fused;
   }
+  flush_adam(&carry, (hipStream_t)stream);
   return SGR_OK;
 }
 
diff --git a/splat_slam_amd/csrc/sgr_aux.hip b/splat_slam_amd/csrc/sgr_aux.hip
--- a/splat_slam_amd/csrc/sgr_aux.hip
+++ b/splat_slam_amd/csrc/sgr_aux.hip
@@ -3,6 +3,7 @@
 #include <cstdint>
 
 #include "sgr_common.h"
+#include "sgr_adam_device.h"
 #include "sgr_se3_device.h"
 
 namespace sgr {
@@ -56,30 +57,6 @@
   }
 }
 
-__device__ __forceinline__ void loss_final_view(const LossPart* __restrict__ parts, int nparts, float inv_rgb, float inv_dep,
-                                                float alpha, float* loss, float* da, float* db, LossPart* red ) {
-#pragma clang fp contract(off)
-  LossPart t = {0.f, 0.f, 0.f, 0.f};
-  for (int i = threadIdx.x; i < nparts; i += 256) {
-    LossPart p = parts[i];
-    t.rgb += p.rgb; t.dep += p.dep; t.da += p.da; t.db += p.db;
-  }
-  float v[4] = {t.rgb, t.dep, t.da, t.db};
-#pragma unroll
-  for (int k = 0; k < 4; ++k) v[k] = wave_sum(v[k]);
-  const int lane = threadIdx.x & 63, wv = threadIdx.x >> 6;
-  if (lane == 0) red[wv] = {v[0], v[1], v[2], v[3]};
-  __syncthreads();
-  if (threadIdx.x == 0) {
-    LossPart s = red[0];
-    for (int w = 1; w < 4; ++w) { s.rgb += red[w].rgb; s.dep += red[w].dep; s.da += red[w].da; s.db += red[w].db; }
-    if (loss) loss[0] = alpha * (s.rgb * inv_rgb) + (1.f - alpha) * (s.dep * inv_dep);
-    if (da) da[0] = s.da;
-    if (db) db[0] = s.db;
-  }
-  __syncthreads();
-}
-
 __global__ void __launch_bounds__(256) mapping_loss_final_kernel(LossTab tab, int nparts, float inv_rgb, float inv_dep, float alpha) {
   __shared__ LossPart red[4];
   const int vw = blockIdx.x;
@@ -140,25 +117,6 @@
   }
 }
 
-__device__ __forceinline__ void masked_adam_row(int r, int width, float* __restrict__ p, const float* __restrict__ g,
-                                                float* __restrict__ m, float* __restrict__ v, int32_t* __restrict__ step,
-                                                float lr, float b1, float b2, float eps) {
-#pragma clang fp contract(off)
-  int st = step[r] + 1;
-  step[r] = st;
-  float bc1 = 1.f - powf(b1, (float)st), bc2 = 1.f - powf(b2, (float)st);
-  float step_size = lr / bc1, bc2s = sqrtf(bc2);
-  for (int k = 0; k < width; ++k) {
-    int i = r * width + k;
-    float gi = g[i], mi = m[i], vi = v[i];
-    mi = mi + (gi - mi) * (1.f - b1);
-    vi = vi * b2 + (1.f - b2) * gi * gi;
-    p[i] = p[i] - step_size * (mi / (sqrtf(vi) / bc2s + eps));
-    m[i] = mi;
-    v[i] = vi;
-  }
-}
-
 __global__ void masked_adam_kernel(int rows, int width, float* __restrict__ p, const float* __restrict__ g,
                                    float* __restrict__ m, float* __restrict__ v, int32_t* __restrict__ step,
                                    const int32_t* __restrict__ active, float lr, float b1, float b2, float eps) {
@@ -187,134 +145,6 @@
   if (o_out) o_out[i] = 1.f / (1.f + expf(-opacity[i]));
 }
 
-#define adam_update(p, g, m, v, GRP, c)                      \
-  do {                                                       \
-    m = m + (g - m) * (1.f - c.b1);                          \
-    v = v * c.b2 + (1.f - c.b2) * g * g;                     \
-    float denom_ = sqrtf(v) / c.bc2_sqrt[GRP] + c.eps;       \
-    p = p - c.step_size[GRP] * (m / denom_);                 \
-  } while (0)
-
-template <int MODE>
-__device__ __forceinline__ float take_grad(float* __restrict__ sink, int64_t j, float gathered) {
-  if (MODE == 2) return gathered;
-  float g = sink[j];
-  sink[j] = 0.f;
-  return MODE == 1 ? g + gathered : g;
-}
-
-template <int MODE>
-__device__ __forceinline__ void gaussian_adam_one(int64_t i, const AdamGroups& G, const AdamConst& c, float iso_coef,
-                                                  const float* e , float* __restrict__ s_out,
-                                                  float* __restrict__ r_out, float* __restrict__ o_out) {
-#pragma clang fp contract(off)
-#pragma unroll
-  for (int grp = 0; grp < 2; ++grp) {
-    const SgrAdamGroup& A = G.g[grp];
-    if (i < G.r0[grp] || i >= G.r1[grp]) continue;
-    float g[3];
-    if (MODE == 2) {
-      g[0] = e[3 * grp]; g[1] = e[3 * grp + 1]; g[2] = e[3 * grp + 2];
-    } else {
-      F3 gs = ld3(A.grad + 3 * i);
-      st3(A.grad + 3 * i, F3{0.f, 0.f, 0.f});
-      g[0] = gs.x; g[1] = gs.y; g[2] = gs.z;
-      if (MODE == 1) { g[0] = g[0] + e[3 * grp]; g[1] = g[1] + e[3 * grp + 1]; g[2] = g[2] + e[3 * grp + 2]; }
-    }
-    if (A.skip) continue;
-    F3 p3 = ld3(A.param + 3 * i), m3 = ld3(A.exp_avg + 3 * i), v3 = ld3(A.exp_avg_sq + 3 * i);
-    float p[3] = {p3.x, p3.y, p3.z}, m[3] = {m3.x, m3.y, m3.z}, v[3] = {v3.x, v3.y, v3.z};
-#pragma unroll
-    for (int k = 0; k < 3; ++k) adam_update(p[k], g[k], m[k], v[k], grp, c);
-    st3(A.param + 3 * i, F3{p[0], p[1], p[2]});
-    st3(A.exp_avg + 3 * i, F3{m[0], m[1], m[2]});
-    st3(A.exp_avg_sq + 3 * i, F3{v[0], v[1], v[2]});
-  }
-  if (i >= G.r0[2] && i < G.r1[2]) {
-    const SgrAdamGroup& A = G.g[2];
-    float p = A.param[i];
-    float sg = 1.f / (1.f + expf(-p));
-    float g = take_grad<MODE>(A.grad, i, e[6]) * sg * (1.f - sg);
-    if (!A.skip) {
-      float m = A.exp_avg[i], v = A.exp_avg_sq[i];
-      adam_update(p, g, m, v, 2, c);
-      A.param[i] = p; A.exp_avg[i] = m; A.exp_avg_sq[i] = v;
-    }
-    if (o_out) o_out[i] = 1.f / (1.f + expf(-p));
-  }
-  if (i >= G.r0[3] && i < G.r1[3]) {
-    const SgrAdamGroup& A = G.g[3];
-    const F3 p3 = ld3(A.param + 3 * i);
-    float p[3] = {p3.x, p3.y, p3.z}, s[3];
-#pragma unroll
-    for (int k = 0; k < 3; ++k) s[k] = expf(p[k]);
-    float mean = (s[0] + s[1] + s[2]) / 3.f;
-    float sg[3], ssum = 0.f;
-#pragma unroll
-    for (int k = 0; k < 3; ++k) { float d = s[k] - mean; sg[k] = d > 0.f ? 1.f : (d < 0.f ? -1.f : 0.f); ssum += sg[k]; }
-    float gin[3];
-    if (MODE == 2) {
-      gin[0] = e[7]; gin[1] = e[8]; gin[2] = e[9];
-    } else {
-      F3 gs = ld3(A.grad + 3 * i);
-      st3(A.grad + 3 * i, F3{0.f, 0.f, 0.f});
-      gin[0] = gs.x; gin[1] = gs.y; gin[2] = gs.z;
-      if (MODE == 1) { gin[0] = gin[0] + e[7]; gin[1] = gin[1] + e[8]; gin[2] = gin[2] + e[9]; }
-    }
-    if (!A.skip) {
-      F3 m3 = ld3(A.exp_avg + 3 * i), v3 = ld3(A.exp_avg_sq + 3 * i);
-      float m[3] = {m3.x, m3.y, m3.z}, v[3] = {v3.x, v3.y, v3.z};
-#pragma unroll
-      for (int k = 0; k < 3; ++k) {
-        float gs = gin[k] + iso_coef * (sg[k] - ssum / 3.f);
-        float g = gs * s[k];
-        adam_update(p[k], g, m[k], v[k], 3, c);
-      }
-      st3(A.param + 3 * i, F3{p[0], p[1], p[2]});
-      st3(A.exp_avg + 3 * i, F3{m[0], m[1], m[2]});
-      st3(A.exp_avg_sq + 3 * i, F3{v[0], v[1], v[2]});
-    }
-    if (s_out) st3(s_out + 3 * i, F3{expf(p[0]), expf(p[1]), expf(p[2])});
-  }
-  if (i >= G.r0[4] && i < G.r1[4]) {
-    const SgrAdamGroup& A = G.g[4];
-    float4 x = *(const float4*)(A.param + 4 * i);
-    float4 gy;
-    if (MODE == 2) {
-      gy = make_float4(e[10], e[11], e[12], e[13]);
-    } else {
-      gy = *(const float4*)(A.grad + 4 * i);
-      *(float4*)(A.grad + 4 * i) = make_float4(0.f, 0.f, 0.f, 0.f);
-      if (MODE == 1) { gy.x += e[10]; gy.y += e[11]; gy.z += e[12]; gy.w += e[13]; }
-    }
-    float nrm = sqrtf(x.x * x.x + x.y * x.y + x.z * x.z + x.w * x.w);
-    float gx[4];
-    if (nrm > 1e-12f) {
-      float inv = 1.f / nrm;
-      float y[4] = {x.x * inv, x.y * inv, x.z * inv, x.w * inv};
-      float dot = y[0] * gy.x + y[1] * gy.y + y[2] * gy.z + y[3] * gy.w;
-      gx[0] = (gy.x - y[0] * dot) * inv; gx[1] = (gy.y - y[1] * dot) * inv;
-      gx[2] = (gy.z - y[2] * dot) * inv; gx[3] = (gy.w - y[3] * dot) * inv;
-    } else {
-      gx[0] = gy.x * 1e12f; gx[1] = gy.y * 1e12f; gx[2] = gy.z * 1e12f; gx[3] = gy.w * 1e12f;
-    }
-    float pp[4] = {x.x, x.y, x.z, x.w};
-    if (!A.skip) {
-      float4 m = *(const float4*)(A.exp_avg + 4 * i), v = *(const float4*)(A.exp_avg_sq + 4 * i);
-      float mm[4] = {m.x, m.y, m.z, m.w}, vv[4] = {v.x, v.y, v.z, v.w};
-#pragma unroll
-      for (int k = 0; k < 4; ++k) adam_update(pp[k], gx[k], mm[k], vv[k], 4, c);
-      *(float4*)(A.param + 4 * i) = make_float4(pp[0], pp[1], pp[2], pp[3]);
-      *(float4*)(A.exp_avg + 4 * i) = make_float4(mm[0], mm[1], mm[2], mm[3]);
-      *(float4*)(A.exp_avg_sq + 4 * i) = make_float4(vv[0], vv[1], vv[2], vv[3]);
-    }
-    if (r_out) {
-      float nn = fmaxf(sqrtf(pp[0] * pp[0] + pp[1] * pp[1] + pp[2] * pp[2] + pp[3] * pp[3]), 1e-12f);
-      *(float4*)(r_out + 4 * i) = make_float4(pp[0] / nn, pp[1] / nn, pp[2] / nn, pp[3] / nn);
-    }
-  }
-}
-
 __global__ void __launch_bounds__(256) gaussian_adam_kernel(int64_t n, AdamGroups G, AdamConst c, float iso_coef,
                                                             float* __restrict__ s_out, float* __restrict__ r_out,
                                                             float* __restrict__ o_out) {
@@ -326,82 +156,16 @@
 
 template <int MODE>
 __global__ void __launch_bounds__(256) gather_adam_kernel(ViewTab tab, int nviews, LOff L, FusedAdam fa) {
+  __shared__ AdamShared sh;
   if ((int)blockIdx.x < fa.tail_views) {
-    __shared__ LossPart red[4];
-    const int v = blockIdx.x;
-    loss_final_view((const LossPart*)fa.tail_parts[v], fa.tail_nparts, fa.tail_inv_rgb, fa.tail_inv_dep, fa.tail_alpha,
-                    fa.tail_loss[v], fa.tail_da[v], fa.tail_db[v], red);
-    if (threadIdx.x == 0 && fa.exp_rows > 0 && fa.tail_da[v] && ((const SavedHeader*)tab.saved[v])->overflow == 0u) {
-      const ptrdiff_t d = fa.tail_da[v] - fa.exp_grad;
-      if (d >= 0 && d < (ptrdiff_t)fa.exp_rows * fa.exp_width && d % fa.exp_width == 0) {
-        const int r = (int)(d / fa.exp_width);
-        if (fa.exp_active[r])
-          masked_adam_row(r, fa.exp_width, fa.exp_param, fa.exp_grad, fa.exp_avg, fa.exp_avg_sq, fa.exp_step, fa.exp_lr,
-                          fa.exp_b1, fa.exp_b2, fa.exp_eps);
-      }
-    }
+    adam_rider_view(fa, tab.saved[blockIdx.x], (int)blockIdx.x, sh);
     return;
   }
-  __shared__ const char* s_scratch[kMaxViews];
-  __shared__ const int32_t* s_radii[kMaxViews];
-  __shared__ uint32_t s_over[kMaxViews];
+  AdamViews av;
 #pragma unroll
-  for (int u = 0; u < kMaxViews; ++u)
-    if ((int)threadIdx.x == u && u < nviews) {
-      s_scratch[u] = tab.scratch[u];
-      s_radii[u] = tab.radii[u];
-      s_over[u] = ((const SavedHeader*)tab.saved[u])->overflow;
-    }
-  __syncthreads();
-  uint32_t truncated = 0u;
-  for (int u = 0; u < nviews; ++u) truncated |= (s_over[u] != 0u ? 1u : 0u) << u;
-  const int i = ((int)blockIdx.x - fa.tail_views) * blockDim.x + threadIdx.x;
-  if (i >= L.N) return;
-  float a[14];
-#pragma unroll
-  for (int k = 0; k < 14; ++k) a[k] = 0.f;
-  float st_norm = 0.f, st_cnt = 0.f, st_maxr = 0.f;
-  uint32_t seen = 0u;
-  for (int p = 0; p < min(L.k1_parts, nviews); ++p) seen |= ((const uint32_t*)(tab.saved[0] + L.o_vismask))[(size_t)p * L.N + i];
-  seen &= ~truncated;
-  const bool any = seen != 0u;
-  while (seen) {
-    const int v = __builtin_ctz(seen);
-    seen &= seen - 1u;
-    const float4* rec = (const float4*)(s_scratch[v] + L.o_gradrec) + (size_t)i * 4;
-    const int r = s_radii[v][i];
-    float4 r0 = rec[0], r1 = rec[1], r2 = rec[2], r3 = rec[3];
-    a[0] += r0.x; a[1] += r0.y; a[2] += r0.z; a[3] += r0.w; a[4] += r1.x; a[5] += r1.y; a[6] += r1.z; a[7] += r1.w;
-    a[8] += r2.x; a[9] += r2.y; a[10] += r2.z; a[11] += r2.w; a[12] += r3.x; a[13] += r3.y;
-    st_norm += sqrtf(r3.z * r3.z + r3.w * r3.w);
-    st_cnt += 1.f;
-    st_maxr = fmaxf(st_maxr, (float)r);
-  }
-  if (any && fa.stat_accum) {
-    fa.stat_accum[i] += st_norm;
-    fa.stat_denom[i] += st_cnt;
-    fa.stat_maxr[i] = fmaxf(fa.stat_maxr[i], st_maxr);
-  }
-  if (MODE == 3) {
-    if (!any) return;
-    float* g0 = fa.G.g[0].grad + 3 * (size_t)i; float* g1 = fa.G.g[1].grad + 3 * (size_t)i; float* g3 = fa.G.g[3].grad + 3 * (size_t)i;
-    float* g4 = fa.G.g[4].grad + 4 * (size_t)i;
-    g0[0] += a[0]; g0[1] += a[1]; g0[2] += a[2];
-    g1[0] += a[3]; g1[1] += a[4]; g1[2] += a[5];
-    fa.G.g[2].grad[i] += a[6];
-    g3[0] += a[7]; g3[1] += a[8]; g3[2] += a[9];
-    g4[0] += a[10]; g4[1] += a[11]; g4[2] += a[12]; g4[3] += a[13];
-    return;
-  }
-  if (MODE == 4) {
-    st3(fa.G.g[0].grad + 3 * (size_t)i, F3{a[0], a[1], a[2]});
-    st3(fa.G.g[1].grad + 3 * (size_t)i, F3{a[3], a[4], a[5]});
-    fa.G.g[2].grad[i] = a[6];
-    st3(fa.G.g[3].grad + 3 * (size_t)i, F3{a[7], a[8], a[9]});
-    *(float4*)(fa.G.g[4].grad + 4 * (size_t)i) = make_float4(a[10], a[11], a[12], a[13]);
-    return;
-  }
-  gaussian_adam_one<MODE >= 3 ? 1 : MODE>(i, fa.G, fa.c, fa.iso_coef, a, fa.s_out, fa.r_out, fa.o_out);
+  for (int u = 0; u < kMaxViews; ++u) { av.saved[u] = tab.saved[u]; av.scratch[u] = tab.scratch[u]; av.radii[u] = tab.radii[u]; }
+  av.nviews = nviews; av.k1_parts = L.k1_parts;
+  gather_adam_segment<MODE>(fa, av, L, (int)blockIdx.x - fa.tail_views, sh);
 }
 
 int gaussian_adam_step_act(int64_t n, const SgrAdamGroup groups[5], float beta1, float beta2, float eps, float iso_weight,
diff --git a/splat_slam_amd/csrc/sgr_common.h b/splat_slam_amd/csrc/sgr_common.h
--- a/splat_slam_amd/csrc/sgr_common.h
+++ b/splat_slam_amd/csrc/sgr_common.h
@@ -280,6 +280,21 @@
 int gaussian_adam_step_act(int64_t n, const SgrAdamGroup groups[5], float beta1, float beta2, float eps, float iso_weight,
                            float* s_out, float* r_out, float* o_out, void* stream);
 void launch_gather_adam(const ViewTab& tab, int nviews, const LOff& L, const FusedAdam& fa, hipStream_t st);
+struct AdamViews {
+  char* saved[kMaxViews];
+  char* scratch[kMaxViews];
+  int32_t* radii[kMaxViews];
+  int nviews, k1_parts;
+};
+#ifndef SGR_ADAM_IN_K1
+#define SGR_ADAM_IN_K1 1
+#endif
+struct K1Adam {
+  FusedAdam fa;
+  AdamViews av;
+  int regs;
+};
+static_assert(sizeof(ViewTab) + sizeof(LOff) + sizeof(Common) + 7 * sizeof(void*) + sizeof(K1Adam) + 64 <= 4096, "K1's kernarg segment");
 
 enum ProfKind { PK_PRE_FWD = 0, PK_SCAN, PK_SCATTER, PK_BLEND_FUSED, PK_BLEND_FWD, PK_BLEND_BWD, PK_PRE_BWD };
 void prof_begin(int kind, hipStream_t st);
diff --git a/splat_slam_amd/csrc/sgr_preprocess.hip b/splat_slam_amd/csrc/sgr_preprocess.hip
--- a/splat_slam_amd/csrc/sgr_preprocess.hip
+++ b/splat_slam_amd/csrc/sgr_preprocess.hip
@@ -1,4 +1,5 @@
 #include "sgr_common.h"
+#include "sgr_adam_device.h"
 
 namespace sgr {
 
@@ -254,10 +255,28 @@
   return !(l < 0.f) && !(r >= 0.f) && !(t < 0.f) && !(b >= 0.f);
 }
 
+template <bool ADAM> struct K1In { typedef const float* __restrict__ ptr; };
+template <> struct K1In<true> { typedef const float* ptr; };
+struct K1NoAdam { int unused; };
+template <bool ADAM> struct K1Step { typedef K1NoAdam type; };
+template <> struct K1Step<true> { typedef K1Adam type; };
+template <bool ADAM> struct K1Lds { typedef char type; };
+template <> struct K1Lds<true> { typedef AdamShared type; };
+
+template <bool ADAM>
 __global__ void __launch_bounds__(256) __attribute__((amdgpu_waves_per_eu(5, 8))) preprocess_fwd_kernel(
-    ViewTab tab, int nviews, LOff L, Common cm, const float* __restrict__ means3D, const float* __restrict__ opacities,
-    const float* __restrict__ shs, const float* __restrict__ colors_precomp, const float* __restrict__ scales,
-    const float* __restrict__ rotations, const float* __restrict__ cov3D_precomp) {
+    ViewTab tab, int nviews, LOff L, Common cm, typename K1In<ADAM>::ptr means3D, typename K1In<ADAM>::ptr opacities,
+    typename K1In<ADAM>::ptr shs, typename K1In<ADAM>::ptr colors_precomp, typename K1In<ADAM>::ptr scales,
+    typename K1In<ADAM>::ptr rotations, typename K1In<ADAM>::ptr cov3D_precomp, typename K1Step<ADAM>::type ka) {
+  __shared__ typename K1Lds<ADAM>::type ash;
+  int nrider = 0;
+  if constexpr (ADAM) {
+    nrider = ka.fa.tail_views;
+    if ((int)blockIdx.x < nrider) {
+      adam_rider_view(ka.fa, ka.av.saved[blockIdx.x], (int)blockIdx.x, ash);
+      return;
+    }
+  }
   __shared__ float mats[kMaxViews][32];
   __shared__ char* p_saved[kMaxViews];
   __shared__ int32_t* p_radii[kMaxViews];
@@ -279,7 +298,7 @@
   __shared__ float seg_box[4][8];
   __shared__ uint32_t seg_views;
   const int N = L.N;
-  const int seg = blockIdx.x, seg0 = seg * kSeg;
+  const int seg = (int)blockIdx.x - nrider, seg0 = seg * kSeg;
   const int part = blockIdx.y, nparts = gridDim.y;
   const int tid = threadIdx.x, lane = tid & 63, wv = tid >> 6;
 
@@ -297,6 +316,14 @@
   __syncthreads();
   if (tid < nviews) cullK[tid] = cull_radius_factor(mats[tid], L.H, L.W, cm.tanfovx, cm.tanfovy);
   __syncthreads();
+  float kept[10] = {0.f, 0.f, 0.f, 0.f, 0.f, 0.f, 0.f, 0.f, 0.f, 0.f};
+  bool use_kept = false;
+  if constexpr (ADAM) {
+    if (ka.fa.grads_clean) gather_adam_segment<2>(ka.fa, ka.av, L, seg, ash, kept);
+    else gather_adam_segment<1>(ka.fa, ka.av, L, seg, ash, kept);
+    use_kept = ka.regs != 0;
+    if (!use_kept) __syncthreads();
+  }
 
   const int ia = seg0 + tid;
   uint32_t passbits = 0, ranks[4] = {0u, 0u, 0u, 0u};
@@ -304,13 +331,16 @@
     float p[3] = {0.f, 0.f, 0.f};
     float trS = 0.f;
     if (ia < N) {
-      { const F3 t = ld3(means3D + 3 * ia); p[0] = t.x; p[1] = t.y; p[2] = t.z; }
-      if (cov3D_precomp) {
+      if (ADAM && use_kept) { p[0] = kept[0]; p[1] = kept[1]; p[2] = kept[2]; }
+      else { const F3 t = ld3(means3D + 3 * ia); p[0] = t.x; p[1] = t.y; p[2] = t.z; }
+      if (cov3D_precomp && !(ADAM && use_kept)) {
         trS = cov3D_precomp[6 * ia] + cov3D_precomp[6 * ia + 3] + cov3D_precomp[6 * ia + 5];
       } else {
-        const F3 sc3 = ld3(scales + 3 * ia);
+        F3 sc3;
+        float4 q;
+        if (ADAM && use_kept) { sc3 = F3{kept[3], kept[4], kept[5]}; q = make_float4(kept[6], kept[7], kept[8], kept[9]); }
+        else { sc3 = ld3(scales + 3 * ia); q = *(const float4*)(rotations + 4 * ia); }
         const float s0 = sc3.x, s1 = sc3.y, s2 = sc3.z;
-        const float4 q = *(const float4*)(rotations + 4 * ia);
         const float n2 = q.x * q.x + q.y * q.y + q.z * q.z + q.w * q.w;
         if (fabsf(n2 - 1.f) < 1e-3f) {
           trS = cm.mod * cm.mod * (s0 * s0 + s1 * s1 + s2 * s2) * 1.01f;
@@ -1161,17 +1191,29 @@
   }
 }
 
-void launch_preprocess_fwd(const ViewTab& tab, int nviews, const LOff& L, const Common& cm, const SgrInputs& in, hipStream_t st) {
+bool k1_can_run_adam(const LOff& L, int nviews) { return SGR_ADAM_IN_K1 != 0 && L.N > 0 && min(L.k1_parts, nviews) == 1; }
+void launch_preprocess_fwd(const ViewTab& tab, int nviews, const LOff& L, const Common& cm, const SgrInputs& in, hipStream_t st,
+                           const K1Adam* adam) {
   if (L.N <= 0) return;
   ProfScope prof(PK_PRE_FWD, st);
-  hipLaunchKernelGGL(preprocess_fwd_kernel, dim3(L.nseg, min(L.k1_parts, nviews)), dim3(256), 0, st, tab, nviews, L, cm, in.means3D, in.opacities,
-                     in.shs, in.colors_precomp, in.scales, in.rotations, in.cov3D_precomp);
-}
-
-void launch_preprocess_bwd(const ViewTab& tab, int nviews, const LOff& L, const Common& cm, const SgrInputs& in,
-                           const SgrGradInputs& g, const FusedAdam* fused, hipStream_t st, bool mapping_loop) {
-  if (L.N <= 0) return;
-  ProfScope prof(PK_PRE_BWD, st);
+#if SGR_ADAM_IN_K1
+  if (adam) {
+    K1Adam ka = *adam;
+    const AdamGroups& G = ka.fa.G;
+    ka.regs = (!in.cov3D_precomp && in.means3D == G.g[0].param && !G.g[0].skip && G.r0[0] <= 0 && G.r1[0] >= L.N && G.r0[3] <= 0 &&
+               G.r1[3] >= L.N && G.r0[4] <= 0 && G.r1[4] >= L.N && ka.fa.s_out && in.scales == ka.fa.s_out && ka.fa.r_out &&
+               in.rotations == ka.fa.r_out) ? 1 : 0;
+    hipLaunchKernelGGL(preprocess_fwd_kernel<true>, dim3(L.nseg + adam->fa.tail_views, 1), dim3(256), 0, st, tab, nviews, L, cm, in.means3D,
+                       in.opacities, in.shs, in.colors_precomp, in.scales, in.rotations, in.cov3D_precomp, ka);
+    return;
+  }
+#endif
+  hipLaunchKernelGGL(preprocess_fwd_kernel<false>, dim3(L.nseg, min(L.k1_parts, nviews)), dim3(256), 0, st, tab, nviews, L, cm, in.means3D, in.opacities,
+                     in.shs, in.colors_precomp, in.scales, in.rotations, in.cov3D_precomp, K1NoAdam{0});
+}
+
+static void launch_preprocess_bwd_dense(const ViewTab& tab, int nviews, const LOff& L, const Common& cm, const SgrInputs& in,
+                                        const SgrGradInputs& g, hipStream_t st, bool mapping_loop) {
   static const int forced = []() { const char* e = getenv("SGR_DENSE_QUAD"); return e ? atoi(e) : -1; }();
   const bool quad = forced >= 0 ? forced != 0 : (mapping_loop && nviews == 1);
   if (quad)
@@ -1180,10 +1222,23 @@
   else
     hipLaunchKernelGGL(preprocess_bwd_dense_kernel<1>, dim3(L.pre_blocks, nviews), dim3(256), 0, st, tab, L, cm, in.means3D, in.shs,
                        in.colors_precomp, in.scales, in.rotations, in.cov3D_precomp, g.dL_dshs, g.dL_dcov3D_precomp, g.accumulate);
+}
+
+void launch_preprocess_bwd(const ViewTab& tab, int nviews, const LOff& L, const Common& cm, const SgrInputs& in,
+                           const SgrGradInputs& g, const FusedAdam* fused, hipStream_t st, bool mapping_loop, bool defer_adam) {
+  if (L.N <= 0) return;
   if (fused) {
+    {
+      ProfScope prof(PK_PRE_BWD, st);
+      launch_preprocess_bwd_dense(tab, nviews, L, cm, in, g, st, mapping_loop);
+    }
+    if (defer_adam) return;
+    ProfScope prof(PK_PRE_BWD, st);
     launch_gather_adam(tab, nviews, L, *fused, st);
     return;
   }
+  ProfScope prof(PK_PRE_BWD, st);
+  launch_preprocess_bwd_dense(tab, nviews, L, cm, in, g, st, mapping_loop);
   hipLaunchKernelGGL(grad_gather_kernel, dim3(L.pre_blocks), dim3(256), 0, st, tab, nviews, L, cm.deg, cm.M,
                      in.colors_precomp != nullptr ? 1 : 0, g.dL_dmeans3D, g.dL_dmeans2D, g.dL_dopacities, g.dL_dshs,
                      g.dL_dcolors_precomp, g.dL_dscales, g.dL_drotations, g.dL_dcov3D_precomp, g.accumulate,
```
